# choi403/ALG

Measured on AMD Instinct MI355X. Metric: frames/sec (whole node) CogVideoX-5B-I2V 49f x 50-step ALG, higher is better.
Workload: dtype bf16; 1 GPU; BASELINE config 2: CogVideoX-5B-I2V bf16, 49 frames @ 480x720, 50 steps, ALG interval down_up (resize_factor 0.25, interval [0, 0.04]), guidance 6.0; one video per GPU; layers=42, dit_sample_forwards=12, parallelism=dp1

## Files before the change

alg_amd/_lib.py:

```python
from __future__ import annotations

import ctypes
from collections import OrderedDict
import os
from ctypes import POINTER, Structure, byref, c_char_p, c_float, c_int, c_int32, c_int64, c_void_p

import torch

_HERE = os.path.dirname(os.path.abspath(__file__))
LIB_PATH = os.environ.get("ALG_HIP_LIB") or os.path.join(_HERE, "libalg_hip.so")

ALG_F32, ALG_BF16 = 0, 1
ACT_NONE, ACT_GELU_TANH, ACT_SILU = 0, 1, 2
GEMM_BIAS_PER_ROW, GEMM_PERMUTE_COLS, GEMM_GATE_F32, GEMM_GATE_SEG_STRIDE = 1, 4, 8, 16
GEMM_B_PACKED11 = 32

EXPORTS = (
    "alg_version", "alg_last_error", "alg_reload_env", "alg_down_up", "alg_gaussian_blur", "alg_cfg_ddim_step", "alg_gemm_bf16", "alg_gemm_bf16_pair", "alg_gemm_bf16_pair_qk", "alg_pack_b_p11", "alg_pack_b_p11_bytes",
    "alg_flash_attn_d64", "alg_layernorm_modulate", "alg_qk_norm_rope", "alg_patchify", "alg_unpatchify",
    "alg_timestep_embedding", "alg_cfg_combine", "alg_lincomb", "alg_unipc_update", "alg_concat_cast", "alg_flash_attn_d128", "alg_layernorm_mod_f32", "alg_layernorm_mod_f32_fp8", "alg_rmsnorm_rope",
    "alg_wan_modulation", "alg_patchify3d", "alg_unpatchify3d", "alg_timestep_embedding_f32", "alg_linear_f32",
    "alg_gelu_erf", "alg_layernorm_modulate_seg", "alg_headnorm_rope", "alg_masked_mean", "alg_silu", "alg_gemm_fp8", "alg_quantize_fp8_rows",
    "alg_conv_cl_bf16", "alg_vae_groupnorm_workspace", "alg_vae_groupnorm_stats", "alg_vae_spatial_norm", "alg_vae_upsample",
    "alg_vae_pack_latent", "alg_vae_unpack_video", "alg_vae_group_norm", "alg_vae_pad", "alg_vae_repitch",
    "alg_vae_unpack_planes", "alg_rms_norm_rows", "alg_softmax_hilo", "alg_flash_attn_d128_ex", "alg_flash_attn_d128_dual", "alg_rope_half", "alg_patchify_t", "alg_unpatchify_t", "alg_qk_norm_rope_scaled", "alg_flash_attn_d64_ex", "alg_embed_rows", "alg_t5_layernorm", "alg_attn_bias", "alg_mul_bf16", "alg_quick_gelu",
    "alg_lowpass_tables_bytes", "alg_lowpass_tables_build", "alg_down_up_workspace_bytes", "alg_gaussian_blur_workspace_bytes",
    "alg_flash_attn_d64_workspace_bytes", "alg_calib_mfma_bf16", "alg_wall_clock_khz", "alg_attn_clock_tap",
)
_RET_I64 = ("alg_vae_groupnorm_workspace", "alg_lowpass_tables_bytes", "alg_down_up_workspace_bytes",
            "alg_gaussian_blur_workspace_bytes", "alg_flash_attn_d64_workspace_bytes", "alg_pack_b_p11_bytes")


class AlgHipError(RuntimeError):
    pass


class GemmArgs(Structure):
    _fields_ = [
        ("A", c_void_p), ("B", c_void_p), ("C", c_void_p), ("bias", c_void_p), ("R", c_void_p), ("gate", c_void_p),
        ("lda", c_int64), ("ldb", c_int64), ("ldc", c_int64), ("ldr", c_int64),
        ("strideA", c_int64), ("strideB", c_int64), ("strideC", c_int64), ("strideR", c_int64),
        ("strideGate", c_int64),
        ("M", c_int32), ("N", c_int32), ("K", c_int32), ("batch", c_int32),
        ("seg_split", c_int32), ("act", c_int32), ("flags", c_int32),
        ("gate_seg_stride", c_int64), ("perm_col0", c_int32), ("conv_cin_log2", c_int32),
        ("a_scale", c_void_p), ("b_scale", c_void_p), ("strideAScale", c_int64), ("strideBScale", c_int64),
        ("conv_wp", c_int32), ("conv_hpwp", c_int32), ("conv_kw", c_int32), ("reserved1", c_int32),
    ]


class QkNormRopeArgs(Structure):
    _fields_ = [("wq", c_void_p), ("bq", c_void_p), ("wk", c_void_p), ("bk", c_void_p), ("cos_tab", c_void_p),
                ("sin_tab", c_void_p), ("heads", c_int32), ("text_len", c_int32), ("eps", c_float),
                ("q_scale", c_float)]


class VaeGeom(Structure):
    _fields_ = [(n, c_int32) for n in ("frames", "H", "W", "C", "first_len", "seg_len", "lat_first_single", "lat_rate",
                                       "lat_scale", "lat_h", "lat_w")]


_lib = None


def build_library(verbose=False):
    import subprocess

    src = os.path.join(_HERE, "csrc")
    r = subprocess.run(["make", "-C", src, "-j8"], capture_output=True, text=True)
    if verbose or r.returncode != 0:
        print(r.stdout[-4000:])
        print(r.stderr[-4000:])
    if r.returncode != 0:
        raise AlgHipError("building libalg_hip.so failed (see output above)")
    return LIB_PATH


def load_library():
    global _lib
    if _lib is not None:
        return _lib
    if not os.path.exists(LIB_PATH):
        raise AlgHipError(
            "%s not found: the HIP extension is not built (run `python -c 'import __graft_entry__ as g; g.build()'` "
            "or `make -C alg_amd/csrc`).  There is no CPU fallback for the ALG hot path." % LIB_PATH)
    lib = ctypes.CDLL(LIB_PATH)
    lib.alg_version.restype = c_int
    lib.alg_last_error.restype = c_char_p
    lib.alg_reload_env.restype = None
    lib.alg_reload_env.argtypes = []
    lib.alg_down_up.argtypes = [c_void_p, c_void_p, c_int64, c_int, c_int, c_int, c_int, c_int, c_int, c_void_p, c_void_p,
                                c_int64, c_void_p]
    lib.alg_gaussian_blur.argtypes = [c_void_p, c_void_p, c_int64, c_int, c_int, c_int, c_float, c_int, c_void_p, c_int64,
                                      c_void_p]
    lib.alg_lowpass_tables_bytes.argtypes = [c_int] * 4
    lib.alg_lowpass_tables_build.argtypes = [c_void_p, c_int64] + [c_int] * 4 + [c_void_p]
    lib.alg_down_up_workspace_bytes.argtypes = [c_int64] + [c_int] * 4
    lib.alg_gaussian_blur_workspace_bytes.argtypes = [c_int64] + [c_int] * 3
    lib.alg_flash_attn_d64_workspace_bytes.argtypes = [c_int] * 4
    lib.alg_pack_b_p11_bytes.argtypes = [c_int, c_int]
    lib.alg_pack_b_p11_bytes.restype = c_int64
    lib.alg_pack_b_p11.argtypes = [c_void_p, c_void_p, c_int, c_int, c_int64, c_void_p]
    lib.alg_cfg_ddim_step.argtypes = [c_void_p, c_int, c_void_p, c_int, c_int, c_int64, c_float, c_float, c_float,
                                      c_float, c_float, c_void_p]
    lib.alg_cfg_combine.argtypes = [c_void_p, c_void_p, c_int, c_int, c_int64, c_float, c_void_p]
    lib.alg_lincomb.argtypes = [POINTER(c_void_p), POINTER(c_float), POINTER(c_int), c_int, c_void_p, c_int, c_int64,
                                c_void_p]
    lib.alg_concat_cast.argtypes = [POINTER(c_void_p), c_int, POINTER(c_void_p), c_int, c_int] + [c_int64] * 7 + [
        c_void_p, c_int, c_void_p]
    lib.alg_flash_attn_d128.argtypes = [c_void_p] * 4 + [c_int] * 4 + [c_int64] * 8 + [c_float, c_void_p]
    lib.alg_flash_attn_d128_ex.argtypes = [c_void_p] * 4 + [c_int] * 4 + [c_int64] * 8 + [c_float, c_int, c_int, c_void_p]
    lib.alg_flash_attn_d128_dual.argtypes = ([c_void_p] * 3 + [c_int] + [c_int64] * 4 + [c_void_p] * 2 + [c_int] + [c_int64] * 4 +
                                             [c_void_p] + [c_int] * 3 + [c_int64] * 4 + [c_float, c_void_p])
    lib.alg_rope_half.argtypes = [c_void_p, c_void_p, c_void_p, c_void_p, c_int64, c_int, c_int64, c_void_p]
    lib.alg_layernorm_mod_f32.argtypes = [c_void_p] * 6 + [c_int64, c_int, c_int, c_int, c_float, c_void_p]
    lib.alg_layernorm_mod_f32_fp8.argtypes = [c_void_p] * 7 + [c_int64, c_int, c_int, c_int, c_float, c_void_p]
    lib.alg_rmsnorm_rope.argtypes = [c_void_p] * 4 + [c_int64, c_int, c_int, c_int, c_float, c_void_p]
    lib.alg_wan_modulation.argtypes = [c_void_p] * 3 + [c_int] * 5 + [c_void_p]
    lib.alg_patchify3d.argtypes = [c_void_p, c_void_p] + [c_int] * 8 + [c_void_p]
    lib.alg_unpatchify3d.argtypes = [c_void_p, c_int64, c_void_p] + [c_int] * 8 + [c_void_p]
    lib.alg_layernorm_modulate_seg.argtypes = [c_void_p] * 6 + [c_int64, c_int64, c_int, c_int, c_int, c_int64, c_int64,
                                               c_int, c_float, c_void_p]
    lib.alg_headnorm_rope.argtypes = [c_void_p] * 4 + [c_int64, c_int64, c_int, c_int, c_int, c_int, c_float, c_void_p]
    lib.alg_masked_mean.argtypes = [c_void_p, c_void_p, c_void_p, c_int, c_int, c_int, c_void_p]
    lib.alg_silu.argtypes = [c_void_p, c_void_p, c_int64, c_void_p]
    lib.alg_rms_norm_rows.argtypes = [c_void_p, c_void_p, c_void_p, c_int64, c_int, c_int, c_int, c_void_p]
    lib.alg_softmax_hilo.argtypes = [c_void_p, c_void_p, c_void_p, c_int64, c_int, c_int64, ctypes.c_float, c_void_p]
    lib.alg_gemm_fp8.argtypes = [POINTER(GemmArgs), c_void_p]
    lib.alg_conv_cl_bf16.argtypes = [c_void_p] * 5 + [c_int] * 7 + [c_void_p]
    lib.alg_vae_groupnorm_workspace.argtypes = [POINTER(VaeGeom)]
    lib.alg_vae_groupnorm_stats.argtypes = [c_void_p, POINTER(VaeGeom), c_float, c_void_p, c_void_p, c_void_p]
    lib.alg_vae_spatial_norm.argtypes = [c_void_p] * 6 + [POINTER(VaeGeom), c_int, c_void_p]
    lib.alg_vae_group_norm.argtypes = [c_void_p] * 5 + [POINTER(VaeGeom), c_int, c_void_p]
    lib.alg_vae_pad.argtypes = [c_void_p, c_void_p] + [c_int] * 4 + [c_void_p]
    lib.alg_vae_repitch.argtypes = [c_void_p, c_void_p] + [c_int] * 6 + [c_void_p]
    lib.alg_vae_unpack_planes.argtypes = [c_void_p, c_void_p] + [c_int] * 4 + [c_void_p]
    lib.alg_embed_rows.argtypes = [c_void_p, c_void_p, c_void_p, c_int64, c_int, c_int, c_void_p]
    lib.alg_t5_layernorm.argtypes = [c_void_p, c_void_p, c_void_p, c_int64, c_int, c_float, c_void_p]
    lib.alg_attn_bias.argtypes = [c_void_p] * 7 + [c_int, c_int, c_int, c_int, c_int64, c_int64, c_float, c_int, c_void_p]
    lib.alg_quick_gelu.argtypes = [c_void_p, c_int64, c_void_p]
    lib.alg_mul_bf16.argtypes = [c_void_p, c_void_p, c_void_p, c_int64, c_void_p]
    lib.alg_vae_upsample.argtypes = [c_void_p, c_void_p] + [c_int] * 6 + [c_void_p]
    lib.alg_vae_pack_latent.argtypes = [c_void_p, c_int64, c_int64, c_void_p, c_int, c_int, c_int, c_int, c_float, c_void_p]
    lib.alg_vae_unpack_video.argtypes = [c_void_p, c_void_p, c_int, c_int, c_int, c_int, c_void_p]
    lib.alg_quantize_fp8_rows.argtypes = [c_void_p, c_int64, c_void_p, c_void_p, c_int64, c_int, c_void_p]
    lib.alg_timestep_embedding_f32.argtypes = [c_void_p, c_void_p, c_int, c_int, c_void_p]
    lib.alg_linear_f32.argtypes = [c_void_p] * 6 + [c_int] * 4 + [c_void_p]
    lib.alg_gelu_erf.argtypes = [c_void_p, c_int64, c_void_p]
    lib.alg_unipc_update.argtypes = [c_void_p] * 5 + [c_int64] + [c_float] * 6 + [c_void_p]
    lib.alg_gemm_bf16.argtypes = [POINTER(GemmArgs), c_void_p]
    lib.alg_gemm_bf16_pair.argtypes = [POINTER(GemmArgs), POINTER(GemmArgs), c_void_p]
    lib.alg_gemm_bf16_pair_qk.argtypes = [POINTER(GemmArgs), POINTER(GemmArgs), POINTER(QkNormRopeArgs), c_void_p]
    lib.alg_flash_attn_d64.argtypes = [c_void_p, c_void_p, c_void_p, c_void_p, c_int, c_int, c_int, c_int64, c_int64,
                                       c_int64, c_int64, c_int64, c_int64, c_float, c_void_p]
    lib.alg_layernorm_modulate.argtypes = [c_void_p, c_void_p, c_void_p, c_void_p, c_void_p, c_void_p, c_int64, c_int,
                                           c_int, c_int, c_int64, c_int64, c_int, c_float, c_void_p]
    lib.alg_qk_norm_rope.argtypes = [c_void_p, c_void_p, c_void_p, c_void_p, c_void_p, c_void_p, c_void_p, c_int,
                                     c_int, c_int, c_int, c_float, c_void_p]
    lib.alg_qk_norm_rope_scaled.argtypes = [c_void_p] * 7 + [c_int, c_int, c_int, c_int, c_float, c_float, c_void_p]
    lib.alg_flash_attn_d64_ex.argtypes = [c_void_p, c_void_p, c_void_p, c_void_p, c_int, c_int, c_int, c_int64, c_int64,
                                          c_int64, c_int64, c_int64, c_int64, c_float, c_int, c_void_p, c_int64, c_void_p]
    lib.alg_patchify.argtypes = [c_void_p, c_int64, POINTER(c_void_p), c_void_p, c_int, c_int, c_int, c_int, c_int,
                                 c_int, c_void_p]
    lib.alg_unpatchify.argtypes = [c_void_p, c_void_p, c_int, c_int, c_int, c_int, c_int, c_int, c_void_p]
    lib.alg_patchify_t.argtypes = [c_void_p, c_int64, POINTER(c_void_p), c_void_p] + [c_int] * 7 + [c_void_p]
    lib.alg_unpatchify_t.argtypes = [c_void_p, c_void_p] + [c_int] * 7 + [c_void_p]
    lib.alg_timestep_embedding.argtypes = [c_void_p, c_void_p, c_int, c_int, c_int, c_void_p]
    lib.alg_calib_mfma_bf16.argtypes = [c_void_p, c_int, ctypes.c_uint, c_int, c_void_p, c_void_p]
    lib.alg_attn_clock_tap.argtypes = [c_void_p, c_int]
    for name in EXPORTS:
        fn = getattr(lib, name)
        if name == "alg_attn_clock_tap":
            fn.restype = None
        elif name not in ("alg_version", "alg_last_error", "alg_reload_env"):
            fn.restype = c_int64 if name in _RET_I64 else c_int
    _lib = lib
    return lib


def reload_env():
    load_library().alg_reload_env()


def _check(rc, what):
    if rc != 0:
        msg = load_library().alg_last_error()
        raise AlgHipError("%s failed (code %d): %s" % (what, rc, msg.decode() if msg else "?"))


def _stream():
    return c_void_p(torch.cuda.current_stream().cuda_stream)


def _dt(t):
    if t.dtype == torch.float32:
        return ALG_F32
    if t.dtype == torch.bfloat16:
        return ALG_BF16
    raise AlgHipError("unsupported dtype %s (the HIP path handles float32 and bfloat16)" % t.dtype)


def _dev(t, name):
    if not t.is_cuda:
        raise AlgHipError("%s must be a device tensor: the ALG hot path is HIP-only (no CPU fallback)" % name)
    return t


def _ptr(t):
    return c_void_p(t.data_ptr()) if t is not None else c_void_p(0)



_TABLES = OrderedDict()
_TABLES_MAX = 64
_SCRATCH = {}
_PINNED = {}


def _stream_key(t):
    return (t.device.index, torch.cuda.current_stream(t.device).cuda_stream)


def _capturing():
    return torch.cuda.is_available() and torch.cuda.is_current_stream_capturing()


def _pin(t):
    _PINNED[id(t)] = t
    return t


def release_captured_buffers():
    _PINNED.clear()


def clear_caches():
    _TABLES.clear()
    _SCRATCH.clear()


def lowpass_tables(x, h1, w1):
    lib = load_library()
    H, W = x.shape[-2:]
    key = _stream_key(x) + (H, W, h1, w1)
    cap = _capturing()
    t = _TABLES.get(key)
    if t is not None:
        _TABLES.move_to_end(key)
        return _pin(t) if cap else t
    n = int(lib.alg_lowpass_tables_bytes(H, W, h1, w1))
    if n <= 0:
        return None
    t = torch.empty(n, dtype=torch.uint8, device=x.device)
    _check(lib.alg_lowpass_tables_build(_ptr(t), n, H, W, h1, w1, _stream()), "alg_lowpass_tables_build")
    if cap:
        return _pin(t)
    _TABLES[key] = t
    while len(_TABLES) > _TABLES_MAX:
        _TABLES.popitem(last=False)
    return t


def scratch(ref, nbytes, tag):
    if nbytes <= 0:
        return None
    key = _stream_key(ref) + (tag,)
    t = _SCRATCH.get(key)
    cap = _capturing()
    if t is None or t.numel() < nbytes:
        t = torch.empty(int(nbytes), dtype=torch.uint8, device=ref.device)
        if cap:
            return _pin(t)
        _SCRATCH[key] = t
    return _pin(t) if cap else t


def calib_mfma_bf16(sink, iters, seed=1, blocks=0, clocks=None):
    lib = load_library()
    if clocks is not None:
        if int(blocks) <= 0:
            blocks = 2 * torch.cuda.get_device_properties(sink.device).multi_processor_count
        if not (clocks.is_cuda and clocks.device == sink.device and clocks.dtype == torch.int64 and clocks.is_contiguous()
                and clocks.numel() >= 4 * int(blocks)):
            raise AlgHipError("calib_mfma_bf16: clocks must be a contiguous int64 tensor on the sink's device with >= 4 * %d "
                              "elements" % int(blocks))
    rc = lib.alg_calib_mfma_bf16(_ptr(_dev(sink, "sink")), int(iters), int(seed), int(blocks), _ptr(clocks), _stream())
    if rc <= 0:
        _check(rc if rc < 0 else -1, "alg_calib_mfma_bf16")
    return rc


def wall_clock_khz():
    return int(load_library().alg_wall_clock_khz())


def attn_clock_tap(buffer):
    lib = load_library()
    if buffer is None:
        lib.alg_attn_clock_tap(None, 0)
        return
    if not (buffer.is_cuda and buffer.dtype == torch.int64 and buffer.is_contiguous() and buffer.dim() == 2 and buffer.shape[1] == 4):
        raise AlgHipError("attn_clock_tap needs a contiguous int64 device tensor [slots, 4]")
    lib.alg_attn_clock_tap(_ptr(buffer), int(buffer.shape[0]))


def clock_mhz_from_taps(taps, wall_khz):
    t = taps.detach().cpu().to(torch.float64)
    dc, dw = t[:, 2] - t[:, 0], t[:, 3] - t[:, 1]
    ok = (dc > 0) & (dw > 0)
    if not bool(ok.any()) or wall_khz <= 0:
        return None
    mhz = dc[ok] / dw[ok] * (wall_khz / 1e3)
    return {"mean": float(mhz.mean()), "min": float(mhz.min()), "max": float(mhz.max()), "workgroups": int(ok.sum())}


def down_up(x, h1, w1, round_intermediate=True):
    lib = load_library()
    _dev(x, "x")
    if not x.is_contiguous():
        raise AlgHipError("down_up needs a contiguous tensor")
    H, W = x.shape[-2:]
    planes = x.numel() // (H * W) if x.numel() else 0
    out = torch.empty_like(x)
    if planes == 0:
        return out
    wsb = int(lib.alg_down_up_workspace_bytes(planes, H, W, h1, w1))
    ws = scratch(x, wsb, "down_up")
    tables = lowpass_tables(x, h1, w1) if wsb == 0 else None
    _check(lib.alg_down_up(_ptr(x), _ptr(out), planes, H, W, h1, w1, _dt(x), 1 if round_intermediate else 0,
                           _ptr(tables), _ptr(ws), wsb, _stream()), "alg_down_up")
    return out


def gaussian_blur(x, ksize, sigma):
    lib = load_library()
    _dev(x, "x")
    if not x.is_contiguous():
        raise AlgHipError("gaussian_blur needs a contiguous tensor")
    H, W = x.shape[-2:]
    planes = x.numel() // (H * W) if x.numel() else 0
    out = torch.empty_like(x)
    wsb = int(lib.alg_gaussian_blur_workspace_bytes(planes, H, W, int(ksize))) if planes else 0
    ws = scratch(x, wsb, "gaussian")
    _check(lib.alg_gaussian_blur(_ptr(x), _ptr(out), planes, H, W, int(ksize), float(sigma), _dt(x), _ptr(ws), wsb,
                                 _stream()), "alg_gaussian_blur")
    return out


def cfg_ddim_step_(pred, latents, n_pass, guidance_scale, sqrt_alpha_t, sqrt_beta_t, coef_a, coef_b):
    lib = load_library()
    _dev(pred, "pred")
    _dev(latents, "latents")
    if not (pred.is_contiguous() and latents.is_contiguous()):
        raise AlgHipError("cfg_ddim_step_ needs contiguous tensors")
    numel = latents.numel()
    if pred.numel() != n_pass * numel:
        raise AlgHipError("pred has %d elements, expected n_pass*numel = %d" % (pred.numel(), n_pass * numel))
    _check(lib.alg_cfg_ddim_step(_ptr(pred), _dt(pred), _ptr(latents), _dt(latents), n_pass, numel,
                                 float(guidance_scale), float(sqrt_alpha_t), float(sqrt_beta_t), float(coef_a),
                                 float(coef_b), _stream()), "alg_cfg_ddim_step")
    return latents


def cfg_combine(pred, n_pass, guidance_scale):
    lib = load_library()
    _dev(pred, "pred")
    if not pred.is_contiguous() or pred.shape[0] % n_pass:
        raise AlgHipError("cfg_combine needs a contiguous [n_pass * B, ...] tensor")
    out = torch.empty((pred.shape[0] // n_pass,) + tuple(pred.shape[1:]), device=pred.device, dtype=pred.dtype)
    _check(lib.alg_cfg_combine(_ptr(pred), _ptr(out), _dt(pred), n_pass, out.numel(), float(guidance_scale), _stream()),
           "alg_cfg_combine")
    return out


def lincomb(terms, out_dtype, out=None):
    lib = load_library()
    xs = [t for _, t in terms]
    for t in xs:
        _dev(t, "term")
        if not t.is_contiguous() or t.shape != xs[0].shape:
            raise AlgHipError("lincomb needs contiguous tensors of one shape")
    n = len(xs)
    if out is None:
        out = torch.empty(xs[0].shape, device=xs[0].device, dtype=out_dtype)
    elif out.dtype != out_dtype or out.shape != xs[0].shape or not out.is_contiguous():
        raise AlgHipError("lincomb: `out` must be a contiguous tensor of the requested dtype and shape")
    arr = (c_void_p * n)(*[t.data_ptr() for t in xs])
    cf = (c_float * n)(*[float(c) for c, _ in terms])
    dts = (c_int * n)(*[_dt(t) for t in xs])
    _check(lib.alg_lincomb(arr, cf, dts, n, _ptr(out), ALG_F32 if out_dtype == torch.float32 else ALG_BF16,
                           out.numel(), _stream()), "alg_lincomb")
    return out


def concat_cast(src0, src1, O, A0, A1, R, s0_ostride, s1_ostride, a1_off, out_dtype):
    lib = load_library()
    n = len(src0)
    for t in list(src0) + list(src1):
        _dev(t, "concat source")
        if not t.is_contiguous():
            raise AlgHipError("concat_cast needs contiguous sources")
    out = torch.empty((n, O, A0 + A1, R), device=src0[0].device, dtype=out_dtype)
    a0 = (c_void_p * n)(*[t.data_ptr() for t in src0])
    a1 = (c_void_p * n)(*[t.data_ptr() for t in src1])
    _check(lib.alg_concat_cast(a0, _dt(src0[0]), a1, _dt(src1[0]), n, O, A0, A1, R, s0_ostride, s1_ostride, a1_off,
                               _ptr(out), ALG_F32 if out_dtype == torch.float32 else ALG_BF16, _stream()),
           "alg_concat_cast")
    return out


def rope_half_(x, cos, sin, pos, rows, heads, x_rstride, x_off=0):
    _check(load_library().alg_rope_half(_p(x, x_off), _p(cos), _p(sin), _p(pos), rows, heads, x_rstride, _stream()),
           "alg_rope_half")
    return x


def flash_attn_d128_dual(q, k, vt, Skv, k_bs, k_rs, vt_bs, vt_rs, k2, vt2, Skv2, k2_bs, k2_rs, vt2_bs, vt2_rs, o, batch, heads, Sq,
                         q_bs, q_rs, o_bs, o_rs, scale):
    lib = load_library()
    for t in (q, k, vt, k2, vt2, o):
        _dev(t, "attention operand")
    _check(lib.alg_flash_attn_d128_dual(_p(q), _p(k), _p(vt), Skv, k_bs, k_rs, vt_bs, vt_rs, _p(k2), _p(vt2), Skv2, k2_bs, k2_rs,
                                        vt2_bs, vt2_rs, _p(o), batch, heads, Sq, q_bs, q_rs, o_bs, o_rs, float(scale), _stream()),
           "alg_flash_attn_d128_dual")
    return o


def flash_attn_d128(q, k, vt, o, batch, heads, Sq, Skv, q_bs, q_rs, k_bs, k_rs, vt_bs, vt_rs, o_bs, o_rs, scale,
                    q_off=0, k_off=0, vt_off=0, o_off=0, kv_group=1, causal=False):
    lib = load_library()
    for t in (q, k, vt, o):
        _dev(t, "attention operand")
    at = lambda t, off: c_void_p(t.data_ptr() + 2 * off)
    if kv_group != 1 or causal:
        _check(lib.alg_flash_attn_d128_ex(at(q, q_off), at(k, k_off), at(vt, vt_off), at(o, o_off), batch, heads, Sq, Skv, q_bs,
                                          q_rs, k_bs, k_rs, vt_bs, vt_rs, o_bs, o_rs, float(scale), int(kv_group),
                                          int(bool(causal)), _stream()), "alg_flash_attn_d128_ex")
        return o
    _check(lib.alg_flash_attn_d128(at(q, q_off), at(k, k_off), at(vt, vt_off), at(o, o_off), batch, heads, Sq, Skv, q_bs, q_rs, k_bs, k_rs, vt_bs, vt_rs, o_bs, o_rs, float(scale),
                                   _stream()), "alg_flash_attn_d128")
    return o


def _p(t, off=0):
    if t is None:
        return c_void_p(0)
    _dev(t, "tensor")
    return c_void_p(t.data_ptr() + off * t.element_size())


def layernorm_mod_f32(x, y, weight, bias, scale, shift, mod_bstride, batch, rows, D, eps, scale_off=0, shift_off=0):
    _check(load_library().alg_layernorm_mod_f32(_p(x), _p(y), _p(weight), _p(bias), _p(scale, scale_off),
                                                _p(shift, shift_off), mod_bstride, batch, rows, D, float(eps), _stream()),
           "alg_layernorm_mod_f32")
    return y


def layernorm_mod_f32_fp8(x, q8, q8_scale, weight, bias, scale, shift, mod_bstride, batch, rows, D, eps, scale_off=0,
                          shift_off=0):
    _check(load_library().alg_layernorm_mod_f32_fp8(_p(x), _p(q8), _p(q8_scale), _p(weight), _p(bias),
                                                    _p(scale, scale_off), _p(shift, shift_off), mod_bstride, batch, rows,
                                                    D, float(eps), _stream()), "alg_layernorm_mod_f32_fp8")
    return q8


def rmsnorm_rope_(x, weight, cos, sin, x_rstride, batch, rows, D, eps, x_off=0):
    _check(load_library().alg_rmsnorm_rope(_p(x, x_off), _p(weight), _p(cos), _p(sin), x_rstride, batch, rows, D,
                                           float(eps), _stream()), "alg_rmsnorm_rope")
    return x


def wan_modulation(table, vec, out, layers, batch, J, D, vec_per_j):
    _check(load_library().alg_wan_modulation(_p(table), _p(vec), _p(out), layers, batch, J, D, int(vec_per_j), _stream()),
           "alg_wan_modulation")
    return out


def patchify3d(x, out, n, C, F, H, W, ph, pw, Kpad):
    _check(load_library().alg_patchify3d(_p(x), _p(out), n, C, F, H, W, ph, pw, Kpad, _stream()), "alg_patchify3d")
    return out


def unpatchify3d(x, ldin, out, n, C, F, H, W, ph, pw, channel_major=False):
    _check(load_library().alg_unpatchify3d(_p(x), ldin, _p(out), n, C, F, H, W, ph, pw, int(channel_major), _stream()),
           "alg_unpatchify3d")
    return out


def layernorm_modulate_seg(x, y, weight, bias, scale, shift, mod_bstride, seg_stride, batch, rows, D, seg_split, eps,
                           x_bstride=None, y_bstride=None, x_off=0, y_off=0, scale_off=0, shift_off=0):
    x_bstride = rows * D if x_bstride is None else x_bstride
    y_bstride = rows * D if y_bstride is None else y_bstride
    _check(load_library().alg_layernorm_modulate_seg(_p(x, x_off), _p(y, y_off), _p(weight), _p(bias), _p(scale, scale_off),
                                                     _p(shift, shift_off), mod_bstride, seg_stride, batch, rows, D,
                                                     x_bstride, y_bstride, seg_split, float(eps), _stream()),
           "alg_layernorm_modulate_seg")
    return y


def headnorm_rope_(x, weight, cos, sin, x_rstride, x_bstride, batch, rows, heads, rope_tokens, eps, x_off=0):
    _check(load_library().alg_headnorm_rope(_p(x, x_off), _p(weight), _p(cos), _p(sin), x_rstride, x_bstride, batch, rows,
                                            heads, rope_tokens, float(eps), _stream()), "alg_headnorm_rope")
    return x


def masked_mean(x, valid, out, batch, L, D):
    _check(load_library().alg_masked_mean(_p(x), _p(valid), _p(out), batch, L, D, _stream()), "alg_masked_mean")
    return out


def silu(x, y):
    _check(load_library().alg_silu(_p(x), _p(y), x.numel(), _stream()), "alg_silu")
    return y


def rms_norm_rows(x, gamma, y, rows, C, Cp, silu=True):
    _check(load_library().alg_rms_norm_rows(_p(x), _p(gamma), _p(y), rows, C, Cp, int(silu), _stream()), "alg_rms_norm_rows")
    return y


def softmax_hilo(neg_hi, lo, p, rows, cols, ld, scale):
    _check(load_library().alg_softmax_hilo(_p(neg_hi), _p(lo), _p(p), rows, cols, ld, float(scale), _stream()),
           "alg_softmax_hilo")
    return p


CONV_PLAIN, CONV_PAIR, CONV_STRIDE2 = 0, 1, 2


def conv_cl(x, w, bias, res, y, frames, Hp, Wp, Cin, Cout, kt, pair=False, stride2=False, x_off=0, y_off=0, res_off=0):
    mode = CONV_STRIDE2 if stride2 else (CONV_PAIR if pair else CONV_PLAIN)
    _check(load_library().alg_conv_cl_bf16(_p(x, x_off), _p(w), _p(bias), _p(res, res_off), _p(y, y_off), frames, Hp, Wp,
                                           Cin, Cout, kt, mode, _stream()), "alg_conv_cl_bf16")
    return y


def embed_rows(ids, table, out):
    _check(load_library().alg_embed_rows(_p(ids), _p(table), _p(out), ids.numel(), table.shape[1], table.shape[0],
                                         _stream()), "alg_embed_rows")
    return out


def t5_layernorm(x, weight, y, rows, D, eps):
    _check(load_library().alg_t5_layernorm(_p(x), _p(weight), _p(y), rows, D, eps, _stream()), "alg_t5_layernorm")
    return y


def attn_bias(qkv, out, bias_table, rel_bucket, key_mask, batch, heads, L, scale=1.0, head_dim=64, causal=False):
    inner = heads * head_dim
    _check(load_library().alg_attn_bias(_p(qkv), _p(qkv, inner), _p(qkv, 2 * inner), _p(out), _p(bias_table),
                                        _p(rel_bucket), _p(key_mask), batch, heads, head_dim, L, 3 * inner, inner,
                                        float(scale), int(causal), _stream()), "alg_attn_bias")
    return out


def quick_gelu_(x):
    _check(load_library().alg_quick_gelu(_p(x), x.numel(), _stream()), "alg_quick_gelu")
    return x


def mul_bf16(a, b, out):
    _check(load_library().alg_mul_bf16(_p(a), _p(b), _p(out), a.numel(), _stream()), "alg_mul_bf16")
    return out


def vae_group_norm(x, stats, gamma, beta, out, g, silu=True):
    _check(load_library().alg_vae_group_norm(_p(x), _p(stats), _p(gamma), _p(beta), _p(out), byref(g), int(silu),
                                             _stream()), "alg_vae_group_norm")
    return out


def vae_pad(x, out, frames, H, W, C):
    _check(load_library().alg_vae_pad(_p(x), _p(out), frames, H, W, C, _stream()), "alg_vae_pad")
    return out


def vae_repitch(x, out, frames, H, W, C, src_rows, src_wp):
    _check(load_library().alg_vae_repitch(_p(x), _p(out), frames, H, W, C, src_rows, src_wp, _stream()), "alg_vae_repitch")
    return out


def vae_unpack_planes(x, out, frames, H, W, C):
    _check(load_library().alg_vae_unpack_planes(_p(x), _p(out), frames, H, W, C, _stream()), "alg_vae_unpack_planes")
    return out


def pack_conv_pair(w, bias, taps_t):
    co = w.shape[0]
    w = w.reshape(co, taps_t, 3, 3, -1)
    wp = w.new_zeros(2, co, taps_t, 3, 4, w.shape[-1])
    wp[0, :, :, :, 0:3] = w
    wp[1, :, :, :, 1:4] = w
    return wp.reshape(2 * co, -1).contiguous(), torch.cat([bias, bias]).contiguous()


def vae_geom(**kw):
    g = VaeGeom()
    for k, v in kw.items():
        setattr(g, k, v)
    return g


def vae_groupnorm_workspace(g):
    n = load_library().alg_vae_groupnorm_workspace(byref(g))
    if n < 0:
        _check(1, "alg_vae_groupnorm_workspace")
    return n


def vae_groupnorm_stats(x, g, eps, workspace, stats):
    _check(load_library().alg_vae_groupnorm_stats(_p(x), byref(g), eps, _p(workspace), _p(stats), _stream()),
           "alg_vae_groupnorm_stats")
    return stats


def vae_spatial_norm(x, stats, gamma, beta, zyb, out, g, silu=True):
    _check(load_library().alg_vae_spatial_norm(_p(x), _p(stats), _p(gamma), _p(beta), _p(zyb), _p(out), byref(g),
                                               int(silu), _stream()), "alg_vae_spatial_norm")
    return out


def vae_upsample(x, out, frames_out, H, W, C, compress_time, first_single):
    _check(load_library().alg_vae_upsample(_p(x), _p(out), frames_out, H, W, C, int(compress_time), int(first_single),
                                           _stream()), "alg_vae_upsample")
    return out


def vae_pack_latent(z, c_stride, frame_stride, out, frames, h, w, channels, scale, z_off=0):
    _check(load_library().alg_vae_pack_latent(_p(z, z_off), c_stride, frame_stride, _p(out), frames, h, w, channels, scale,
                                              _stream()), "alg_vae_pack_latent")
    return out


def vae_unpack_video(x, out, frames, H, W, to_uint8=False):
    _check(load_library().alg_vae_unpack_video(_p(x), _p(out), frames, H, W, int(to_uint8), _stream()),
           "alg_vae_unpack_video")
    return out


def timestep_embedding_f32(t, out, n, dim):
    _check(load_library().alg_timestep_embedding_f32(_p(t), _p(out), n, dim, _stream()), "alg_timestep_embedding_f32")
    return out


def linear_f32(x, W, b, y, y_bf16, y_silu_bf16, M, N, K, act=0):
    _check(load_library().alg_linear_f32(_p(x), _p(W), _p(b), _p(y), _p(y_bf16), _p(y_silu_bf16), M, N, K, act, _stream()),
           "alg_linear_f32")


def gelu_erf_(x):
    _check(load_library().alg_gelu_erf(_p(x), x.numel(), _stream()), "alg_gelu_erf")
    return x


def unipc_update(x, m0, m1, m_new, r, c, k, rk=1.0, rho0=0.0, rho_new=0.0):
    lib = load_library()
    for t in (x, m0, m1, m_new):
        if t is None:
            continue
        _dev(t, "unipc term")
        if t.dtype != torch.float32 or not t.is_contiguous() or t.shape != x.shape:
            raise AlgHipError("unipc_update needs contiguous fp32 tensors of one shape")
    out = torch.empty_like(x)
    p = lambda t: None if t is None else _ptr(t)
    _check(lib.alg_unipc_update(p(x), p(m0), p(m1), p(m_new), _ptr(out), x.numel(), float(r), float(c), float(k),
                                float(rk), float(rho0), float(rho_new), _stream()), "alg_unipc_update")
    return out


def gemm_args(A, B, C, M, N, K, lda, ldb, ldc, bias=None, R=None, ldr=0, gate=None, batch=1, strideA=0, strideB=0,
              strideC=0, strideR=0, strideGate=0, seg_split=0, act=ACT_NONE, flags=0, a_off=0, b_off=0, c_off=0, r_off=0,
              gate_off=0, gate_seg_stride=None, bias_off=0, perm_col0=0, a_scale=None, b_scale=None, strideAScale=0,
              strideBScale=0, a_scale_off=0, b_scale_off=0):
    args = GemmArgs()
    fp8 = a_scale is not None
    if isinstance(B, PackedB):
        if fp8:
            raise AlgHipError("a packed B holds bf16 weight fragments for GEMM schedule 11: the e4m3 GEMM takes a row-major B")
        if (B.N, B.K) != (N, K) or b_off or strideB:
            raise AlgHipError("packed B was built for N = %d, K = %d (shared by the batch, no offset)" % (B.N, B.K))
        flags |= GEMM_B_PACKED11
    args.A = A.data_ptr() + A.element_size() * a_off
    args.B = B.data_ptr() + B.element_size() * b_off
    if fp8:
        args.a_scale = a_scale.data_ptr() + 4 * a_scale_off
        args.b_scale = b_scale.data_ptr() + 4 * b_scale_off
        args.strideAScale, args.strideBScale = strideAScale, strideBScale
    args.C = C.data_ptr() + 2 * c_off
    args.bias = (bias.data_ptr() + 2 * bias_off) if bias is not None else None
    if gate_seg_stride is not None:
        flags |= GEMM_GATE_SEG_STRIDE
        args.gate_seg_stride = gate_seg_stride
    args.R = (R.data_ptr() + 2 * r_off) if R is not None else None
    args.gate = (gate.data_ptr() + gate.element_size() * gate_off) if gate is not None else None
    args.lda, args.ldb, args.ldc, args.ldr = lda, ldb, ldc, ldr
    args.strideA, args.strideB, args.strideC, args.strideR, args.strideGate = strideA, strideB, strideC, strideR, strideGate
    args.M, args.N, args.K, args.batch = M, N, K, batch
    args.seg_split, args.act, args.flags = seg_split, act, flags
    args.perm_col0 = perm_col0
    return args, fp8


class PackedB:

    def __init__(self, w):
        lib = load_library()
        _dev(w, "weight")
        if w.dtype != torch.bfloat16 or w.dim() != 2 or w.stride(1) != 1:
            raise AlgHipError("PackedB takes a 2-D bf16 weight with unit column stride")
        self.N, self.K = int(w.shape[0]), int(w.shape[1])
        nbytes = int(lib.alg_pack_b_p11_bytes(self.N, self.K))
        if nbytes <= 0:
            raise AlgHipError("PackedB: K = %d must be a positive multiple of 64" % self.K)
        self.data = torch.empty(nbytes, dtype=torch.uint8, device=w.device)
        _check(lib.alg_pack_b_p11(_ptr(w), _ptr(self.data), self.N, self.K, int(w.stride(0)), _stream()), "alg_pack_b_p11")

    def data_ptr(self):
        return self.data.data_ptr()

    def element_size(self):
        return 2


def gemm(*a, **kw):
    lib = load_library()
    args, fp8 = gemm_args(*a, **kw)
    if fp8:
        _check(lib.alg_gemm_fp8(ctypes.byref(args), _stream()), "alg_gemm_fp8")
    else:
        _check(lib.alg_gemm_bf16(ctypes.byref(args), _stream()), "alg_gemm_bf16")


def gemm_pair(first, second):
    lib = load_library()
    a, fa = gemm_args(*first[0], **first[1])
    b, fb = gemm_args(*second[0], **second[1])
    if fa or fb:
        raise AlgHipError("gemm_pair takes bf16 problems")
    _check(lib.alg_gemm_bf16_pair(ctypes.byref(a), ctypes.byref(b), _stream()), "alg_gemm_bf16_pair")


def gemm_pair_qk(first, second, wq, bq, wk, bk, cos, sin, heads, text_len, eps, q_scale=1.0):
    lib = load_library()
    a, fa = gemm_args(*first[0], **first[1])
    b, fb = gemm_args(*second[0], **second[1])
    if fa or fb:
        raise AlgHipError("gemm_pair_qk takes bf16 problems")
    ptrs = [t.data_ptr() if t is not None else None for t in (wq, bq, wk, bk, cos, sin)]
    e = QkNormRopeArgs(*ptrs, heads, text_len, float(eps), float(q_scale))
    _check(lib.alg_gemm_bf16_pair_qk(ctypes.byref(a), ctypes.byref(b), ctypes.byref(e), _stream()), "alg_gemm_bf16_pair_qk")


def quantize_fp8_rows(x, q, scale, rows, K, x_rstride=None, x_off=0, q_off=0, scale_off=0):
    x_rstride = K if x_rstride is None else x_rstride
    _check(load_library().alg_quantize_fp8_rows(_p(x, x_off), x_rstride, _p(q, q_off), _p(scale, scale_off), rows, K,
                                                _stream()), "alg_quantize_fp8_rows")
    return q, scale


ATTN_Q_PRESCALED = 1


def flash_attn_d64(q, k, vt, o, batch, heads, S, q_bstride, q_rstride, vt_bstride, vt_rstride, o_bstride, o_rstride,
                   scale, q_off=0, k_off=0, q_prescaled=False):
    lib = load_library()
    flags = ATTN_Q_PRESCALED if q_prescaled else 0
    wsb = int(lib.alg_flash_attn_d64_workspace_bytes(batch, heads, S, flags))
    ws = scratch(o, wsb, "attn_d64")
    _check(lib.alg_flash_attn_d64_ex(c_void_p(q.data_ptr() + 2 * q_off), c_void_p(k.data_ptr() + 2 * k_off), _ptr(vt),
                                     _ptr(o), batch, heads, S, q_bstride, q_rstride, vt_bstride, vt_rstride, o_bstride,
                                     o_rstride, float(scale), flags, _ptr(ws), wsb, _stream()),
           "alg_flash_attn_d64")


def layernorm_modulate(x, y, weight, bias, scale, shift, mod_bstride, batch, rows, D, seg_split, eps,
                       x_bstride=None, y_bstride=None, x_off=0, y_off=0, scale_off=0, shift_off=0):
    lib = load_library()
    x_bstride = rows * D if x_bstride is None else x_bstride
    y_bstride = rows * D if y_bstride is None else y_bstride
    sc = c_void_p(scale.data_ptr() + 2 * scale_off) if scale is not None else c_void_p(0)
    sh = c_void_p(shift.data_ptr() + 2 * shift_off) if shift is not None else c_void_p(0)
    _check(lib.alg_layernorm_modulate(c_void_p(x.data_ptr() + 2 * x_off), c_void_p(y.data_ptr() + 2 * y_off),
                                      _ptr(weight), _ptr(bias), sc, sh, mod_bstride, batch, rows, D, x_bstride,
                                      y_bstride, seg_split, float(eps), _stream()), "alg_layernorm_modulate")


def qk_norm_rope_(qk, wq, bq, wk, bk, cos, sin, batch, S, heads, text_len, eps, q_scale=1.0):
    lib = load_library()
    _check(lib.alg_qk_norm_rope_scaled(_ptr(qk), _ptr(wq), _ptr(bq), _ptr(wk), _ptr(bk), _ptr(cos), _ptr(sin), batch, S,
                                       heads, text_len, float(eps), float(q_scale), _stream()), "alg_qk_norm_rope")


def patchify(latents, lat_bstride, conds, out, n_samples, frames, C, H, W, p, p_t=1):
    lib = load_library()
    arr = (c_void_p * n_samples)(*[c.data_ptr() for c in conds])
    _check(lib.alg_patchify_t(_ptr(latents), lat_bstride, arr, _ptr(out), n_samples, frames, C, H, W, p, p_t, _stream()),
           "alg_patchify")


def unpatchify(x, out, n_samples, frames, C, H, W, p, p_t=1):
    lib = load_library()
    _check(lib.alg_unpatchify_t(_ptr(x), _ptr(out), n_samples, frames, C, H, W, p, p_t, _stream()), "alg_unpatchify")


def timestep_embedding(t, out, n, dim, flip_sin_to_cos=True):
    lib = load_library()
    _check(lib.alg_timestep_embedding(_ptr(t), _ptr(out), n, dim, 1 if flip_sin_to_cos else 0, _stream()),
           "alg_timestep_embedding")
```

alg_amd/csrc/capi.hip:

```cpp
#include <stdarg.h>
#include <stdlib.h>
#include <string.h>

#include "common.h"

namespace alg {

static thread_local char g_err[512] = "";

void set_error(const char* fmt, ...) {
  va_list ap;
  va_start(ap, fmt);
  vsnprintf(g_err, sizeof(g_err), fmt, ap);
  va_end(ap);
}

int check_launch(const char* what) {
  hipError_t e = hipGetLastError();
  if (e != hipSuccess) {
    set_error("%s: launch failed: %s", what, hipGetErrorString(e));
    return ALG_ELAUNCH;
  }
  return ALG_OK;
}

struct OptDef {
  const char* name;
  int def;
  int n_ok;
  int ok[4];
};
static const OptDef g_defs[OPT_COUNT] = {
    {"ALG_ATTN_SPLIT_TAIL", 1, 2, {0, 1}},
    {"ALG_ATTN_PP", 4, 3, {0, 4, 7}},
    {"ALG_ATTN_VARIANT", 33, 2, {1, 33}},
    {"ALG_ATTN128_PIPE", 1, 2, {0, 1}},
    {"ALG_ATTN128_Q64", 1, 4, {0, 1, 2, 3}},
    {"ALG_GEMM_PIPE", 10, 3, {6, 9, 10}},
    {"ALG_LOWPASS_PATH", 0, 0, {}},
};
static std::atomic<int> g_opt[OPT_COUNT];

static void load_options() {
  for (int i = 0; i < OPT_COUNT; ++i) {
    const OptDef& d = g_defs[i];
    int v = d.def;
    const char* e = getenv(d.name);
    if (e && *e) {
      char* end = nullptr;
      const long x = strtol(e, &end, 10);
      bool ok = end != e && *end == '\0' && x >= -2147483647L && x <= 2147483647L && (d.n_ok == 0);
      if (end != e && *end == '\0')
        for (int j = 0; j < d.n_ok; ++j) ok |= d.ok[j] == x;
      if (ok) v = (int)x;
    }
    g_opt[i].store(v, std::memory_order_relaxed);
  }
}
namespace {
struct OptInit {
  OptInit() { load_options(); }
} g_opt_init;
}

int opt(Opt o) { return g_opt[o].load(std::memory_order_relaxed); }

}

extern "C" void alg_reload_env(void) { alg::load_options(); }
extern "C" int alg_version(void) { return ALG_VERSION; }
extern "C" const char* alg_last_error(void) { return alg::g_err; }
```

alg_amd/csrc/gemm.hip:

```cpp
#include <stdlib.h>

#include "common.h"

namespace alg {
constexpr int BM = 256, BN = 256;
int launch_gemm_p6(const alg_gemm_args* a, int m_tiles, int n_tiles, int64_t nwg, hipStream_t s);
int launch_gemm_p9(const alg_gemm_args* a, int m_tiles, int n_tiles, int64_t nwg, hipStream_t s);
int launch_gemm_p9_pair(const alg_gemm_args* a, int m_tiles_a, int n_tiles_a, const alg_gemm_args* b, int m_tiles_b, int n_tiles_b,
                        hipStream_t s);
int launch_gemm_p9_pair_qk(const alg_gemm_args* a, int m_tiles_a, int n_tiles_a, const alg_gemm_args* b, int m_tiles_b, int n_tiles_b,
                           const alg_qk_norm_rope_args* e, hipStream_t s);
int launch_gemm_p10(const alg_gemm_args* a, int m_tiles, int n_tiles, int64_t nwg, hipStream_t s);
int launch_gemm_p10_pair(const alg_gemm_args* a, int m_tiles_a, int n_tiles_a, const alg_gemm_args* b, int m_tiles_b, int n_tiles_b,
                         hipStream_t s);
int launch_gemm_p10_pair_qk(const alg_gemm_args* a, int m_tiles_a, int n_tiles_a, const alg_gemm_args* b, int m_tiles_b, int n_tiles_b,
                            const alg_qk_norm_rope_args* e, hipStream_t s);
int launch_gemm_p11(const alg_gemm_args* a, int m_tiles, int n_tiles, int64_t nwg, hipStream_t s);
int launch_gemm_p6_fp8(const alg_gemm_args* a, int m_tiles, int n_tiles, int64_t nwg, hipStream_t s);
int launch_gemm_p9_fp8(const alg_gemm_args* a, int m_tiles, int n_tiles, int64_t nwg, hipStream_t s);
int launch_gemm_p6_conv(const alg_gemm_args* a, int m_tiles, int n_tiles, int64_t nwg, hipStream_t s);
static int gemm_pipe() { return opt(OPT_GEMM_PIPE); }
static bool asm_pipe() { return gemm_pipe() == 9 || gemm_pipe() == 10; }
}

using namespace alg;

static int gemm_entry(const alg_gemm_args* a, void* stream, bool fp8, bool validate_only = false) {
  if (!a || !a->A || !a->B || !a->C) {
    set_error("alg_gemm_bf16: null argument");
    return ALG_EINVAL;
  }
  if (a->M <= 0 || a->N <= 0 || a->K <= 0 || a->batch <= 0) {
    set_error("alg_gemm_bf16: bad shape M=%d N=%d K=%d batch=%d", a->M, a->N, a->K, a->batch);
    return ALG_EINVAL;
  }
  if (a->K % (fp8 ? 128 : 64) != 0) {
    set_error("alg_gemm_%s: K=%d must be a multiple of %d", fp8 ? "fp8" : "bf16", a->K, fp8 ? 128 : 64);
    return ALG_EINVAL;
  }
  const int al = fp8 ? 16 : 8;
  if (a->lda % al || a->ldb % al || a->strideA % al || a->strideB % al || ((uintptr_t)a->A & 15) ||
      ((uintptr_t)a->B & 15)) {
    set_error("alg_gemm: A/B must be 16-byte aligned with lda/ldb/strides multiples of 16 bytes");
    return ALG_EINVAL;
  }
  if (fp8 && (!a->a_scale || !a->b_scale || ((uintptr_t)a->b_scale & 15) || (a->strideBScale & 3))) {
    set_error("alg_gemm_fp8: a_scale / b_scale are required (b_scale 16-byte aligned)");
    return ALG_EINVAL;
  }
  if (a->act < ALG_ACT_NONE || a->act > ALG_ACT_SILU) {
    set_error("alg_gemm_bf16: unknown activation %d", a->act);
    return ALG_EINVAL;
  }
  if ((a->flags & ALG_GEMM_PERMUTE_COLS) && (a->R || a->gate)) {
    set_error("alg_gemm_bf16: PERMUTE_COLS cannot be combined with residual/gate");
    return ALG_EINVAL;
  }
  if (a->R && a->act != ALG_ACT_NONE) {
    set_error("alg_gemm_bf16: an activation cannot be combined with the residual epilogue");
    return ALG_EINVAL;
  }
  if (a->gate && !a->R) {
    set_error("alg_gemm_bf16: gate needs a residual");
    return ALG_EINVAL;
  }
  if ((a->N & 3) == 0) {
    const bool bad = (a->ldc & 3) || (a->strideC & 3) || ((uintptr_t)a->C & 7) ||
                     (a->bias && !(a->flags & ALG_GEMM_BIAS_PER_ROW) && ((uintptr_t)a->bias & 7)) ||
                     (a->R && ((a->ldr & 3) || (a->strideR & 3) || ((uintptr_t)a->R & 7))) ||
                     (a->gate && ((a->strideGate & 3) ||
                                  ((uintptr_t)a->gate & ((a->flags & ALG_GEMM_GATE_F32) ? 15 : 7))));
    if (bad) {
      set_error("alg_gemm_bf16: C/bias/R/gate must be 8-byte aligned with ldc/ldr/strides multiples of 4 elements");
      return ALG_EINVAL;
    }
  }
  if (a->conv_wp) {
    const int cl = a->conv_cin_log2;
    const int taps = (cl >= 6 && cl <= 12) ? a->K >> cl : 0;
    const int kw = a->conv_kw;
    if (fp8 || (kw != 3 && kw != 4) || (taps != 3 * kw && taps != 9 * kw) || (taps << cl) != a->K ||
        (a->lda != ((int64_t)(kw - 2) << cl) && !(kw == 3 && a->lda == (2ll << cl))) || a->conv_wp < 3 ||
        a->conv_hpwp < 3 * a->conv_wp || a->act != ALG_ACT_NONE ||
        ((2ll * a->conv_hpwp + 2ll * a->conv_wp + 3) << cl) >= (1ll << 31)) {
      set_error("alg_gemm_bf16: bad convolution addressing (cin_log2=%d K=%d lda=%lld wp=%d hpwp=%d)", cl, a->K,
                (long long)a->lda, a->conv_wp, a->conv_hpwp);
      return ALG_EINVAL;
    }
  }
  if (a->flags & ALG_GEMM_B_PACKED11) {
    if (fp8) {
      set_error("alg_gemm_fp8: a packed B (ALG_GEMM_B_PACKED11) holds bf16 fragments for schedule 11; the e4m3 GEMM reads a row-major B");
      return ALG_EINVAL;
    }
    if (a->conv_wp) {
      set_error("alg_gemm_bf16: convolution addressing cannot be combined with a packed B (ALG_GEMM_B_PACKED11)");
      return ALG_EINVAL;
    }
    if (a->K < 128 || 256 * a->lda * 2 + (int64_t)a->K * 2 >= (1ll << 32) || a->strideB != 0 ||
        (a->flags & (ALG_GEMM_BIAS_PER_ROW | ALG_GEMM_PERMUTE_COLS)) || ((uintptr_t)a->B & 15)) {
      set_error("alg_gemm_bf16: a packed B (ALG_GEMM_B_PACKED11) needs K >= 128, 32-bit byte offsets inside a 256-row A panel, a B shared by "
                "the batch (strideB = 0) and a plain column layout (no per-row bias / column permutation)");
      return ALG_EINVAL;
    }
  }
  if (validate_only) return ALG_OK;
  if ((int64_t)a->M * a->ldc >= (1ll << 31) || (a->R && (int64_t)a->M * a->ldr >= (1ll << 31))) {
    const int64_t ld = (a->R && a->ldr > a->ldc) ? a->ldr : a->ldc;
    const int64_t rows = ((1ll << 31) - 1) / ld / BM * BM;
    if (a->conv_wp || rows <= 0) {
      set_error("alg_gemm_bf16: M*ldc must stay below 2^31 (32-bit epilogue offsets)");
      return ALG_ELIMIT;
    }
    const int64_t esz = fp8 ? 1 : 2;
    for (int64_t m0 = 0; m0 < a->M; m0 += rows) {
      alg_gemm_args c = *a;
      c.M = (int32_t)((a->M - m0) < rows ? (a->M - m0) : rows);
      c.A = (const char*)a->A + m0 * a->lda * esz;
      c.C = (char*)a->C + m0 * a->ldc * 2;
      if (a->R) c.R = (const char*)a->R + m0 * a->ldr * 2;
      if (a->bias && (a->flags & ALG_GEMM_BIAS_PER_ROW)) c.bias = (const char*)a->bias + m0 * 2;
      if (a->a_scale) c.a_scale = a->a_scale + m0;
      c.seg_split = a->seg_split > m0 ? (int32_t)(a->seg_split - m0) : 0;
      const int rc = gemm_entry(&c, stream, fp8);
      if (rc != ALG_OK) return rc;
    }
    return ALG_OK;
  }
  const int m_tiles = (a->M + BM - 1) / BM, n_tiles = (a->N + BN - 1) / BN;
  const int64_t nwg = (int64_t)m_tiles * n_tiles * a->batch;
  if (nwg > 0x7fffffff) {
    set_error("alg_gemm_bf16: grid too large");
    return ALG_ELIMIT;
  }
  hipStream_t s = (hipStream_t)stream;
  if (fp8) {
    if (asm_pipe() && a->K >= 256 && 256 * a->lda + (int64_t)a->K < (1ll << 32) && 256 * a->ldb + (int64_t)a->K < (1ll << 32))
      return launch_gemm_p9_fp8(a, m_tiles, n_tiles, nwg, s);
    return launch_gemm_p6_fp8(a, m_tiles, n_tiles, nwg, s);
  }
  if (a->conv_wp) return launch_gemm_p6_conv(a, m_tiles, n_tiles, nwg, s);
  if (a->flags & ALG_GEMM_B_PACKED11) return launch_gemm_p11(a, m_tiles, n_tiles, nwg, s);
  switch (gemm_pipe()) {
    case 9:
    case 10:
      if (a->K >= 128 && 256 * a->lda * 2 + (int64_t)a->K * 2 < (1ll << 32) && 256 * a->ldb * 2 + (int64_t)a->K * 2 < (1ll << 32))
        return gemm_pipe() == 10 ? launch_gemm_p10(a, m_tiles, n_tiles, nwg, s) : launch_gemm_p9(a, m_tiles, n_tiles, nwg, s);
      return launch_gemm_p6(a, m_tiles, n_tiles, nwg, s);
    default: return launch_gemm_p6(a, m_tiles, n_tiles, nwg, s);
  }
}

extern "C" int alg_gemm_bf16(const alg_gemm_args* a, void* stream) { return gemm_entry(a, stream, false); }

static bool pair_eligible(const alg_gemm_args* a) {
  return a && a->A && a->B && a->C && !(a->flags & ALG_GEMM_B_PACKED11) && !a->R && !a->gate && a->act == ALG_ACT_NONE &&
         !a->conv_wp && a->M > 0 && a->N > 0 && a->batch > 0 && a->K >= 128 && a->K % 64 == 0 && 256 * a->lda * 2 + (int64_t)a->K * 2 < (1ll << 32) &&
         256 * a->ldb * 2 + (int64_t)a->K * 2 < (1ll << 32) && (int64_t)a->M * a->ldc < (1ll << 31) &&
         !(a->lda % 8 || a->ldb % 8 || a->strideA % 8 || a->strideB % 8 || ((uintptr_t)a->A & 15) || ((uintptr_t)a->B & 15)) &&
         ((a->N & 3) != 0 || !((a->ldc & 3) || (a->strideC & 3) || ((uintptr_t)a->C & 7) ||
                               (a->bias && !(a->flags & ALG_GEMM_BIAS_PER_ROW) && ((uintptr_t)a->bias & 7))));
}

extern "C" int alg_gemm_bf16_pair(const alg_gemm_args* a, const alg_gemm_args* b, void* stream) {
  int rc = gemm_entry(a, stream, false, true);
  if (rc == ALG_OK) rc = gemm_entry(b, stream, false, true);
  if (rc != ALG_OK) return rc;
  if (asm_pipe() && pair_eligible(a) && pair_eligible(b)) {
    const int64_t ta = (int64_t)((a->M + BM - 1) / BM) * ((a->N + BN - 1) / BN) * a->batch;
    const int64_t tb = (int64_t)((b->M + BM - 1) / BM) * ((b->N + BN - 1) / BN) * b->batch;
    if (ta + tb <= 0x7fffffff)
      return (gemm_pipe() == 10 ? launch_gemm_p10_pair : launch_gemm_p9_pair)(a, (a->M + BM - 1) / BM, (a->N + BN - 1) / BN, b, (b->M + BM - 1) / BM, (b->N + BN - 1) / BN,
                                 (hipStream_t)stream);
  }
  rc = gemm_entry(a, stream, false);
  return rc != ALG_OK ? rc : gemm_entry(b, stream, false);
}

extern "C" int alg_gemm_bf16_pair_qk(const alg_gemm_args* a, const alg_gemm_args* b, const alg_qk_norm_rope_args* e, void* stream) {
  int rc = gemm_entry(a, stream, false, true);
  if (rc == ALG_OK) rc = gemm_entry(b, stream, false, true);
  if (rc != ALG_OK) return rc;
  if (!e || !e->wq || !e->bq || !e->wk || !e->bk || e->heads <= 0 || e->text_len < 0 || e->text_len > a->M ||
      (e->cos_tab == nullptr) != (e->sin_tab == nullptr)) {
    set_error("alg_gemm_bf16_pair_qk: bad LayerNorm / rotary arguments");
    return ALG_EINVAL;
  }
  if (((uintptr_t)e->wq & 15) || ((uintptr_t)e->bq & 15) || ((uintptr_t)e->wk & 15) || ((uintptr_t)e->bk & 15) ||
      ((uintptr_t)e->cos_tab & 15) || ((uintptr_t)e->sin_tab & 15) || ((uintptr_t)a->C & 15)) {
    set_error("alg_gemm_bf16_pair_qk: pointers must be 16-byte aligned");
    return ALG_EINVAL;
  }
  if (a->N != 2 * e->heads * 64 || a->ldc != a->N || a->strideC != (int64_t)a->M * a->N || (a->flags & ALG_GEMM_PERMUTE_COLS) ||
      a->R || a->act != ALG_ACT_NONE) {
    set_error("alg_gemm_bf16_pair_qk: qk must be a plain GEMM onto the contiguous [batch][S][2][heads][64] tensor (N=%d heads=%d ldc=%lld)",
              a->N, e->heads, (long long)a->ldc);
    return ALG_EINVAL;
  }
  const bool fused = asm_pipe() && pair_eligible(a) && pair_eligible(b) && e->heads % 4 == 0 &&
                     !(a->bias && (a->flags & ALG_GEMM_BIAS_PER_ROW));
  if (fused) {
    const int64_t ta = (int64_t)((a->M + BM - 1) / BM) * ((a->N + BN - 1) / BN) * a->batch;
    const int64_t tb = (int64_t)((b->M + BM - 1) / BM) * ((b->N + BN - 1) / BN) * b->batch;
    if (ta + tb <= 0x7fffffff)
      return (gemm_pipe() == 10 ? launch_gemm_p10_pair_qk : launch_gemm_p9_pair_qk)(a, (a->M + BM - 1) / BM, (a->N + BN - 1) / BN, b, (b->M + BM - 1) / BM, (b->N + BN - 1) / BN, e,
                                    (hipStream_t)stream);
  }
  rc = alg_gemm_bf16_pair(a, b, stream);
  if (rc != ALG_OK) return rc;
  return alg_qk_norm_rope_scaled(a->C, e->wq, e->bq, e->wk, e->bk, e->cos_tab, e->sin_tab, a->batch, a->M, e->heads, e->text_len,
                                 e->eps, e->q_scale, stream);
}

extern "C" int alg_gemm_fp8(const alg_gemm_args* a, void* stream) { return gemm_entry(a, stream, true); }

extern "C" int alg_conv_cl_bf16(const void* x, const void* w, const void* bias, const void* res, void* y, int frames,
                                int Hp, int Wp, int Cin, int Cout, int kt, int mode, void* stream) {
  const bool pair = mode == ALG_CONV_PAIR, down = mode == ALG_CONV_STRIDE2;
  if (frames <= 0 || Hp < 3 || Wp < 3 || (kt != 1 && kt != 3) || Cin < 64 || (Cin & (Cin - 1)) || Cout <= 0 || (Cout & 3) ||
      mode < 0 || mode > ALG_CONV_STRIDE2 || (pair && (((Hp * Wp) & 1) || Cout > 128)) ||
      (down && (kt != 1 || (Hp & 1) || (Wp & 1)))) {
    set_error("alg_conv_cl_bf16: bad shape frames=%d Hp=%d Wp=%d Cin=%d Cout=%d kt=%d (Cin a power of two >= 64, Cout %% 4 == 0)",
              frames, Hp, Wp, Cin, Cout, kt);
    return ALG_EINVAL;
  }
  alg_gemm_args a = {};
  a.A = x, a.B = w, a.C = y, a.bias = bias, a.R = res;
  const int vox = pair ? 2 : 1, kw = pair ? 4 : 3;
  a.lda = (int64_t)vox * Cin, a.ldb = (int64_t)kt * 3 * kw * Cin, a.ldc = (int64_t)vox * Cout, a.ldr = a.ldc;
  a.strideA = (int64_t)Hp * Wp * Cin, a.strideB = 0, a.strideC = (int64_t)Hp * Wp * Cout, a.strideR = a.strideC;
  a.M = Hp * Wp / vox, a.N = vox * Cout, a.K = kt * 3 * kw * Cin, a.batch = frames;
  a.act = ALG_ACT_NONE;
  a.conv_cin_log2 = __builtin_ctz((unsigned)Cin), a.conv_wp = Wp, a.conv_hpwp = Hp * Wp, a.conv_kw = kw;
  if (down) {
    a.A = (const bf16_t*)x + (int64_t)(Wp + 1) * Cin;
    a.lda = 2ll * Cin;
    a.M = (Hp - 2) / 2 * Wp;
    a.strideC = a.strideR = (int64_t)a.M * Cout;
  }
  return gemm_entry(&a, stream, false);
}
```

alg_amd/csrc/gemm_kernel.h:

```cpp
#pragma once
#include <stdlib.h>

#include <type_traits>

#include "common.h"
#include "qk_norm_rope.h"
#ifdef ALG_P9_LOOP_INC
#include ALG_P9_LOOP_INC
#else
#include "gemm_p9_loop.inc"
#endif
#include "gemm_p9_fp8_loop.inc"
#ifdef ALG_P11_LOOP_INC
#include ALG_P11_LOOP_INC
#else
#include "gemm_p11_loop.inc"
#endif
#ifdef ALG_P10_LOOP_INC
#include ALG_P10_LOOP_INC
#else
#include "gemm_p10_loop.inc"
#endif

#ifndef ALG_FP8_MX
#define ALG_FP8_MX 1
#endif

namespace alg {

#ifdef ALG_ABL_NOSTORE
#define ALG_STORE16(ptr, val) asm volatile("" ::"v"((val).x), "v"((val).y), "v"((val).z), "v"((val).w))
#else
#define ALG_STORE16(ptr, val) (*(uint4*)(ptr) = (val))
#endif
#ifdef ALG_GEMM_TAP
static __device__ uint64_t gemm_tap_buf[1024 * 4];
static inline int gemm_tap_read(uint64_t* host) { return hipMemcpyFromSymbol(host, HIP_SYMBOL(gemm_tap_buf), sizeof(uint64_t) * 4096) == hipSuccess ? 0 : -1; }
#endif

#ifndef ALG_AUX_A
#define ALG_AUX_A 0
#endif
#ifndef ALG_AUX_B
#define ALG_AUX_B 0
#endif
constexpr int BM = 256, BN = 256;
constexpr int GEMM_LDS = 128 * 1024;
constexpr int GEMM_LDS_P9 = 160 * 1024;
constexpr int GROUP_M = 8;

template <int V>
struct IntC { static constexpr int value = V; };

template <typename F, int... I>
__device__ __forceinline__ void static_for_impl(F&& f, std::integer_sequence<int, I...>) {
  (f(IntC<I>{}), ...);
}
template <int N, typename F>
__device__ __forceinline__ void static_for(F&& f) {
  static_for_impl(f, std::make_integer_sequence<int, N>{});
}

template <int BLK>
__device__ __forceinline__ f32x16 read_acc_block() {
  float f[16];
  asm volatile("v_accvgpr_read_b32 %0, a[%c16]\n\tv_accvgpr_read_b32 %1, a[%c17]\n\tv_accvgpr_read_b32 %2, a[%c18]\n\t"
               "v_accvgpr_read_b32 %3, a[%c19]\n\tv_accvgpr_read_b32 %4, a[%c20]\n\tv_accvgpr_read_b32 %5, a[%c21]\n\t"
               "v_accvgpr_read_b32 %6, a[%c22]\n\tv_accvgpr_read_b32 %7, a[%c23]\n\tv_accvgpr_read_b32 %8, a[%c24]\n\t"
               "v_accvgpr_read_b32 %9, a[%c25]\n\tv_accvgpr_read_b32 %10, a[%c26]\n\tv_accvgpr_read_b32 %11, a[%c27]\n\t"
               "v_accvgpr_read_b32 %12, a[%c28]\n\tv_accvgpr_read_b32 %13, a[%c29]\n\tv_accvgpr_read_b32 %14, a[%c30]\n\t"
               "v_accvgpr_read_b32 %15, a[%c31]\n\ts_nop 0"
               : "=v"(f[0]), "=v"(f[1]), "=v"(f[2]), "=v"(f[3]), "=v"(f[4]), "=v"(f[5]), "=v"(f[6]), "=v"(f[7]), "=v"(f[8]),
                 "=v"(f[9]), "=v"(f[10]), "=v"(f[11]), "=v"(f[12]), "=v"(f[13]), "=v"(f[14]), "=v"(f[15])
               : "n"(BLK * 16), "n"(BLK * 16 + 1), "n"(BLK * 16 + 2), "n"(BLK * 16 + 3), "n"(BLK * 16 + 4), "n"(BLK * 16 + 5),
                 "n"(BLK * 16 + 6), "n"(BLK * 16 + 7), "n"(BLK * 16 + 8), "n"(BLK * 16 + 9), "n"(BLK * 16 + 10),
                 "n"(BLK * 16 + 11), "n"(BLK * 16 + 12), "n"(BLK * 16 + 13), "n"(BLK * 16 + 14), "n"(BLK * 16 + 15)
               : ALG_GEMM_P9_ACC_CLOBBERS);
  f32x16 r;
#pragma unroll
  for (int e = 0; e < 16; ++e) r[e] = f[e];
  return r;
}

typedef const __attribute__((address_space(1))) void* gptr_t;
typedef __attribute__((address_space(3))) void* lptr_t;

__device__ __forceinline__ float act_apply(float x, int act) {
  if (act == ALG_ACT_GELU_TANH) {
    const float k1 = -2.0f * 1.4426950408889634f * 0.7978845608028654f, k2 = 0.044715f * k1;
    return x * __builtin_amdgcn_rcpf(1.0f + __builtin_amdgcn_exp2f(x * fmaf(k2, x * x, k1)));
  }
  if (act == ALG_ACT_SILU) {
    return x * __builtin_amdgcn_rcpf(1.0f + __builtin_amdgcn_exp2f(-1.4426950408889634f * x));
  }
  return x;
}

__device__ __forceinline__ void unpack4(const uint2 v, float (&f)[4]) {
  f[0] = __uint_as_float(v.x << 16);
  f[1] = __uint_as_float(v.x & 0xffff0000u);
  f[2] = __uint_as_float(v.y << 16);
  f[3] = __uint_as_float(v.y & 0xffff0000u);
}

struct GemmNoPair {};
struct GemmPairArgs {
  alg_gemm_args p;
  int m_tiles, n_tiles, group_m;
};
struct GemmPairQkArgs : GemmPairArgs {
  QkNormRope qe;
};
template <int PAIR> struct GemmPairT { typedef GemmNoPair type; };
template <> struct GemmPairT<1> { typedef GemmPairArgs type; };
template <> struct GemmPairT<2> { typedef GemmPairQkArgs type; };
template <int ACT, bool RES, int PIPE, int WNW = 4, bool FP8 = false, bool CONV = false, int PAIR = 0>
__global__ __launch_bounds__((PIPE == 11 ? 1 : 2) * WNW * 64) void gemm_bf16_kernel(
    const alg_gemm_args p1, int m_tiles1, int n_tiles1, int group_m1, const typename GemmPairT<PAIR>::type pr) {
  constexpr bool P9 = PIPE == 9 || PIPE == 10 || PIPE == 11;
  constexpr bool M16 = PIPE == 10 || PIPE == 11;
  constexpr bool P11 = PIPE == 11;
  constexpr int WMW = P11 ? 1 : 2;
  constexpr int MT = BM / WMW / 32;
  static_assert(!PAIR || (P9 && !P11 && !RES && ACT == ALG_ACT_NONE), "the pair launch is built for the plain schedule-9 / 10 kernels");
  static_assert(!FP8 || PIPE == 6 || PIPE == 9, "the fp8 operands are built on the ping-pong schedule and on schedule 9");
  static_assert(!CONV || (PIPE == 6 && !FP8), "the convolution addressing is built on the bf16 ping-pong schedule");
  typedef typename std::conditional<FP8, uint8_t, bf16_t>::type elem_t;
  constexpr int EPS = 16 / (int)sizeof(elem_t);
  constexpr int GEMM_THREADS = WMW * WNW * 64;
  constexpr int NT = BN / WNW / 32;
  static_assert(PIPE == 0 || PIPE == 6 || PIPE == 7 || PIPE == 8 || P9,
                "schedules built: 0 (2-stage ring), 6 (ping-pong), 7 (4-wave interleaved), 8 (4-wave BK = 32 ring), 9 / 10 (asm loops)");
  static_assert((PIPE == 7 || PIPE == 8 || PIPE == 9 || PIPE == 10) == (WNW == 2) && P11 == (WNW == 4 && WMW == 1),
                "PIPE 7 / 8 / 9 / 10 are the 2 x 2 4-wave layouts, 11 the 1 x 4 one, the others run 8 waves");
  static_assert(!P11 || (!FP8 && !CONV), "schedule 11 takes bf16 plain GEMM addressing with a packed B");
  static_assert(!P9 || !CONV, "schedules 9 / 10 take plain GEMM addressing (bf16, or e4m3 on 9 since round 4)");
  constexpr bool BK64 = true;
  constexpr bool PP = PIPE == 6;
  constexpr int BK = FP8 ? 128 : 64;
  constexpr int NSTAGE = 2;
  constexpr int ROW_BYTES = BK * (int)sizeof(elem_t);
  constexpr int SLOTS = ROW_BYTES / 16;
  constexpr int TILE_BYTES = BM * ROW_BYTES;
  constexpr int STAGE_BYTES = 2 * TILE_BYTES;
  constexpr int LD_PER_OP = TILE_BYTES / (GEMM_THREADS * 16);
  constexpr int ROWS_PER_LD = GEMM_THREADS / SLOTS;
  static_assert(NSTAGE * STAGE_BYTES == GEMM_LDS, "ring must fill the 128 KiB LDS budget");

  extern __shared__ __attribute__((aligned(16))) char smem[];
  const int tid = threadIdx.x;
  const int lane = tid & 63;
  const int wave = __builtin_amdgcn_readfirstlane(tid >> 6);
  const int wm = wave / WNW, wn = wave % WNW;

  constexpr int abl = 0;
#ifdef ALG_GEMM_TAP
  uint64_t tap_loop = 0, tap_tiles = 0;
  const uint64_t tap_c0 = __builtin_readcyclecounter(), tap_r0 = wall_clock64();
#endif
  group_m1 &= 0xffff;
  const int total1 = m_tiles1 * n_tiles1 * p1.batch;
  auto do_tile = [&](const int wg_in) __attribute__((always_inline)) {
  bool second = false;
  if constexpr (PAIR) second = wg_in >= total1;
  const alg_gemm_args& p = [&]() -> const alg_gemm_args& {
    if constexpr (PAIR) return second ? pr.p : p1;
    else return p1;
  }();
  int m_tiles = m_tiles1, n_tiles = n_tiles1, group_m = group_m1, wg = wg_in;
  if constexpr (PAIR) {
    if (second) m_tiles = pr.m_tiles, n_tiles = pr.n_tiles, group_m = pr.group_m, wg = wg_in - total1;
  }
  const int tiles = m_tiles * n_tiles;
  const int b = wg / tiles;
  int t = wg - b * tiles;
  const int grp = t / (group_m * n_tiles);
  const int first_m = grp * group_m;
  const int gsize = min(m_tiles - first_m, group_m);
  t -= grp * group_m * n_tiles;
  const int m0 = (first_m + t % gsize) * BM;
  const int n0 = (t / gsize) * BN;

  const elem_t* A = (const elem_t*)p.A + (int64_t)b * p.strideA;
  const elem_t* B = (const elem_t*)p.B + (int64_t)b * p.strideB;

  const int srow = tid / SLOTS;
  const int sw_src = !BK64 ? ((tid >> 4) & 3) : ((tid >> 4) & 7);
  const int sslot = (tid & (SLOTS - 1)) ^ sw_src;
  const elem_t* a_src[LD_PER_OP];
  const elem_t* b_src[LD_PER_OP];
#pragma unroll
  for (int i = 0; i < LD_PER_OP; ++i) {
    const int r = i * ROWS_PER_LD + srow;
    const int am = (abl & 8) ? 0 : m0, bn = (abl & 8) ? 0 : n0;
    a_src[i] = A + (int64_t)min(am + r, p.M - 1) * p.lda + sslot * EPS;
    b_src[i] = B + (int64_t)min(bn + r, p.N - 1) * p.ldb + sslot * EPS;
  }
  auto a_koff = [&](int kt) -> int {
    if constexpr (CONV) {
      const int cl = p.conv_cin_log2 - 6;
      const int tap = kt >> cl;
      const bool k4 = p.conv_kw == 4;
      const int dt = k4 ? tap / 12 : tap / 9, r9 = tap - dt * (k4 ? 12 : 9);
      const int dy = k4 ? r9 >> 2 : r9 / 3, dx = r9 - dy * (k4 ? 4 : 3);
      return ((dt * p.conv_hpwp + dy * p.conv_wp + dx) << p.conv_cin_log2) + (kt & ((1 << cl) - 1)) * BK;
    } else {
      return kt * BK;
    }
  };
  auto stage = [&](int buf, int kt) {
    char* base = smem + buf * STAGE_BYTES;
#pragma unroll
    for (int i = 0; i < LD_PER_OP; ++i) {
      __builtin_amdgcn_global_load_lds((gptr_t)(a_src[i] + kt * BK),
                                       (lptr_t)(base + (i * GEMM_THREADS + wave * 64) * 16), 16, 0, 0);
      __builtin_amdgcn_global_load_lds((gptr_t)(b_src[i] + kt * BK),
                                       (lptr_t)(base + TILE_BYTES + (i * GEMM_THREADS + wave * 64) * 16), 16, 0, 0);
    }
  };

  auto stage_piece = [&](int buf, int kt, int w) {
    char* base = smem + buf * STAGE_BYTES;
    const int i = w >> 1;
    if (w & 1)
      __builtin_amdgcn_global_load_lds((gptr_t)(b_src[i] + kt * BK),
                                       (lptr_t)(base + TILE_BYTES + (i * GEMM_THREADS + wave * 64) * 16), 16, 0, 0);
    else
      __builtin_amdgcn_global_load_lds((gptr_t)(a_src[i] + kt * BK),
                                       (lptr_t)(base + (i * GEMM_THREADS + wave * 64) * 16), 16, 0, 0);
  };

  const int l31 = lane & 31, h2 = lane >> 5;
  const int sw = !BK64 ? ((l31 >> 2) & 3) : ((l31 >> 1) & 7);
  const int a_row_off = (wm * 128 + l31) * ROW_BYTES;
  const int b_row_off = (wn * (NT * 32) + l31) * ROW_BYTES;
  auto pp_a_row = [&](int mt) { return ((mt >> 1) * 128 + wm * 64 + (mt & 1) * 32 + l31) * ROW_BYTES; };
  auto pp_b_row = [&](int nt) { return (nt * 128 + wn * 32 + l31) * ROW_BYTES; };

  auto fma_frag = [](const bf16x8 bfrag, const bf16x8 afrag, f32x16 c) -> f32x16 {
    if constexpr (FP8) {
      typedef long l2 __attribute__((ext_vector_type(2)));
      const l2 bq = __builtin_bit_cast(l2, bfrag), aq = __builtin_bit_cast(l2, afrag);
      c = __builtin_amdgcn_mfma_f32_32x32x16_fp8_fp8(bq[0], aq[0], c, 0, 0, 0);
      return __builtin_amdgcn_mfma_f32_32x32x16_fp8_fp8(bq[1], aq[1], c, 0, 0, 0);
    } else {
      return __builtin_amdgcn_mfma_f32_32x32x16_bf16(bfrag, afrag, c, 0, 0, 0);
    }
  };

  f32x16 acc[4][NT];
  if constexpr (!P9) {
#pragma unroll
    for (int i = 0; i < 4; ++i)
#pragma unroll
      for (int j = 0; j < NT; ++j)
#pragma unroll
        for (int e = 0; e < 16; ++e) acc[i][j][e] = 0.0f;
  }
  auto get_acc = [&](auto mt_c, auto nt_c) -> f32x16 {
    constexpr int mt = decltype(mt_c)::value, nt = decltype(nt_c)::value;
    if constexpr (P9)
      return read_acc_block<NT * mt + nt>();
    else
      return acc[mt][nt];
  };

  auto load_frags = [&](const char* As, const char* Bs, int ks, bf16x8 (&af)[4], bf16x8 (&bfr)[NT]) {
    const int so = ((2 * ks + h2) ^ sw) * 16;
#pragma unroll
    for (int nt = 0; nt < NT; ++nt) bfr[nt] = *(const bf16x8*)(Bs + b_row_off + nt * 32 * ROW_BYTES + so);
#pragma unroll
    for (int mt = 0; mt < 4; ++mt) af[mt] = *(const bf16x8*)(As + a_row_off + mt * 32 * ROW_BYTES + so);
  };
  auto mma = [&](const bf16x8 (&af)[4], const bf16x8 (&bfr)[NT]) {
#pragma unroll
    for (int mt = 0; mt < 4; ++mt)
#pragma unroll
      for (int nt = 0; nt < NT; ++nt)
        acc[mt][nt] = fma_frag(bfr[nt], af[mt], acc[mt][nt]);
  };
  auto compute = [&](int buf) {
    const char* As = smem + buf * STAGE_BYTES;
    const char* Bs = As + TILE_BYTES;
    constexpr int KS = BK / 16;
    bf16x8 af0[4], bf0[NT], af1[4], bf1[NT];
    load_frags(As, Bs, 0, af0, bf0);
    auto interleave = [&]() {
#pragma unroll
      for (int i = 0; i < 4 + NT; ++i) {
        __builtin_amdgcn_sched_group_barrier(0x008, 1, 0);
        __builtin_amdgcn_sched_group_barrier(0x100, 1, 0);
      }
      __builtin_amdgcn_sched_group_barrier(0x008, 4 * NT - (4 + NT), 0);
    };
    __builtin_amdgcn_sched_barrier(0);
#pragma unroll
    for (int ks = 0; ks < KS; ks += 2) {
      load_frags(As, Bs, ks + 1, af1, bf1);
      mma(af0, bf0);
      interleave();
      __builtin_amdgcn_sched_barrier(0);
      if (ks + 2 < KS) {
        load_frags(As, Bs, ks + 2, af0, bf0);
        mma(af1, bf1);
        interleave();
      } else {
        mma(af1, bf1);
      }
      __builtin_amdgcn_sched_barrier(0);
    }
  };

  const int nk = p.K / BK;
  if constexpr (PIPE == 0) {
    stage(0, 0);
    for (int kt = 0; kt < nk; ++kt) {
      asm volatile("s_waitcnt vmcnt(0)" ::: "memory");
      __syncthreads();
      if (kt + 1 < nk) stage((kt + 1) & 1, kt + 1);
      compute(kt & 1);
    }
  } else if constexpr (PIPE == 6) {
    auto stage_half = [&](int kt, int kind) {
      char* base = smem + (kt & 1) * STAGE_BYTES + (kind >> 1) * TILE_BYTES;
#pragma unroll
      for (int ii = 0; ii < 2; ++ii) {
        const int i = (kind & 1) * 2 + ii;
        const elem_t* src = (kind >> 1) ? b_src[i] + kt * BK : a_src[i] + a_koff(kt);
        if (kind >> 1)
          __builtin_amdgcn_global_load_lds((gptr_t)src, (lptr_t)(base + (i * GEMM_THREADS + wave * 64) * 16), 16, 0, ALG_AUX_B);
        else
          __builtin_amdgcn_global_load_lds((gptr_t)src, (lptr_t)(base + (i * GEMM_THREADS + wave * 64) * 16), 16, 0, ALG_AUX_A);
      }
    };
    bf16x8 af[2][4], b0f[4], b1f[4];
    auto load_a = [&](const char* As, int half) {
#pragma unroll
      for (int m2 = 0; m2 < 2; ++m2)
#pragma unroll
        for (int ks = 0; ks < 4; ++ks)
          af[m2][ks] = *(const bf16x8*)(As + pp_a_row(half * 2 + m2) + (((2 * ks + h2) ^ sw) * 16));
    };
    auto load_b = [&](const char* Bs, int half, bf16x8 (&bf)[4]) {
#pragma unroll
      for (int ks = 0; ks < 4; ++ks) bf[ks] = *(const bf16x8*)(Bs + pp_b_row(half) + (((2 * ks + h2) ^ sw) * 16));
    };
    auto quad = [&](int mh, int nt, const bf16x8 (&bf)[4]) {
      __builtin_amdgcn_s_setprio(1);
      if constexpr (FP8 && ALG_FP8_MX) {
        typedef int i8v __attribute__((ext_vector_type(8)));
        typedef int i4v __attribute__((ext_vector_type(4)));
        auto cat = [](const bf16x8 lo, const bf16x8 hi) -> i8v {
          const i4v l = __builtin_bit_cast(i4v, lo), h = __builtin_bit_cast(i4v, hi);
          return i8v{l[0], l[1], l[2], l[3], h[0], h[1], h[2], h[3]};
        };
#pragma unroll
        for (int kp = 0; kp < 2; ++kp) {
          const i8v bq = cat(bf[2 * kp], bf[2 * kp + 1]);
#pragma unroll
          for (int m2 = 0; m2 < 2; ++m2)
            acc[mh * 2 + m2][nt] = __builtin_amdgcn_mfma_scale_f32_32x32x64_f8f6f4(
                bq, cat(af[m2][2 * kp], af[m2][2 * kp + 1]), acc[mh * 2 + m2][nt], 0, 0, 0, 0x7f7f7f7f, 0, 0x7f7f7f7f);
        }
      } else {
#pragma unroll
        for (int ks = 0; ks < 4; ++ks)
#pragma unroll
          for (int m2 = 0; m2 < 2; ++m2)
            acc[mh * 2 + m2][nt] = fma_frag(bf[ks], af[m2][ks], acc[mh * 2 + m2][nt]);
      }
      __builtin_amdgcn_s_setprio(0);
    };
    auto enter_mfma = [&]() {
      asm volatile("s_waitcnt lgkmcnt(0)" ::: "memory");
      __builtin_amdgcn_s_barrier();
      __builtin_amdgcn_sched_barrier(0);
    };
    auto leave_mfma = [&]() {
      __builtin_amdgcn_sched_barrier(0);
      __builtin_amdgcn_s_barrier();
      __builtin_amdgcn_sched_barrier(0);
    };
    stage_half(0, 0); stage_half(0, 3); stage_half(0, 1); stage_half(0, 2);
    if (nk > 1) {
      stage_half(1, 0); stage_half(1, 3); stage_half(1, 1);
      asm volatile("s_waitcnt vmcnt(6)" ::: "memory");
    } else {
      asm volatile("s_waitcnt vmcnt(0)" ::: "memory");
    }
    __builtin_amdgcn_s_barrier();
    if (wm == 1) __builtin_amdgcn_s_barrier();
    for (int t = 0; t < nk; ++t) {
      const char* As = smem + (t & 1) * STAGE_BYTES;
      const char* Bs = As + TILE_BYTES;
      bool do_b0 = true, do_b1 = true;
      if constexpr (CONV) {
        if (p.conv_kw == 4 && p.N == 256) {
          const int dx = (t >> (p.conv_cin_log2 - 6)) & 3;
          do_b0 = dx != 3, do_b1 = dx != 0;
        }
      }
      load_a(As, 0);
      if (do_b0) load_b(Bs, 0, b0f);
      if (t + 1 < nk) stage_half(t + 1, 2);
      enter_mfma();
      if (do_b0) quad(0, 0, b0f);
      leave_mfma();
      if (do_b1) load_b(Bs, 1, b1f);
      if (t + 2 < nk) stage_half(t + 2, 0);
      enter_mfma();
      if (do_b1) quad(0, 1, b1f);
      leave_mfma();
      load_a(As, 1);
      if (t + 2 < nk) stage_half(t + 2, 3);
      enter_mfma();
      if (do_b1) quad(1, 1, b1f);
      leave_mfma();
      if (t + 2 < nk) {
        stage_half(t + 2, 1);
        asm volatile("s_waitcnt vmcnt(6)" ::: "memory");
      } else {
        asm volatile("s_waitcnt vmcnt(0)" ::: "memory");
      }
      enter_mfma();
      if (do_b0) quad(1, 0, b0f);
      leave_mfma();
    }
    if (wm == 0) __builtin_amdgcn_s_barrier();
  } else if constexpr (PIPE == 7) {
    constexpr int NDMA = 2 * LD_PER_OP;
    bf16x8 af0[4], bf0[NT], af1[4], bf1[NT];
    auto il_ds = [&]() {
#pragma unroll
      for (int i = 0; i < 4 + NT; ++i) {
        __builtin_amdgcn_sched_group_barrier(0x008, 1, 0);
        __builtin_amdgcn_sched_group_barrier(0x100, 1, 0);
      }
      __builtin_amdgcn_sched_group_barrier(0x008, 4 * NT - (4 + NT), 0);
    };
    auto il_ds_dma = [&]() {
#pragma unroll
      for (int i = 0; i < 4 + NT; ++i) {
        __builtin_amdgcn_sched_group_barrier(0x008, 1, 0);
        __builtin_amdgcn_sched_group_barrier(0x100, 1, 0);
      }
#pragma unroll
      for (int i = 0; i < NDMA / 2; ++i) {
        __builtin_amdgcn_sched_group_barrier(0x008, 1, 0);
        __builtin_amdgcn_sched_group_barrier(0x010, 1, 0);
      }
    };
    auto iter = [&](int kt, auto dma0_c, auto bar_c, auto dma3_c) {
      constexpr bool DMA0 = decltype(dma0_c)::value, BAR = decltype(bar_c)::value, DMA3 = decltype(dma3_c)::value;
      const char* As = smem + (kt & 1) * STAGE_BYTES;
      const char* Bs = As + TILE_BYTES;
      load_frags(As, Bs, 1, af1, bf1);
      mma(af0, bf0);
      if (DMA0) {
#pragma unroll
        for (int w = NDMA / 2; w < NDMA; ++w) stage_piece((kt + 1) & 1, kt + 1, w);
        il_ds_dma();
      } else {
        il_ds();
      }
      __builtin_amdgcn_sched_barrier(0);
      load_frags(As, Bs, 2, af0, bf0);
      mma(af1, bf1);
      il_ds();
      __builtin_amdgcn_sched_barrier(0);
      load_frags(As, Bs, 3, af1, bf1);
      mma(af0, bf0);
      il_ds();
      __builtin_amdgcn_sched_barrier(0);
      if (BAR) {
        asm volatile("s_waitcnt vmcnt(0) lgkmcnt(0)" ::: "memory");
        __builtin_amdgcn_s_barrier();
        __builtin_amdgcn_sched_barrier(0);
        const char* An = smem + ((kt + 1) & 1) * STAGE_BYTES;
        load_frags(An, An + TILE_BYTES, 0, af0, bf0);
        mma(af1, bf1);
        if (DMA3) {
#pragma unroll
          for (int w = 0; w < NDMA / 2; ++w) stage_piece(kt & 1, kt + 2, w);
          il_ds_dma();
        } else {
          il_ds();
        }
        __builtin_amdgcn_sched_barrier(0);
      } else {
        mma(af1, bf1);
      }
    };
    using T = IntC<1>;
    using F = IntC<0>;
    stage(0, 0);
    asm volatile("s_waitcnt vmcnt(0)" ::: "memory");
    __syncthreads();
    if (nk > 1) stage(1, 1);
    load_frags(smem, smem + TILE_BYTES, 0, af0, bf0);
    __builtin_amdgcn_sched_barrier(0);
    if (nk == 1) {
      iter(0, F{}, F{}, F{});
    } else if (nk == 2) {
      iter(0, F{}, T{}, F{});
      iter(1, F{}, F{}, F{});
    } else {
      iter(0, F{}, T{}, T{});
      for (int kt = 1; kt + 2 < nk; ++kt) iter(kt, T{}, T{}, T{});
      iter(nk - 2, T{}, T{}, F{});
      iter(nk - 1, F{}, F{}, F{});
    }
  }

  auto staged_epilogue = [&]() -> bool {
    const int64_t gs = (p.flags & ALG_GEMM_GATE_SEG_STRIDE) ? p.gate_seg_stride : p.N;
    const int c0p = (p.flags & ALG_GEMM_PERMUTE_COLS) ? p.perm_col0 : 0;
    return (p.N & 7) == 0 && (p.ldc & 7) == 0 && (p.strideC & 7) == 0 && (((uintptr_t)p.C) & 15) == 0 && (c0p & 15) == 0 &&
           !(abl & 32) && (!RES || ((p.ldr & 7) == 0 && (p.strideR & 7) == 0 && (((uintptr_t)p.R) & 15) == 0)) &&
           (!(RES && p.gate) || ((p.strideGate & 7) == 0 && (gs & 7) == 0 && (((uintptr_t)p.gate) & 15) == 0));
  };
  constexpr int NIT = 2 * MT * NT;
  uint4 rbuf[RES ? NIT : 1];
  constexpr bool BIAS_EARLY = P9 && !RES && !FP8;
  uint2 bcol_early[BIAS_EARLY ? NT : 1][4];

  if constexpr (P9) {
#ifdef ALG_GEMM_TAP
    const uint64_t tap_l0s = __builtin_readcyclecounter();
#endif
    auto uniform64 = [](const void* ptr) -> uint64_t {
      const uint64_t v = (uint64_t)(uintptr_t)ptr;
      return ((uint64_t)(uint32_t)__builtin_amdgcn_readfirstlane((int)(v >> 32)) << 32) |
             (uint32_t)__builtin_amdgcn_readfirstlane((int)(uint32_t)v);
    };
    const uint64_t pa = uniform64(A + (int64_t)m0 * p.lda);
    const uint64_t pb = uniform64(B + (int64_t)n0 * p.ldb);
    const int lda2_ = (int)p.lda * (int)sizeof(elem_t), ldb2_ = (int)p.ldb * (int)sizeof(elem_t);
    const int rmaxa_ = min(255, p.M - 1 - m0), rmaxb_ = min(255, p.N - 1 - n0);
    int zero = 0;
    asm volatile("" : "+s"(zero));
    const int ln = __builtin_amdgcn_mbcnt_hi(~0u, __builtin_amdgcn_mbcnt_lo(~0u, zero));
    const int l31q = ln & 31, h2q = ln >> 5, swq = (l31q >> 1) & 7;
    const int vrow = wave * 8 + (ln >> 3);
    const int vslot = ((ln & 7) ^ ((wave * 4 + (ln >> 4)) & 7)) * 16;
    const int l15q = ln & 15, g4q = ln >> 4, sw16 = (l15q >> 1) & 7;
    const int vl0 = M16 ? l15q * 128 + (((0 + g4q) ^ sw16) * 16) : l31q * 128 + (((0 + h2q) ^ swq) * 16);
    const int vl1 = M16 ? l15q * 128 + (((4 + g4q) ^ sw16) * 16) : l31q * 128 + (((2 + h2q) ^ swq) * 16);
    const int vl2 = l31q * 128 + (((4 + h2q) ^ swq) * 16), vl3 = l31q * 128 + (((6 + h2q) ^ swq) * 16);
    const int vb0 = ln * 16, vb1 = ln * 16 + 4096;
    const int wave1k_ = (int)(uintptr_t)(lptr_t)smem + wave * 1024;
    const int nloop_ = p.K / BK - 2, wn2_ = 2 + wn;
    int t0, t1, t2, t3, t4, t5, t6, t7, t8, t9;
    auto sreg = [](int v) -> int { return __builtin_amdgcn_readfirstlane(v); };
    const int lda2 = sreg(lda2_), ldb2 = sreg(ldb2_), rmaxa = sreg(rmaxa_), rmaxb = sreg(rmaxb_), nloop = sreg(nloop_);
    const int wm_s = sreg(wm), wn2 = sreg(wn2_), wave1k = sreg(wave1k_);
    if constexpr (RES) {
      const bf16_t* Rq = (const bf16_t*)p.R + (int64_t)b * p.strideR;
      const int ldr_ = (int)p.ldr;
      typedef int i32x4 __attribute__((ext_vector_type(4)));
      typedef unsigned int u32x4 __attribute__((ext_vector_type(4)));
      const uint64_t rbase = uniform64(Rq);
      const i32x4 rs = {(int)(uint32_t)rbase, (int)(uint32_t)(rbase >> 32) & 0xffff,
                        sreg((int)(uint32_t)((((int64_t)p.M - 1) * ldr_ + p.N) * 2)), 0x00020000};
      const int rvoff = (int)(((uint32_t)(m0 + wm * (MT * 32) + (ln >> 2)) * (uint32_t)ldr_ +
                               (uint32_t)(n0 + wn * (NT * 32) + (ln & 3) * 8)) * 2u);
      const int ldr16 = sreg(ldr_ * 32);
      u32x4 q[32];
#define ALG_Q(i) [r##i] "=&v"(q[i])
#define ALG_P9_RES_STATEMENT(TEXT, CLOBBERS) \
      asm volatile(TEXT \
                   : [t0] "=&s"(t0), [t1] "=&s"(t1), [t2] "=&s"(t2), [t3] "=&s"(t3), [t4] "=&s"(t4), [t5] "=&s"(t5), \
                     [t6] "=&s"(t6), [t7] "=&s"(t7), [t8] "=&s"(t8), [t9] "=&s"(t9), ALG_Q(0), ALG_Q(1), ALG_Q(2), ALG_Q(3), \
                     ALG_Q(4), ALG_Q(5), ALG_Q(6), ALG_Q(7), ALG_Q(8), ALG_Q(9), ALG_Q(10), ALG_Q(11), ALG_Q(12), ALG_Q(13), \
                     ALG_Q(14), ALG_Q(15), ALG_Q(16), ALG_Q(17), ALG_Q(18), ALG_Q(19), ALG_Q(20), ALG_Q(21), ALG_Q(22), \
                     ALG_Q(23), ALG_Q(24), ALG_Q(25), ALG_Q(26), ALG_Q(27), ALG_Q(28), ALG_Q(29), ALG_Q(30), ALG_Q(31) \
                   : [vl0] "v"(vl0), [vl1] "v"(vl1), [vl2] "v"(vl2), [vl3] "v"(vl3), [vrow] "v"(vrow), [vslot] "v"(vslot), \
                     [pa] "s"(pa), [pb] "s"(pb), [lda2] "s"(lda2), [ldb2] "s"(ldb2), [rmaxa] "s"(rmaxa), [rmaxb] "s"(rmaxb), \
                     [nloop] "s"(nloop), [wm] "s"(wm_s), [wn2] "s"(wn2), [wave1k] "s"(wave1k), [rs] "s"(rs), \
                     [rvoff] "v"(rvoff), [ldr16] "s"(ldr16) \
                   : "memory", "vcc", "scc", CLOBBERS)
      if constexpr (P11) {
        const uint64_t bbase = uniform64((const char*)p.B + ((int64_t)(n0 / BN) * (p.K / BK)) * 32768 + wave * 8192);
        const i32x4 db = {(int)(uint32_t)bbase, (int)(uint32_t)(bbase >> 32) & 0xffff, sreg((p.K / BK) * 32768 - wave * 8192), 0x00020000};
        asm volatile(ALG_GEMM_P11_LOOP_ASM_RES
                     : [t0] "=&s"(t0), [t1] "=&s"(t1), [t2] "=&s"(t2), [t3] "=&s"(t3), [t4] "=&s"(t4), [t5] "=&s"(t5),
                       [t6] "=&s"(t6), [t7] "=&s"(t7), [t8] "=&s"(t8), [t9] "=&s"(t9), ALG_Q(0), ALG_Q(1), ALG_Q(2), ALG_Q(3),
                       ALG_Q(4), ALG_Q(5), ALG_Q(6), ALG_Q(7), ALG_Q(8), ALG_Q(9), ALG_Q(10), ALG_Q(11), ALG_Q(12), ALG_Q(13),
                       ALG_Q(14), ALG_Q(15), ALG_Q(16), ALG_Q(17), ALG_Q(18), ALG_Q(19), ALG_Q(20), ALG_Q(21), ALG_Q(22),
                       ALG_Q(23), ALG_Q(24), ALG_Q(25), ALG_Q(26), ALG_Q(27), ALG_Q(28), ALG_Q(29), ALG_Q(30), ALG_Q(31)
                     : [vl0] "v"(vl0), [vl1] "v"(vl1), [vrow] "v"(vrow), [vslot] "v"(vslot), [vb0] "v"(vb0), [vb1] "v"(vb1),
                       [pa] "s"(pa), [db] "s"(db), [lda2] "s"(lda2), [rmaxa] "s"(rmaxa), [nloop] "s"(nloop), [wave1k] "s"(wave1k),
                       [rs] "s"(rs), [rvoff] "v"(rvoff), [ldr16] "s"(ldr16)
                     : "memory", "vcc", "scc", ALG_GEMM_P11_CLOBBERS);
      } else if constexpr (FP8) {
        ALG_P9_RES_STATEMENT(ALG_GEMM_P9_FP8_LOOP_ASM_RES, ALG_GEMM_P9_CLOBBERS);
      } else if constexpr (M16) {
        ALG_P9_RES_STATEMENT(ALG_GEMM_P10_LOOP_ASM_RES, ALG_GEMM_P10_CLOBBERS);
      } else
      asm volatile(ALG_GEMM_P9_LOOP_ASM_RES
                   : [t0] "=&s"(t0), [t1] "=&s"(t1), [t2] "=&s"(t2), [t3] "=&s"(t3), [t4] "=&s"(t4), [t5] "=&s"(t5),
                     [t6] "=&s"(t6), [t7] "=&s"(t7), [t8] "=&s"(t8), [t9] "=&s"(t9), ALG_Q(0), ALG_Q(1), ALG_Q(2), ALG_Q(3),
                     ALG_Q(4), ALG_Q(5), ALG_Q(6), ALG_Q(7), ALG_Q(8), ALG_Q(9), ALG_Q(10), ALG_Q(11), ALG_Q(12), ALG_Q(13),
                     ALG_Q(14), ALG_Q(15), ALG_Q(16), ALG_Q(17), ALG_Q(18), ALG_Q(19), ALG_Q(20), ALG_Q(21), ALG_Q(22),
                     ALG_Q(23), ALG_Q(24), ALG_Q(25), ALG_Q(26), ALG_Q(27), ALG_Q(28), ALG_Q(29), ALG_Q(30), ALG_Q(31)
                   : [vl0] "v"(vl0), [vl1] "v"(vl1), [vl2] "v"(vl2), [vl3] "v"(vl3), [vrow] "v"(vrow), [vslot] "v"(vslot),
                     [pa] "s"(pa), [pb] "s"(pb), [lda2] "s"(lda2), [ldb2] "s"(ldb2), [rmaxa] "s"(rmaxa), [rmaxb] "s"(rmaxb),
                     [nloop] "s"(nloop), [wm] "s"(wm_s), [wn2] "s"(wn2), [wave1k] "s"(wave1k), [rs] "s"(rs),
                     [rvoff] "v"(rvoff), [ldr16] "s"(ldr16)
                   : "memory", "vcc", "scc", ALG_GEMM_P9_CLOBBERS);
#undef ALG_P9_RES_STATEMENT
#undef ALG_Q
#pragma unroll
      for (int it = 0; it < 32; ++it) rbuf[it] = make_uint4(q[it][0], q[it][1], q[it][2], q[it][3]);
    } else {
      if constexpr (BIAS_EARLY) {
        const bf16_t* bias_q = (const bf16_t*)p.bias;
        const bool col_bias = bias_q && !(p.flags & ALG_GEMM_BIAS_PER_ROW) && (p.N & 7) == 0;
#pragma unroll
        for (int nt = 0; nt < NT; ++nt)
#pragma unroll
          for (int g = 0; g < (M16 ? 2 : 4); ++g) {
            const int n = n0 + wn * (NT * 32) + nt * 32 + (M16 ? 16 * g + 4 * (ln >> 4) : 8 * g + 4 * (ln >> 5));
            bcol_early[nt][g] = col_bias ? *(const uint2*)(bias_q + (n < p.N ? n : 0)) : make_uint2(0u, 0u);
          }
      }
#ifdef ALG_GEMM_P9_BUF
    typedef int i32x4 __attribute__((ext_vector_type(4)));
    auto rsrc = [](uint64_t base) -> i32x4 {
      return i32x4{(int)(uint32_t)base, (int)(uint32_t)(base >> 32) & 0xffff, -1, 0x00020000};
    };
    const i32x4 da = rsrc(pa), db = rsrc(pb);
    asm volatile(ALG_GEMM_P9_LOOP_ASM
                 : [t0] "=&s"(t0), [t1] "=&s"(t1), [t2] "=&s"(t2), [t3] "=&s"(t3), [t4] "=&s"(t4), [t5] "=&s"(t5),
                   [t6] "=&s"(t6), [t7] "=&s"(t7), [t8] "=&s"(t8), [t9] "=&s"(t9)
                 : [vl0] "v"(vl0), [vl1] "v"(vl1), [vl2] "v"(vl2), [vl3] "v"(vl3), [vrow] "v"(vrow), [vslot] "v"(vslot),
                   [da] "s"(da), [db] "s"(db), [lda2] "s"(lda2), [ldb2] "s"(ldb2), [rmaxa] "s"(rmaxa), [rmaxb] "s"(rmaxb),
                   [nloop] "s"(nloop), [wm] "s"(wm_s), [wn2] "s"(wn2), [wave1k] "s"(wave1k)
                 : "memory", "vcc", "scc", ALG_GEMM_P9_CLOBBERS);
#else
#define ALG_P9_STATEMENT(TEXT, CLOBBERS) \
    asm volatile(TEXT \
                 : [t0] "=&s"(t0), [t1] "=&s"(t1), [t2] "=&s"(t2), [t3] "=&s"(t3), [t4] "=&s"(t4), [t5] "=&s"(t5), \
                   [t6] "=&s"(t6), [t7] "=&s"(t7), [t8] "=&s"(t8), [t9] "=&s"(t9) \
                 : [vl0] "v"(vl0), [vl1] "v"(vl1), [vl2] "v"(vl2), [vl3] "v"(vl3), [vrow] "v"(vrow), [vslot] "v"(vslot), \
                   [pa] "s"(pa), [pb] "s"(pb), [lda2] "s"(lda2), [ldb2] "s"(ldb2), [rmaxa] "s"(rmaxa), [rmaxb] "s"(rmaxb), \
                   [nloop] "s"(nloop), [wm] "s"(wm_s), [wn2] "s"(wn2), [wave1k] "s"(wave1k) \
                 : "memory", "vcc", "scc", CLOBBERS)
    if constexpr (P11) {
      typedef int i32x4 __attribute__((ext_vector_type(4)));
      const uint64_t bbase = uniform64((const char*)p.B + ((int64_t)(n0 / BN) * (p.K / BK)) * 32768 + wave * 8192);
      const i32x4 db = {(int)(uint32_t)bbase, (int)(uint32_t)(bbase >> 32) & 0xffff, sreg((p.K / BK) * 32768 - wave * 8192), 0x00020000};
      asm volatile(ALG_GEMM_P11_LOOP_ASM
                   : [t0] "=&s"(t0), [t1] "=&s"(t1), [t2] "=&s"(t2), [t3] "=&s"(t3), [t4] "=&s"(t4), [t5] "=&s"(t5),
                     [t6] "=&s"(t6), [t7] "=&s"(t7), [t8] "=&s"(t8), [t9] "=&s"(t9)
                   : [vl0] "v"(vl0), [vl1] "v"(vl1), [vrow] "v"(vrow), [vslot] "v"(vslot), [vb0] "v"(vb0), [vb1] "v"(vb1),
                     [pa] "s"(pa), [db] "s"(db), [lda2] "s"(lda2), [rmaxa] "s"(rmaxa), [nloop] "s"(nloop), [wave1k] "s"(wave1k)
                   : "memory", "vcc", "scc", ALG_GEMM_P11_CLOBBERS);
    } else if constexpr (FP8) {
      ALG_P9_STATEMENT(ALG_GEMM_P9_FP8_LOOP_ASM, ALG_GEMM_P9_CLOBBERS);
    } else if constexpr (M16) {
      ALG_P9_STATEMENT(ALG_GEMM_P10_LOOP_ASM, ALG_GEMM_P10_CLOBBERS);
    } else {
      ALG_P9_STATEMENT(ALG_GEMM_P9_LOOP_ASM, ALG_GEMM_P9_CLOBBERS);
    }
#undef ALG_P9_STATEMENT
#endif
    }
#ifdef ALG_GEMM_TAP
    tap_loop += __builtin_readcyclecounter() - tap_l0s, ++tap_tiles;
#endif
    __builtin_amdgcn_s_barrier();
  }

  if constexpr (PIPE == 8) {
    constexpr int SB = 32768, OPB = 16384;
    const int nst = p.K / 32;
    const int sw8 = (l31 >> 2) & 3;
    const elem_t* a8[4];
    const elem_t* b8[4];
    {
      const int r0 = tid >> 2, q = (tid & 3) ^ ((tid >> 4) & 3);
      const int am = (abl & 8) ? 0 : m0, bn = (abl & 8) ? 0 : n0;
#pragma unroll
      for (int i = 0; i < 4; ++i) {
        a8[i] = A + (int64_t)min(am + i * 64 + r0, p.M - 1) * p.lda + q * 8;
        b8[i] = B + (int64_t)min(bn + i * 64 + r0, p.N - 1) * p.ldb + q * 8;
      }
    }
    auto src_off = [&](int st) -> int64_t { return (int64_t)st * 32; };
    auto stage8 = [&](int st) {
      char* base = smem + (st & 3) * SB;
#pragma unroll
      for (int i = 0; i < 4; ++i) {
        __builtin_amdgcn_global_load_lds((gptr_t)(a8[i] + src_off(st)), (lptr_t)(base + (i * 256 + wave * 64) * 16), 16, 0, ALG_AUX_A);
        __builtin_amdgcn_global_load_lds((gptr_t)(b8[i] + src_off(st)), (lptr_t)(base + OPB + (i * 256 + wave * 64) * 16), 16, 0, ALG_AUX_B);
      }
    };
    const int a_off8 = (wm * 128 + l31) * 64, b_off8 = (wn * 128 + l31) * 64;
    auto load8 = [&](int st, bf16x8 (&af)[2][4], bf16x8 (&bfr)[2][4]) {
      const char* As = smem + (st & 3) * SB;
      const char* Bs = As + OPB;
#pragma unroll
      for (int ksl = 0; ksl < 2; ++ksl) {
        const int so = ((2 * ksl + h2) ^ sw8) * 16;
#pragma unroll
        for (int nt = 0; nt < 4; ++nt) bfr[ksl][nt] = *(const bf16x8*)(Bs + b_off8 + nt * 32 * 64 + so);
#pragma unroll
        for (int mt = 0; mt < 4; ++mt) af[ksl][mt] = *(const bf16x8*)(As + a_off8 + mt * 32 * 64 + so);
      }
    };
    auto mma8 = [&](const bf16x8 (&af)[2][4], const bf16x8 (&bfr)[2][4]) {
#pragma unroll
      for (int ksl = 0; ksl < 2; ++ksl)
#pragma unroll
        for (int mt = 0; mt < 4; ++mt)
#pragma unroll
          for (int nt = 0; nt < 4; ++nt) acc[mt][nt] = fma_frag(bfr[ksl][nt], af[ksl][mt], acc[mt][nt]);
    };
    bf16x8 fa0[2][4], fb0[2][4], fa1[2][4], fb1[2][4];
    auto step = [&](int j, bf16x8 (&ca)[2][4], bf16x8 (&cb)[2][4], bf16x8 (&na)[2][4], bf16x8 (&nb)[2][4]) {
      asm volatile("s_waitcnt vmcnt(16) lgkmcnt(0)" ::: "memory");
      __builtin_amdgcn_s_barrier();
      __builtin_amdgcn_sched_barrier(0);
#ifndef ALG_P8_NO_READS
      load8(j + 1, na, nb);
#endif
#ifndef ALG_P8_NO_DMA
      {
        const int st = min(j + 4, nst - 1);
        char* base = smem + (j & 3) * SB;
#pragma unroll
        for (int i = 0; i < 4; ++i) {
          __builtin_amdgcn_global_load_lds((gptr_t)(a8[i] + src_off(st)), (lptr_t)(base + (i * 256 + wave * 64) * 16), 16, 0, ALG_AUX_A);
          __builtin_amdgcn_global_load_lds((gptr_t)(b8[i] + src_off(st)), (lptr_t)(base + OPB + (i * 256 + wave * 64) * 16), 16, 0, ALG_AUX_B);
        }
      }
#endif
      mma8(ca, cb);
#pragma unroll
      for (int i = 0; i < 16; ++i) {
        __builtin_amdgcn_sched_group_barrier(0x008, 1, 0);
        __builtin_amdgcn_sched_group_barrier(0x100, 1, 0);
      }
#pragma unroll
      for (int i = 0; i < 8; ++i) {
        __builtin_amdgcn_sched_group_barrier(0x008, 1, 0);
        __builtin_amdgcn_sched_group_barrier(0x010, 1, 0);
      }
      __builtin_amdgcn_sched_group_barrier(0x008, 8, 0);
      __builtin_amdgcn_sched_barrier(0);
    };
    stage8(0);
    stage8(1);
    stage8(min(2, nst - 1));
    stage8(min(3, nst - 1));
    asm volatile("s_waitcnt vmcnt(24)" ::: "memory");
    __builtin_amdgcn_s_barrier();
    load8(0, fa0, fb0);
    __builtin_amdgcn_sched_barrier(0);
    for (int j = 0; j < nst; j += 2) {
      step(j, fa0, fb0, fa1, fb1);
      step(j + 1, fa1, fb1, fa0, fb0);
    }
    asm volatile("s_waitcnt vmcnt(0) lgkmcnt(0)" ::: "memory");
    __builtin_amdgcn_s_barrier();
  }

  const bf16_t* bias = (const bf16_t*)p.bias;
  const bf16_t* R = RES ? (const bf16_t*)p.R + (int64_t)b * p.strideR : nullptr;
  const bf16_t* gate = (RES && p.gate) ? (const bf16_t*)p.gate + (int64_t)b * p.strideGate : nullptr;
  const bool bias_row = p.flags & ALG_GEMM_BIAS_PER_ROW;
  const bool perm = p.flags & ALG_GEMM_PERMUTE_COLS;
  const int64_t gate_seg = (p.flags & ALG_GEMM_GATE_SEG_STRIDE) ? p.gate_seg_stride : p.N;
  const bool gate_f32 = RES && p.gate && (p.flags & ALG_GEMM_GATE_F32);
  bf16_t* Cb = (bf16_t*)p.C + (int64_t)b * p.strideC;
  const int ldc = (int)p.ldc, ldr = (int)p.ldr;
  const int col0 = perm ? p.perm_col0 : 0;
  const bool n_vec = (p.N & 3) == 0 && (col0 & 15) == 0;
  auto blk_row = [&](int mt) { return PP ? (mt >> 1) * 128 + wm * 64 + (mt & 1) * 32 : wm * (MT * 32) + mt * 32; };
  auto blk_col = [&](int nt) { return PP ? nt * 128 + wn * 32 : wn * (NT * 32) + nt * 32; };
  auto quad_row = [](int q, int ln_) { return M16 ? 16 * (q >> 1) + (ln_ & 15) : (ln_ & 31); };
  auto quad_col = [](int q, int ln_) { return M16 ? 16 * (q & 1) + 4 * (ln_ >> 4) : 8 * q + 4 * (ln_ >> 5); };
  auto rq = [](int q) { return M16 ? q >> 1 : 0; };
  auto cq = [](int q) { return M16 ? q & 1 : q; };
  constexpr int NRQ = M16 ? 2 : 1, NCQ = M16 ? 2 : 4;
  if constexpr (PP || PIPE == 8 || P9) {
    const bool staged = staged_epilogue() && ((!RES && ACT == ALG_ACT_NONE) || !(bias && bias_row));
    int lane_e = lane, l31_e = l31, h2_e = h2;
    if constexpr (P9) {
      int z = 0;
      asm volatile("" : "+s"(z));
      lane_e = __builtin_amdgcn_mbcnt_hi(~0u, __builtin_amdgcn_mbcnt_lo(~0u, z));
      l31_e = lane_e & 31, h2_e = lane_e >> 5;
    }
    if (staged) {
      char* const my = smem + wave * (MT * NT * 2048);
      constexpr bool NT_OUTER = FP8 && PIPE == 9 && RES;
      uint2 bcol[NT_OUTER ? 1 : NT][4];
      float4 scol[FP8 && !NT_OUTER ? NT : 1][FP8 && !NT_OUTER ? 4 : 1];
      float brow4[MT][NRQ], a_sc4[MT];
      if constexpr (!NT_OUTER)
#pragma unroll
      for (int nt = 0; nt < NT; ++nt)
#pragma unroll
        for (int g = 0; g < NCQ; ++g) {
          const int n = n0 + blk_col(nt) + (M16 ? quad_col(g, lane_e) : 8 * g + 4 * h2_e);
          const int nc = n < p.N ? n : 0;
          if constexpr (BIAS_EARLY) bcol[nt][g] = bcol_early[nt][g];
          else bcol[nt][g] = (bias && !bias_row) ? *(const uint2*)(bias + nc) : make_uint2(0u, 0u);
          if constexpr (FP8) scol[nt][g] = *(const float4*)(p.b_scale + (int64_t)b * p.strideBScale + nc);
        }
#pragma unroll
      for (int mt = 0; mt < MT; ++mt) {
#pragma unroll
        for (int r = 0; r < NRQ; ++r) {
          const int row = m0 + blk_row(mt) + quad_row(2 * r, lane_e);
          const int rowc = row < p.M ? row : p.M - 1;
          brow4[mt][r] = (bias && bias_row) ? bf2f(bias[rowc]) : 0.0f;
          if (r == 0) a_sc4[mt] = FP8 ? p.a_scale[(int64_t)b * p.strideAScale + rowc] : 1.0f;
        }
      }
      constexpr bool GATE_EARLY = false;
      const bool seg_lo = m0 + BM <= p.seg_split, seg_hi = m0 >= p.seg_split;
      const int gkind = !RES ? -1 : !gate ? 0 : !gate_f32 ? 1 : (seg_lo || seg_hi) ? 2 : 3;
      uint4 g0p[RES ? NT : 1], g1p[RES ? NT : 1];
      float4 gfa[RES ? NT : 1], gfb[RES ? NT : 1];
      auto load_gates = [&]() {
        if (gkind != 1 && gkind != 2) return;
#pragma unroll
        for (int nt = 0; nt < NT; ++nt) {
          const int c0 = n0 + blk_col(nt) + (lane_e & 3) * 8;
          const int cc = c0 < p.N ? c0 : 0;
          if (gkind == 1) {
            g0p[nt] = *(const uint4*)(gate + cc);
            g1p[nt] = *(const uint4*)(gate + gate_seg + cc);
          } else {
            const float* gp = (const float*)p.gate + (int64_t)b * p.strideGate + (seg_hi ? gate_seg : 0) + cc;
            gfa[nt] = *(const float4*)gp;
            gfb[nt] = *(const float4*)(gp + 4);
          }
        }
      };
      if constexpr (RES && GATE_EARLY) load_gates();
      constexpr bool BIAS_F32 = P9 && !RES && !FP8;
      float bvf[BIAS_F32 ? NT : 1][4][4];
      if constexpr (BIAS_F32) {
#pragma unroll
        for (int nt = 0; nt < NT; ++nt)
#pragma unroll
          for (int g = 0; g < NCQ; ++g) unpack4(bcol[nt][g], bvf[nt][g]);
      }
      __builtin_amdgcn_sched_barrier(0);
      auto park_band = [&](auto mt_c, auto br_c) {
        constexpr int mt = decltype(mt_c)::value;
        constexpr bool BR = decltype(br_c)::value != 0;
        const float a_sc = a_sc4[mt];
        static_for<NT>([&](auto nt_c) {
          constexpr int nt = decltype(nt_c)::value;
          const f32x16 blk = get_acc(mt_c, nt_c);
#pragma unroll
          for (int g = 0; g < 4; ++g) {
            const float brow = brow4[mt][rq(g)];
            float bv[4], sv[4] = {1.f, 1.f, 1.f, 1.f};
            if constexpr (BIAS_F32) {
#pragma unroll
              for (int i = 0; i < 4; ++i) bv[i] = bvf[nt][cq(g)][i];
            } else {
              unpack4(bcol[nt][cq(g)], bv);
            }
            if constexpr (FP8) {
              const float4 s4 = scol[nt][g];
              sv[0] = s4.x * a_sc; sv[1] = s4.y * a_sc; sv[2] = s4.z * a_sc; sv[3] = s4.w * a_sc;
            }
            float v[4];
#pragma unroll
            for (int i = 0; i < 4; ++i) {
              const float dot = FP8 ? blk[4 * g + i] * sv[i] : blk[4 * g + i];
              v[i] = BR ? dot + bv[i] + brow : dot + bv[i];
            }
            if constexpr (ACT != ALG_ACT_NONE) {
#pragma unroll
              for (int i = 0; i < 4; i += 2) {
                const uint32_t pk = pack_bf2(v[i], v[i + 1]);
                v[i] = act_apply(__uint_as_float(pk << 16), ACT);
                v[i + 1] = act_apply(__uint_as_float(pk & 0xffff0000u), ACT);
              }
            }
            uint2 o;
            o.x = pack_bf2(v[0], v[1]);
            o.y = pack_bf2(v[2], v[3]);
            if constexpr (M16) {
              const int pr_ = quad_row(g, lane_e), pc_ = quad_col(g, lane_e);
              *(uint2*)(my + (mt * NT + nt) * 2048 + pr_ * 64 + (((pc_ >> 3) ^ ((pr_ >> 2) & 3)) * 16) + (pc_ & 7) * 2) = o;
            } else {
              *(uint2*)(my + (mt * NT + nt) * 2048 + l31_e * 64 + ((g ^ ((l31_e >> 2) & 3)) * 16) + h2_e * 8) = o;
            }
          }
          if constexpr (FP8 && PIPE == 9) __builtin_amdgcn_sched_barrier(0);
        });
      };
      if constexpr (NT_OUTER) {
        uint2 bc[2][4];
        float4 sc4[2][4];
        auto load_cols = [&](auto nt_c) {
          constexpr int nt = decltype(nt_c)::value;
#pragma unroll
          for (int g = 0; g < 4; ++g) {
            const int n = n0 + blk_col(nt) + 8 * g + 4 * h2_e;
            const int nc = n < p.N ? n : 0;
            bc[nt & 1][g] = (bias && !bias_row) ? *(const uint2*)(bias + nc) : make_uint2(0u, 0u);
            sc4[nt & 1][g] = *(const float4*)(p.b_scale + (int64_t)b * p.strideBScale + nc);
          }
        };
        load_cols(IntC<0>{});
        static_for<NT>([&](auto nt_c) {
          constexpr int nt = decltype(nt_c)::value;
          if constexpr (nt + 1 < NT) load_cols(IntC<nt + 1>{});
          static_for<4>([&](auto mt_c) {
            constexpr int mt = decltype(mt_c)::value;
            const float a_sc = a_sc4[mt];
            const f32x16 blk = get_acc(mt_c, nt_c);
#pragma unroll
            for (int g = 0; g < 4; ++g) {
              float bv[4];
              unpack4(bc[nt & 1][g], bv);
              const float4 s4 = sc4[nt & 1][g];
              const float sv[4] = {s4.x * a_sc, s4.y * a_sc, s4.z * a_sc, s4.w * a_sc};
              float v[4];
#pragma unroll
              for (int i = 0; i < 4; ++i) v[i] = blk[4 * g + i] * sv[i] + bv[i];
              uint2 o;
              o.x = pack_bf2(v[0], v[1]);
              o.y = pack_bf2(v[2], v[3]);
              *(uint2*)(my + (mt * NT + nt) * 2048 + l31_e * 64 + ((g ^ ((l31_e >> 2) & 3)) * 16) + h2_e * 8) = o;
            }
            __builtin_amdgcn_sched_barrier(0);
          });
        });
      } else {
      constexpr bool BR_SPLIT = !RES && ACT == ALG_ACT_NONE;
      constexpr bool BR_ALWAYS = BR_SPLIT && FP8 && PIPE == 9;
      if (BR_ALWAYS) {
        static_for<MT>([&](auto mt_c) { park_band(mt_c, IntC<1>{}); });
      } else if (BR_SPLIT && bias && bias_row) {
        static_for<MT>([&](auto mt_c) { park_band(mt_c, IntC<1>{}); });
      } else {
        static_for<MT>([&](auto mt_c) { park_band(mt_c, IntC<0>{}); });
      }
      }
      asm volatile("s_waitcnt lgkmcnt(0)" ::: "memory");
      if (RES && !P9) {
#pragma unroll
        for (int it = 0; it < NIT; ++it) {
          const int blk = it >> 1, mt = blk / NT, nt = blk % NT;
          const int rr = (it & 1) * 16 + (lane_e >> 2), ch = lane_e & 3;
          const int row = m0 + blk_row(mt) + rr;
          const int c0 = n0 + blk_col(nt) + ch * 8;
          rbuf[it] = (row < p.M && c0 < p.N) ? *(const uint4*)(R + row * ldr + c0) : make_uint4(0, 0, 0, 0);
        }
        __builtin_amdgcn_sched_barrier(0);
      }
      if constexpr (RES) {
        auto res_loop = [&](auto kind_c) {
          constexpr int KIND = decltype(kind_c)::value;
          if constexpr (!GATE_EARLY) load_gates();
          if constexpr (KIND == 1) {
#pragma unroll
            for (int nt = 0; nt < NT; ++nt)
              asm volatile("" : "+v"(g0p[nt].x), "+v"(g0p[nt].y), "+v"(g0p[nt].z), "+v"(g0p[nt].w), "+v"(g1p[nt].x),
                           "+v"(g1p[nt].y), "+v"(g1p[nt].z), "+v"(g1p[nt].w));
          }
          if constexpr (KIND == 2) {
#pragma unroll
            for (int nt = 0; nt < NT; ++nt)
              asm volatile("" : "+v"(gfa[nt].x), "+v"(gfa[nt].y), "+v"(gfa[nt].z), "+v"(gfa[nt].w), "+v"(gfb[nt].x),
                           "+v"(gfb[nt].y), "+v"(gfb[nt].z), "+v"(gfb[nt].w));
          }
          const int lrow = lane_e >> 2, ch = lane_e & 3;
          const uint32_t voff = (uint32_t)(lrow * ldc + ch * 8) * 2;
          const char* ldsl = my + lrow * 64 + ((ch ^ ((lrow >> 2) & 3)) * 16);
          auto lds_raw = [&](auto it_c) -> uint4 {
            constexpr int it = decltype(it_c)::value;
            return *(const uint4*)(ldsl + (it >> 1) * 2048 + (it & 1) * 1024);
          };
          uint4 raw_next = lds_raw(IntC<0>{});
          static_for<NIT>([&](auto it_c) {
            constexpr int it = decltype(it_c)::value;
            constexpr int blk = it >> 1, mt = blk / NT, nt = blk % NT;
            const uint4 raw = raw_next;
            if constexpr (it + 1 < NIT) raw_next = lds_raw(IntC<it + 1>{});
            const int r0 = m0 + blk_row(mt) + (it & 1) * 16, cb = n0 + blk_col(nt);
            char* const cp = (char*)(Cb + (int64_t)r0 * ldc + cb);
            const bool ok = lrow < p.M - r0 && ch * 8 < p.N - cb;
            const uint4 rraw = rbuf[it];
            const uint32_t u[4] = {raw.x, raw.y, raw.z, raw.w};
            const uint32_t ru[4] = {rraw.x, rraw.y, rraw.z, rraw.w};
            uint32_t gu[4] = {0, 0, 0, 0};
            float gq[8] = {1.f, 1.f, 1.f, 1.f, 1.f, 1.f, 1.f, 1.f};
            if constexpr (KIND == 1) {
              const bool seg1 = lrow >= p.seg_split - r0;
              gu[0] = seg1 ? g1p[nt].x : g0p[nt].x; gu[1] = seg1 ? g1p[nt].y : g0p[nt].y;
              gu[2] = seg1 ? g1p[nt].z : g0p[nt].z; gu[3] = seg1 ? g1p[nt].w : g0p[nt].w;
            }
            if constexpr (KIND == 2) {
              gq[0] = gfa[nt].x; gq[1] = gfa[nt].y; gq[2] = gfa[nt].z; gq[3] = gfa[nt].w;
              gq[4] = gfb[nt].x; gq[5] = gfb[nt].y; gq[6] = gfb[nt].z; gq[7] = gfb[nt].w;
            }
            float y[8];
#pragma unroll
            for (int k = 0; k < 4; ++k) {
              const float x0 = __uint_as_float(u[k] << 16), x1 = __uint_as_float(u[k] & 0xffff0000u);
              const float r0f = __uint_as_float(ru[k] << 16), r1f = __uint_as_float(ru[k] & 0xffff0000u);
              if constexpr (KIND == 0) {
                y[2 * k] = r0f + x0;
                y[2 * k + 1] = r1f + x1;
              } else if constexpr (KIND == 1) {
                const uint32_t pk = pack_bf2(__uint_as_float(gu[k] << 16) * x0, __uint_as_float(gu[k] & 0xffff0000u) * x1);
                y[2 * k] = r0f + __uint_as_float(pk << 16);
                y[2 * k + 1] = r1f + __uint_as_float(pk & 0xffff0000u);
              } else {
                float m0_ = gq[2 * k] * x0, m1_ = gq[2 * k + 1] * x1;
                asm volatile("" : "+v"(m0_), "+v"(m1_));
                y[2 * k] = r0f + m0_;
                y[2 * k + 1] = r1f + m1_;
              }
            }
            if (ok) {
              uint4 outv;
              outv.x = pack_bf2(y[0], y[1]); outv.y = pack_bf2(y[2], y[3]);
              outv.z = pack_bf2(y[4], y[5]); outv.w = pack_bf2(y[6], y[7]);
              ALG_STORE16(cp + voff, outv);
            }
            __builtin_amdgcn_sched_barrier(0);
          });
        };
        if (gkind == 0) { res_loop(IntC<0>{}); return; }
        if (gkind == 1) { res_loop(IntC<1>{}); return; }
        if (gkind == 2) { res_loop(IntC<2>{}); return; }
      } else {
        const int lrow = lane_e >> 2, ch = lane_e & 3;
        const uint32_t voff = (uint32_t)(lrow * ldc + ch * 8) * 2;
        const char* ldsl = my + lrow * 64 + ((ch ^ ((lrow >> 2) & 3)) * 16);
        auto plain_loop = [&](auto perm_c) {
          constexpr bool PERM = decltype(perm_c)::value != 0;
          static_for<NIT / 8>([&](auto grp_c) {
            constexpr int g0 = decltype(grp_c)::value * 8;
            uint4 raw[8];
            static_for<8>([&](auto j_c) {
              constexpr int it = g0 + decltype(j_c)::value;
              raw[decltype(j_c)::value] = *(const uint4*)(ldsl + (it >> 1) * 2048 + (it & 1) * 1024);
            });
            static_for<8>([&](auto j_c) {
              constexpr int it = g0 + decltype(j_c)::value;
              constexpr int blk = it >> 1, mt = blk / NT, nt = blk % NT;
              const int r0 = m0 + blk_row(mt) + (it & 1) * 16, cb = n0 + blk_col(nt);
              const uint4 outv = raw[decltype(j_c)::value];
              if (lrow < p.M - r0 && ch * 8 < p.N - cb) {
                if constexpr (PERM) {
                  const int c0 = cb + ch * 8;
                  bf16_t* crow = Cb + (int64_t)(r0 + lrow) * ldc;
                  const int base = col0 + (c0 & ~12), b3 = (c0 >> 3) & 1;
                  *(uint2*)(crow + base + (b3 << 2)) = make_uint2(outv.x, outv.y);
                  *(uint2*)(crow + base + 8 + (b3 << 2)) = make_uint2(outv.z, outv.w);
                } else {
                  ALG_STORE16((char*)(Cb + (int64_t)r0 * ldc + cb) + voff, outv);
                }
              }
            });
            __builtin_amdgcn_sched_barrier(0);
          });
        };
        if constexpr (PAIR == 2) {
          if (!second) {
            const QkNormRope& e = pr.qe;
            const bool is_k = n0 >= e.heads * 64;
            const float qs = is_k ? 1.0f : e.q_scale;
            float wA[8], bA[8], wB[8], bB[8];
            unpack8(*(const uint4*)((is_k ? e.wk : e.wq) + ch * 8), wA);
            unpack8(*(const uint4*)((is_k ? e.wk : e.wq) + 32 + ch * 8), wB);
            unpack8(*(const uint4*)((is_k ? e.bk : e.bq) + ch * 8), bA);
            unpack8(*(const uint4*)((is_k ? e.bk : e.bq) + 32 + ch * 8), bB);
            const bool any_rope = e.cos_tab && e.text_len < p.M;
            float tab[2][32] = {};
            bool rp[2];
            auto fetch = [&](auto u_c) {
              constexpr int u = decltype(u_c)::value, slot = u & 1;
              const int srow = m0 + blk_row(u >> 1) + (u & 1) * 16 + lrow;
              rp[slot] = any_rope && srow >= e.text_len && srow < p.M;
              if (any_rope) {
                const int64_t pos = rp[slot] ? (int64_t)(srow - e.text_len) * 64 + ch * 8 : (int64_t)ch * 8;
                const float4 c0 = *(const float4*)(e.cos_tab + pos), c1 = *(const float4*)(e.cos_tab + pos + 4);
                const float4 c2 = *(const float4*)(e.cos_tab + pos + 32), c3 = *(const float4*)(e.cos_tab + pos + 36);
                const float4 s0 = *(const float4*)(e.sin_tab + pos), s1 = *(const float4*)(e.sin_tab + pos + 4);
                const float4 s2 = *(const float4*)(e.sin_tab + pos + 32), s3 = *(const float4*)(e.sin_tab + pos + 36);
                const float4 q[8] = {c0, c1, c2, c3, s0, s1, s2, s3};
#pragma unroll
                for (int k = 0; k < 8; ++k)
                  tab[slot][4 * k] = q[k].x, tab[slot][4 * k + 1] = q[k].y, tab[slot][4 * k + 2] = q[k].z, tab[slot][4 * k + 3] = q[k].w;
              }
            };
            fetch(IntC<0>{});
            static_for<8>([&](auto u_c) {
              constexpr int u = decltype(u_c)::value, mt = u >> 1, half = u & 1, slot = u & 1;
              uint4 raw[4];
              static_for<4>([&](auto nt_c) {
                constexpr int nt = decltype(nt_c)::value;
                raw[nt] = *(const uint4*)(ldsl + (mt * NT + nt) * 2048 + half * 1024);
              });
              const bool roped = rp[slot];
              float csA[8], csB[8], snA[8], snB[8];
#pragma unroll
              for (int k = 0; k < 8; ++k)
                csA[k] = tab[slot][k], csB[k] = tab[slot][8 + k], snA[k] = tab[slot][16 + k], snB[k] = tab[slot][24 + k];
              if constexpr (u + 1 < 8) fetch(IntC<u + 1>{});
              static_for<2>([&](auto hh_c) {
                constexpr int hh = decltype(hh_c)::value;
                uint4& ra = raw[2 * hh];
                uint4& rb = raw[2 * hh + 1];
                float va[8], vb[8];
                unpack8(ra, va);
                unpack8(rb, vb);
                float sa = qk_chunk_sum(va), sb = qk_chunk_sum(vb);
                sa += __shfl_xor(sa, 1, 64); sb += __shfl_xor(sb, 1, 64);
                sa += __shfl_xor(sa, 2, 64); sb += __shfl_xor(sb, 2, 64);
                const float mean = qk_mean(sa + sb);
                float qa = qk_chunk_sqdev(va, mean), qb = qk_chunk_sqdev(vb, mean);
                qa += __shfl_xor(qa, 1, 64); qb += __shfl_xor(qb, 1, 64);
                qa += __shfl_xor(qa, 2, 64); qb += __shfl_xor(qb, 2, 64);
                const float rstd = qk_rstd(qa + qb, e.eps);
                float oa[8], ob[8];
                qk_ln_chunk(va, mean, rstd, wA, bA, roped, qs, oa);
                qk_ln_chunk(vb, mean, rstd, wB, bB, roped, qs, ob);
                float ta[8], tb[8];
#pragma unroll
                for (int k = 0; k < 8; ++k) ta[k] = oa[k], tb[k] = ob[k];
                qk_rope_chunk(ta, csA, snA, qs);
                qk_rope_chunk(tb, csB, snB, qs);
#pragma unroll
                for (int k = 0; k < 8; ++k) oa[k] = roped ? ta[k] : oa[k], ob[k] = roped ? tb[k] : ob[k];
                ra = pack8(oa);
                rb = pack8(ob);
              });
              const int r0 = m0 + blk_row(mt) + half * 16;
              static_for<4>([&](auto nt_c) {
                constexpr int nt = decltype(nt_c)::value;
                const int cb = n0 + blk_col(nt);
                if (lrow < p.M - r0 && ch * 8 < p.N - cb) *(uint4*)((char*)(Cb + (int64_t)r0 * ldc + cb) + voff) = raw[nt];
              });
              __builtin_amdgcn_sched_barrier(0);
            });
            return;
          }
        }
        if (perm) plain_loop(IntC<1>{}); else plain_loop(IntC<0>{});
        return;
      }
#pragma unroll
      for (int it = 0; it < NIT; ++it) {
        const int blk = it >> 1, mt = blk / NT, nt = blk % NT;
        const int rr = (it & 1) * 16 + (lane_e >> 2), ch = lane_e & 3;
        const uint4 raw = *(const uint4*)(my + blk * 2048 + rr * 64 + ((ch ^ ((rr >> 2) & 3)) * 16));
        const int row = m0 + blk_row(mt) + rr;
        const int c0 = n0 + blk_col(nt) + ch * 8;
        if (row < p.M && c0 < p.N) {
          uint4 outv = raw;
          if (RES) {
            float x[8], r[8], gq[8];
            const uint32_t u[4] = {raw.x, raw.y, raw.z, raw.w};
            const uint4 rraw = rbuf[it];
            const uint32_t ru[4] = {rraw.x, rraw.y, rraw.z, rraw.w};
#pragma unroll
            for (int k = 0; k < 4; ++k) {
              x[2 * k] = __uint_as_float(u[k] << 16);
              x[2 * k + 1] = __uint_as_float(u[k] & 0xffff0000u);
              r[2 * k] = __uint_as_float(ru[k] << 16);
              r[2 * k + 1] = __uint_as_float(ru[k] & 0xffff0000u);
              gq[2 * k] = gq[2 * k + 1] = 1.0f;
            }
            const bool seg1 = row >= p.seg_split;
            if (gate) {
              if (gate_f32) {
                const float* gp = (const float*)p.gate + (int64_t)b * p.strideGate + (seg1 ? gate_seg : 0) + c0;
                const float4 g0 = *(const float4*)gp, g1 = *(const float4*)(gp + 4);
                gq[0] = g0.x; gq[1] = g0.y; gq[2] = g0.z; gq[3] = g0.w; gq[4] = g1.x; gq[5] = g1.y; gq[6] = g1.z; gq[7] = g1.w;
              } else {
                const uint4 graw = *(const uint4*)(gate + (seg1 ? gate_seg : 0) + c0);
                const uint32_t gu[4] = {graw.x, graw.y, graw.z, graw.w};
#pragma unroll
                for (int k = 0; k < 4; ++k) {
                  gq[2 * k] = __uint_as_float(gu[k] << 16);
                  gq[2 * k + 1] = __uint_as_float(gu[k] & 0xffff0000u);
                }
              }
            }
            float y[8];
#pragma unroll
            for (int k = 0; k < 8; ++k) y[k] = gate_f32 ? r[k] + gq[k] * x[k] : r[k] + rbf(gq[k] * x[k]);
            outv.x = pack_bf2(y[0], y[1]); outv.y = pack_bf2(y[2], y[3]);
            outv.z = pack_bf2(y[4], y[5]); outv.w = pack_bf2(y[6], y[7]);
          }
          bf16_t* crow = Cb + row * ldc;
          if (perm) {
            const int base = col0 + (c0 & ~12), b3 = (c0 >> 3) & 1;
            *(uint2*)(crow + base + (b3 << 2)) = make_uint2(outv.x, outv.y);
            *(uint2*)(crow + base + 8 + (b3 << 2)) = make_uint2(outv.z, outv.w);
          } else {
            *(uint4*)(crow + c0) = outv;
          }
        }
      }
      return;
    }
  }

  auto epilogue_band = [&](auto mt_c) {
    constexpr int mt = decltype(mt_c)::value;
    int row_[NRQ], rowc_[NRQ];
    float brow_[NRQ];
#pragma unroll
    for (int r = 0; r < NRQ; ++r) {
      row_[r] = (PP ? m0 + (mt >> 1) * 128 + wm * 64 + (mt & 1) * 32 : m0 + wm * (MT * 32) + mt * 32) + quad_row(2 * r, lane);
      rowc_[r] = row_[r] < p.M ? row_[r] : p.M - 1;
      brow_[r] = (bias && bias_row) ? bf2f(bias[rowc_[r]]) : 0.0f;
    }
    const float a_sc = FP8 ? p.a_scale[(int64_t)b * p.strideAScale + rowc_[0]] : 1.0f;
    static_for<NT>([&](auto nt_c) {
      constexpr int nt = decltype(nt_c)::value;
      const f32x16 blk = get_acc(mt_c, nt_c);
#pragma unroll
      for (int g = 0; g < 4; ++g) {
        const int row = row_[rq(g)], rowc = rowc_[rq(g)];
        const bool row_ok = row < p.M;
        const float brow = brow_[rq(g)];
        const bool seg1 = row >= p.seg_split;
        const int n = (PP ? n0 + nt * 128 + wn * 32 : n0 + wn * (NT * 32) + nt * 32) + quad_col(g, lane);
        if (n_vec) {
          if (n < p.N) {
            float bv[4] = {0.f, 0.f, 0.f, 0.f}, gv[4] = {1.f, 1.f, 1.f, 1.f}, rv[4] = {0.f, 0.f, 0.f, 0.f};
            if (bias && !bias_row) unpack4(*(const uint2*)(bias + n), bv);
            if (RES && gate) {
              if (gate_f32) {
                const float4 g4 = *(const float4*)((const float*)p.gate + (int64_t)b * p.strideGate + (seg1 ? gate_seg : 0) + n);
                gv[0] = g4.x; gv[1] = g4.y; gv[2] = g4.z; gv[3] = g4.w;
              } else {
                unpack4(*(const uint2*)(gate + (seg1 ? gate_seg : 0) + n), gv);
              }
            }
            if (RES) unpack4(*(const uint2*)(R + rowc * ldr + n), rv);
            float sv[4] = {1.f, 1.f, 1.f, 1.f};
            if (FP8) {
              const float4 s4 = *(const float4*)(p.b_scale + (int64_t)b * p.strideBScale + n);
              sv[0] = s4.x * a_sc; sv[1] = s4.y * a_sc; sv[2] = s4.z * a_sc; sv[3] = s4.w * a_sc;
            }
            float v[4];
#pragma unroll
            for (int i = 0; i < 4; ++i) {
              const float dot = FP8 ? blk[4 * g + i] * sv[i] : blk[4 * g + i];
              float x = rbf(dot + bv[i] + brow);
              if (ACT != ALG_ACT_NONE) x = rbf(act_apply(x, ACT));
              if (RES) x = gate_f32 ? rv[i] + gv[i] * x : rv[i] + rbf(gv[i] * x);
              v[i] = x;
            }
            if (row_ok) {
              const int nc = perm ? col0 + ((n & ~12) | ((n & 4) << 1) | ((n & 8) >> 1)) : n;
              uint2 o;
              o.x = pack_bf2(v[0], v[1]);
              o.y = pack_bf2(v[2], v[3]);
              *(uint2*)(Cb + row * ldc + nc) = o;
            }
          }
        } else {
#pragma unroll
          for (int i = 0; i < 4; ++i) {
            const int nn = n + i;
            if (nn < p.N && row_ok) {
              const float dot = FP8 ? blk[4 * g + i] * (a_sc * p.b_scale[(int64_t)b * p.strideBScale + nn]) : blk[4 * g + i];
              float x = rbf(dot + ((bias && !bias_row) ? bf2f(bias[nn]) : 0.0f) + brow);
              if (ACT != ALG_ACT_NONE) x = rbf(act_apply(x, ACT));
              if (RES) {
                if (gate_f32) {
                  x = bf2f(R[rowc * ldr + nn]) +
                      ((const float*)p.gate)[(int64_t)b * p.strideGate + (seg1 ? gate_seg : 0) + nn] * x;
                } else {
                  const float gg = gate ? bf2f(gate[(seg1 ? gate_seg : 0) + nn]) : 1.0f;
                  x = bf2f(R[rowc * ldr + nn]) + rbf(gg * x);
                }
              }
              const int nj = nn + col0;
              const int nc = perm ? ((nj & ~12) | ((nj & 4) << 1) | ((nj & 8) >> 1)) : nn;
              Cb[row * ldc + nc] = f2bf(x);
            }
          }
        }
      }
    });
  };
#ifndef ALG_EPI_STAGED_ONLY
  static_for<MT>([&](auto mt_c) { epilogue_band(mt_c); });
#endif
  };

  int total_wg = total1;
  if constexpr (PAIR) total_wg += pr.m_tiles * pr.n_tiles * pr.p.batch;
  for (int L = blockIdx.x; L < total_wg; L += gridDim.x) {
    const int xcd = L & 7, q = total_wg >> 3, r = total_wg & 7;
    const int wg = (xcd < r ? xcd * (q + 1) : r * (q + 1) + (xcd - r) * q) + (L >> 3);
    if (L != (int)blockIdx.x) __syncthreads();
    do_tile(wg);
  }
#ifdef ALG_GEMM_TAP
  if (threadIdx.x == 0 && blockIdx.x < 1024) {
    uint64_t* t = gemm_tap_buf + blockIdx.x * 4;
    t[0] = __builtin_readcyclecounter() - tap_c0, t[1] = wall_clock64() - tap_r0, t[2] = tap_loop, t[3] = tap_tiles;
  }
#endif
}

inline unsigned gemm_grid(int64_t nwg) {
  static std::atomic<int> cus{0};
  int n = cus.load();
  if (n == 0) {
    hipDeviceProp_t prop;
    int dev = 0;
    n = (hipGetDevice(&dev) == hipSuccess && hipGetDeviceProperties(&prop, dev) == hipSuccess) ? prop.multiProcessorCount : 256;
    n &= ~7;
    if (n < 8) n = 8;
    cus.store(n);
  }
  return (unsigned)(nwg < n ? nwg : n);
}

inline int gemm_group_m(int pipe, int n_tiles = 0, int K = 0) {
  const int dflt = (pipe != 9 && pipe != 10 && pipe != 11) ? GROUP_M : n_tiles >= 32 ? 4 : (K >= 8192 && n_tiles <= 16) ? 2 : 3;
#ifdef ALG_GROUP_M_OVERRIDE
  return ALG_GROUP_M_OVERRIDE;
#endif
  return dflt;
}

}

using namespace alg;

template <int PIPE, int WNW = 4, bool FP8 = false>
int launch_gemm(const alg_gemm_args* a, int m_tiles, int n_tiles, int64_t nwg, hipStream_t s) {
  constexpr int LDS = (PIPE == 9 || PIPE == 10 || PIPE == 11) ? GEMM_LDS_P9 : GEMM_LDS;
  static PerDeviceOnce attr_set;
  const int dev_slot = current_device_slot();
  if (!device_done(attr_set, dev_slot)) {
    const void* fns[4] = {(const void*)gemm_bf16_kernel<ALG_ACT_NONE, true, PIPE, WNW, FP8>,
                          (const void*)gemm_bf16_kernel<ALG_ACT_GELU_TANH, false, PIPE, WNW, FP8>,
                          (const void*)gemm_bf16_kernel<ALG_ACT_SILU, false, PIPE, WNW, FP8>,
                          (const void*)gemm_bf16_kernel<ALG_ACT_NONE, false, PIPE, WNW, FP8>};
    for (const void* fn : fns) {
      hipError_t e = hipFuncSetAttribute(fn, hipFuncAttributeMaxDynamicSharedMemorySize, LDS);
      if (e != hipSuccess) {
        set_error("alg_gemm_bf16: hipFuncSetAttribute(%d B LDS): %s", LDS, hipGetErrorString(e));
        return ALG_ELAUNCH;
      }
    }
    device_mark(attr_set, dev_slot);
  }
  const dim3 grid(gemm_grid(nwg)), block((PIPE == 11 ? 1 : 2) * WNW * 64);
  const int gm = gemm_group_m(PIPE, n_tiles, a->K);
  if (a->R) {
    hipLaunchKernelGGL((gemm_bf16_kernel<ALG_ACT_NONE, true, PIPE, WNW, FP8>), grid, block, LDS, s, *a, m_tiles,
                       n_tiles, gm, GemmNoPair{});
  } else if (a->act == ALG_ACT_GELU_TANH) {
    hipLaunchKernelGGL((gemm_bf16_kernel<ALG_ACT_GELU_TANH, false, PIPE, WNW, FP8>), grid, block, LDS, s, *a, m_tiles,
                       n_tiles, gm, GemmNoPair{});
  } else if (a->act == ALG_ACT_SILU) {
    hipLaunchKernelGGL((gemm_bf16_kernel<ALG_ACT_SILU, false, PIPE, WNW, FP8>), grid, block, LDS, s, *a, m_tiles,
                       n_tiles, gm, GemmNoPair{});
  } else {
    hipLaunchKernelGGL((gemm_bf16_kernel<ALG_ACT_NONE, false, PIPE, WNW, FP8>), grid, block, LDS, s, *a, m_tiles,
                       n_tiles, gm, GemmNoPair{});
  }
  return check_launch("alg_gemm_bf16");
}
```

alg_amd/csrc/gemm_p11.hip:

```cpp
#include "gemm_kernel.h"

namespace alg {
int launch_gemm_p11(const alg_gemm_args* a, int m_tiles, int n_tiles, int64_t nwg, hipStream_t s) {
  return launch_gemm<11, 4>(a, m_tiles, n_tiles, nwg, s);
}

__global__ __launch_bounds__(256) void pack_b_p11_kernel(const bf16_t* __restrict__ w, uint4* __restrict__ out, int N, int K, int64_t ldb,
                                                          int64_t total) {
  const int64_t i = (int64_t)blockIdx.x * 256 + threadIdx.x;
  if (i >= total) return;
  const int lane = (int)(i & 63);
  const int f = (int)((i >> 6) & 7), wv = (int)((i >> 9) & 3);
  const int64_t tile = i >> 11;
  const int nkt = K / 64;
  const int kt = (int)(tile % nkt);
  const int64_t nt = tile / nkt;
  const int n = (int)(nt * 256) + wv * 64 + (f & 3) * 16 + (lane & 15);
  const int k = kt * 64 + (f >> 2) * 32 + (lane >> 4) * 8;
  uint4 v = make_uint4(0u, 0u, 0u, 0u);
  if (n < N) v = *(const uint4*)(w + (int64_t)n * ldb + k);
  out[i] = v;
}
}

using namespace alg;

extern "C" int64_t alg_pack_b_p11_bytes(int N, int K) {
  if (N <= 0 || K <= 0 || K % 64) return 0;
  return (int64_t)((N + 255) / 256) * (K / 64) * 32768;
}

extern "C" int alg_pack_b_p11(const void* w, void* packed, int N, int K, int64_t ldb, void* stream) {
  if (!w || !packed || N <= 0 || K < 128 || K % 64 || ldb < K || ldb % 8 || ((uintptr_t)w & 15) || ((uintptr_t)packed & 15)) {
    set_error("alg_pack_b_p11: bad argument (N=%d K=%d ldb=%lld; K a multiple of 64 and >= 128, 16-byte aligned rows)", N, K, (long long)ldb);
    return ALG_EINVAL;
  }
  const int64_t total = alg_pack_b_p11_bytes(N, K) / 16;
  hipLaunchKernelGGL(pack_b_p11_kernel, dim3((unsigned)((total + 255) / 256)), dim3(256), 0, (hipStream_t)stream, (const bf16_t*)w,
                     (uint4*)packed, N, K, ldb, total);
  return check_launch("alg_pack_b_p11");
}

#ifdef ALG_GEMM_TAP
extern "C" int alg_dbg_gemm_tap(uint64_t* host) { return alg::gemm_tap_read(host); }
#endif
```

alg_amd/transformer_cogvideox.py:

```python
from __future__ import annotations

import math
import os
from dataclasses import dataclass, asdict
from typing import Optional

import torch

from . import _lib


@dataclass
class CogVideoXTransformerConfig:

    num_attention_heads: int = 48
    attention_head_dim: int = 64
    in_channels: int = 32
    out_channels: int = 16
    num_layers: int = 42
    time_embed_dim: int = 512
    text_embed_dim: int = 4096
    max_text_seq_length: int = 226
    sample_width: int = 90
    sample_height: int = 60
    sample_frames: int = 49
    patch_size: int = 2
    patch_size_t: Optional[int] = None
    temporal_compression_ratio: int = 4
    ff_inner_mult: int = 4
    norm_eps: float = 1e-5
    qk_norm_eps: float = 1e-6
    flip_sin_to_cos: bool = True
    freq_shift: int = 0
    use_rotary_positional_embeddings: bool = True
    use_learned_positional_embeddings: bool = True
    ofs_embed_dim: Optional[int] = None
    spatial_interpolation_scale: float = 1.875
    temporal_interpolation_scale: float = 1.0

    @property
    def inner_dim(self):
        return self.num_attention_heads * self.attention_head_dim

    def to_dict(self):
        return asdict(self)


def _bf(t, device):
    return t.to(device=device, dtype=torch.bfloat16).contiguous()


class CogVideoXTransformer3DModel:
    dtype = torch.bfloat16

    def __init__(self, config: CogVideoXTransformerConfig, weights: dict, device="cuda"):
        cfg = self.config = config
        self.device = torch.device(device)
        if self.device.type != "cuda":
            raise _lib.AlgHipError("CogVideoXTransformer3DModel runs on the GPU only (HIP kernels, no CPU fallback)")
        if cfg.attention_head_dim != 64:
            raise _lib.AlgHipError("the attention kernel is specialised for head_dim 64")
        if cfg.ofs_embed_dim is not None and cfg.ofs_embed_dim != cfg.time_embed_dim:
            raise _lib.AlgHipError("ofs_embed_dim must equal time_embed_dim (emb = emb + ofs_emb)")
        D = cfg.inner_dim
        if D % 512:
            raise _lib.AlgHipError("inner_dim must be a multiple of 512 (LayerNorm kernel tiling)")
        _lib.load_library()
        self.attn_prescale = True
        self.pair_qkv = True
        self.fuse_qk_norm = False
        self.packed_weights = True
        self._sincos = {}
        dev = self.device
        w = weights
        p = cfg.patch_size
        self.p_t = cfg.patch_size_t or 1
        self.k_patch = cfg.in_channels * p * p * self.p_t
        if self.k_patch % 64 or cfg.text_embed_dim % 64 or cfg.time_embed_dim % 64:
            raise _lib.AlgHipError("GEMM K dimensions must be multiples of 64")
        self.w_patch = _bf(w["patch_embed.proj.weight"].reshape(D, self.k_patch), dev)
        self.b_patch = _bf(w["patch_embed.proj.bias"], dev)
        self.w_text = _bf(w["patch_embed.text_proj.weight"], dev)
        self.b_text = _bf(w["patch_embed.text_proj.bias"], dev)
        self.pos_emb = _bf(w["patch_embed.pos_embedding"][0], dev) if cfg.use_learned_positional_embeddings else None
        self.w_t1 = _bf(w["time_embedding.linear_1.weight"], dev)
        self.b_t1 = _bf(w["time_embedding.linear_1.bias"], dev)
        self.w_t2 = _bf(w["time_embedding.linear_2.weight"], dev)
        self.b_t2 = _bf(w["time_embedding.linear_2.bias"], dev)
        if cfg.ofs_embed_dim is not None:
            self.w_o1, self.b_o1 = _bf(w["ofs_embedding.linear_1.weight"], dev), _bf(w["ofs_embedding.linear_1.bias"], dev)
            self.w_o2, self.b_o2 = _bf(w["ofs_embedding.linear_2.weight"], dev), _bf(w["ofs_embedding.linear_2.bias"], dev)

        def reorder6(t):
            c = t.chunk(6, dim=0)
            return torch.cat([c[3], c[0], c[4], c[1], c[5], c[2]], dim=0)

        mw, mb = [], []
        self.layers = []
        for i in range(cfg.num_layers):
            b = "transformer_blocks.%d." % i
            L = {}
            for nm in ("norm1", "norm2"):
                mw.append(reorder6(w[b + nm + ".linear.weight"]))
                mb.append(reorder6(w[b + nm + ".linear.bias"]))
                L[nm + "_w"] = _bf(w[b + nm + ".norm.weight"], dev)
                L[nm + "_b"] = _bf(w[b + nm + ".norm.bias"], dev)
            L["wqk"] = _bf(torch.cat([w[b + "attn1.to_q.weight"], w[b + "attn1.to_k.weight"]], dim=0), dev)
            L["bqk"] = _bf(torch.cat([w[b + "attn1.to_q.bias"], w[b + "attn1.to_k.bias"]], dim=0), dev)
            L["wv"] = _bf(w[b + "attn1.to_v.weight"], dev)
            L["bv"] = _bf(w[b + "attn1.to_v.bias"], dev)
            for nm in ("norm_q", "norm_k"):
                L[nm + "_w"] = _bf(w[b + "attn1." + nm + ".weight"], dev)
                L[nm + "_b"] = _bf(w[b + "attn1." + nm + ".bias"], dev)
            L["wo"] = _bf(w[b + "attn1.to_out.0.weight"], dev)
            L["bo"] = _bf(w[b + "attn1.to_out.0.bias"], dev)
            L["wf1"] = _bf(w[b + "ff.net.0.proj.weight"], dev)
            L["bf1"] = _bf(w[b + "ff.net.0.proj.bias"], dev)
            L["wf2"] = _bf(w[b + "ff.net.2.weight"], dev)
            L["bf2"] = _bf(w[b + "ff.net.2.bias"], dev)
            for nm in ("wo", "wf1", "wf2"):
                L["p" + nm] = _lib.PackedB(L[nm])
            self.layers.append(L)
        ow, ob = w["norm_out.linear.weight"], w["norm_out.linear.bias"]
        sh_w, sc_w = ow.chunk(2, dim=0)
        sh_b, sc_b = ob.chunk(2, dim=0)
        mw.append(torch.cat([sh_w, sh_w, sc_w, sc_w], dim=0))
        mb.append(torch.cat([sh_b, sh_b, sc_b, sc_b], dim=0))
        self.w_mod = _bf(torch.cat(mw, dim=0), dev)
        self.b_mod = _bf(torch.cat(mb, dim=0), dev)
        self.mod_cols = self.w_mod.shape[0]
        self.norm_final_w = _bf(w["norm_final.weight"], dev)
        self.norm_final_b = _bf(w["norm_final.bias"], dev)
        self.norm_out_w = _bf(w["norm_out.norm.weight"], dev)
        self.norm_out_b = _bf(w["norm_out.norm.bias"], dev)
        self.w_out = _bf(w["proj_out.weight"], dev)
        self.b_out = _bf(w["proj_out.bias"], dev)
        self._ws = {}
        self._rope_cache = {}
        self.profile = None

    def _positional(self, Hh, Ww, Fr, S):
        cfg = self.config
        learned = cfg.use_learned_positional_embeddings
        if not learned and cfg.use_rotary_positional_embeddings:
            return None
        pre_frames = (Fr - 1) * cfg.temporal_compression_ratio + 1
        if learned and pre_frames == cfg.sample_frames and self.pos_emb is not None and self.pos_emb.shape[0] == S:
            return self.pos_emb
        p = cfg.patch_size
        gh, gw, gt = Hh // p, Ww // p, Fr // self.p_t
        key = (gh, gw, gt)
        hit = self._sincos.get(key)
        if hit is None:
            D = cfg.inner_dim
            ds, dt = 3 * D // 4, D // 4

            def sc1(dim, pos):
                omega = 1.0 / 10000 ** (torch.arange(dim // 2, dtype=torch.float64) / (dim / 2.0))
                out = torch.outer(pos.reshape(-1).double(), omega)
                return torch.cat([out.sin(), out.cos()], dim=1)

            hh = torch.arange(gh, dtype=torch.float32) / cfg.spatial_interpolation_scale
            ww = torch.arange(gw, dtype=torch.float32) / cfg.spatial_interpolation_scale
            tt = torch.arange(gt, dtype=torch.float32) / cfg.temporal_interpolation_scale
            grid = torch.stack(torch.meshgrid(ww, hh, indexing="xy"), dim=0).reshape(2, 1, gh, gw)
            sp = torch.cat([sc1(ds // 2, grid[0]), sc1(ds // 2, grid[1])], dim=1)
            tp = sc1(dt, tt)
            pe = torch.cat([tp[:, None].expand(-1, gh * gw, -1), sp[None].expand(gt, -1, -1)], dim=-1).reshape(gt * gh * gw, D)
            joint = torch.zeros(cfg.max_text_seq_length + pe.shape[0], D, dtype=torch.float32)
            joint[cfg.max_text_seq_length:] = pe.float()
            hit = joint.to(device=self.device, dtype=torch.bfloat16).contiguous()
            self._sincos[key] = hit
        if hit.shape[0] != S:
            raise ValueError("positional embedding covers %d tokens, the sequence has %d" % (hit.shape[0], S))
        return hit

    def _timed(self, name, fn, *args, **kwargs):
        if self.profile is None:
            return fn(*args, **kwargs)
        e0, e1 = torch.cuda.Event(enable_timing=True), torch.cuda.Event(enable_timing=True)
        e0.record()
        out = fn(*args, **kwargs)
        e1.record()
        self.profile.setdefault(name, []).append((e0, e1))
        return out

    @classmethod
    def from_synthetic(cls, config=None, seed=1234, std=0.02, device="cuda", randomize_affine=False):
        from .weights import synthetic_state_dict

        config = config or CogVideoXTransformerConfig()
        return cls(config, synthetic_state_dict(config, seed=seed, std=std, device=device,
                                                 randomize_affine=randomize_affine), device=device)

    @classmethod
    def from_pretrained(cls, path, subfolder="transformer", torch_dtype=torch.bfloat16, device="cuda", **_):
        from .weights import load_diffusers_transformer

        config, sd = load_diffusers_transformer(path, subfolder)
        return cls(config, sd, device=device)

    def to(self, *args, **kwargs):
        return self

    def _workspace(self, N, S, P):
        key = (N, S, P)
        ws = self._ws.get(key)
        if ws is not None:
            return ws
        cfg, dev = self.config, self.device
        D = cfg.inner_dim
        bf = dict(device=dev, dtype=torch.bfloat16)
        S_pad = (S + 127) // 128 * 128
        ws = dict(
            S_pad=S_pad,
            x=torch.empty(N, S, D, **bf),
            y=torch.empty(N, S, D, **bf),
            qk=torch.empty(N, S, 2 * D, **bf),
            vt=torch.zeros(N, D, S_pad, **bf),
            att=torch.empty(N, S, D, **bf),
            h=torch.empty(N, S, cfg.ff_inner_mult * D, **bf),
            patches=torch.empty(N, P, self.k_patch, **bf),
            tsin=torch.empty(N, D, **bf),
            t1=torch.empty(N, cfg.time_embed_dim, **bf),
            semb=torch.empty(N, cfg.time_embed_dim, **bf),
            mod=torch.empty(N, self.mod_cols, **bf),
            po=torch.empty(N * P, self.w_out.shape[0], **bf),
        )
        if len(self._ws) >= 4:
            self._ws.pop(next(iter(self._ws)))
        self._ws[key] = ws
        return ws

    def _rope(self, image_rotary_emb):
        if image_rotary_emb is None:
            return None, None
        cos, sin = image_rotary_emb
        key = (cos.data_ptr(), sin.data_ptr(), tuple(cos.shape))
        hit = self._rope_cache.get(key)
        if hit is None:
            hit = (cos.to(device=self.device, dtype=torch.float32).contiguous(),
                   sin.to(device=self.device, dtype=torch.float32).contiguous())
            self._rope_cache = {key: hit}
        return hit

    def forward_assembled(self, latents, conds, encoder_hidden_states, timestep, image_rotary_emb=None, ofs=None):
        cfg = self.config
        N = len(conds)
        lat = latents.to(device=self.device, dtype=torch.bfloat16).contiguous()
        Bl, Fr, C, Hh, Ww = lat.shape
        if Bl not in (1, N):
            raise ValueError("latents batch must be 1 or len(conds)")
        if 2 * C != cfg.in_channels:
            raise ValueError("latents have %d channels, transformer expects in_channels=%d" % (C, cfg.in_channels))
        conds = [c.to(device=self.device, dtype=torch.bfloat16).contiguous() for c in conds]
        for c in conds:
            if c.numel() != Fr * C * Hh * Ww:
                raise ValueError("conditioning latents must have shape [1, F, C, H, W] matching the latents")
        ehs = encoder_hidden_states.to(device=self.device, dtype=torch.bfloat16).contiguous()
        if ehs.shape[0] != N:
            raise ValueError("encoder_hidden_states batch %d != %d samples" % (ehs.shape[0], N))
        T = ehs.shape[1]
        p, p_t = cfg.patch_size, self.p_t
        if Fr % p_t:
            raise ValueError("latent frames (%d) must be a multiple of patch_size_t=%d (cog:963-968 pads them)" % (Fr, p_t))
        P = (Fr // p_t) * (Hh // p) * (Ww // p)
        S = T + P
        D, Hn = cfg.inner_dim, cfg.num_attention_heads
        if cfg.use_learned_positional_embeddings:
            if cfg.sample_width != Ww or cfg.sample_height != Hh:
                raise ValueError(
                    "It is currently not possible to generate videos at a different resolution that the defaults. "
                    "This should only be the case with 'THUDM/CogVideoX-5b-I2V'.")
        pos_emb = self._positional(Hh, Ww, Fr, S)
        ws = self._workspace(N, S, P)
        x, y, qk, vt, att, h, mod = ws["x"], ws["y"], ws["qk"], ws["vt"], ws["att"], ws["h"], ws["mod"]
        S_pad = ws["S_pad"]
        cos, sin = self._rope(image_rotary_emb)
        G = _lib.gemm
        TM = self._timed

        ts = timestep.to(device=self.device, dtype=torch.float32).contiguous()
        if ts.numel() != N:
            ts = ts.reshape(-1)[:1].expand(N).contiguous()
        _lib.timestep_embedding(ts, ws["tsin"], N, D, cfg.flip_sin_to_cos)
        E = cfg.time_embed_dim
        G(ws["tsin"], self.w_t1, ws["t1"], N, E, D, D, D, E, bias=self.b_t1, act=_lib.ACT_SILU)
        if cfg.ofs_embed_dim is None:
            G(ws["t1"], self.w_t2, ws["semb"], N, E, E, E, E, E, bias=self.b_t2, act=_lib.ACT_SILU)
        else:
            if ofs is None:
                raise ValueError("this transformer has an ofs embedding: pass `ofs` (cog:998)")
            O = cfg.ofs_embed_dim
            emb, osin, o1, oemb = (torch.empty(N, E, device=self.device, dtype=torch.bfloat16) for _ in range(4))
            G(ws["t1"], self.w_t2, emb, N, E, E, E, E, E, bias=self.b_t2)
            ofs_v = ofs.to(device=self.device, dtype=torch.float32).reshape(-1)
            ofs_v = (ofs_v if ofs_v.numel() == N else ofs_v[:1].expand(N)).contiguous()
            _lib.timestep_embedding(ofs_v, osin, N, O, cfg.flip_sin_to_cos)
            G(osin, self.w_o1, o1, N, O, O, O, O, O, bias=self.b_o1, act=_lib.ACT_SILU)
            G(o1, self.w_o2, oemb, N, O, O, O, O, O, bias=self.b_o2)
            _lib.lincomb([(1.0, emb), (1.0, oemb)], torch.bfloat16, out=emb)
            _lib.silu(emb, ws["semb"])
        G(ws["semb"], self.w_mod, mod, N, self.mod_cols, E, E, E, self.mod_cols, bias=self.b_mod)

        G(ehs, self.w_text, x, T, D, cfg.text_embed_dim, cfg.text_embed_dim, cfg.text_embed_dim, D,
          bias=self.b_text, R=pos_emb, ldr=D, batch=N, strideA=T * cfg.text_embed_dim, strideC=S * D)
        _lib.patchify(lat, 0 if Bl == 1 else Fr * C * Hh * Ww, conds, ws["patches"], N, Fr, C, Hh, Ww, p, p_t)
        G(ws["patches"], self.w_patch, x, P, D, self.k_patch, self.k_patch, self.k_patch, D, bias=self.b_patch,
          R=pos_emb, ldr=D, r_off=T * D, batch=N, strideA=P * self.k_patch, strideC=S * D, c_off=T * D)

        scale = 1.0 / math.sqrt(cfg.attention_head_dim)
        prescale = self.attn_prescale
        q_scale = scale * 1.4426950408889634 if prescale else 1.0
        F4 = cfg.ff_inner_mult * D
        packed = self.packed_weights and os.environ.get("ALG_GEMM_PIPE", "10") == "10"
        wo_k, wf1_k, wf2_k = ("pwo", "pwf1", "pwf2") if packed else ("wo", "wf1", "wf2")
        for li, L in enumerate(self.layers):
            m1 = li * 12 * D
            m2 = m1 + 6 * D
            TM("ln_mod", _lib.layernorm_modulate, x, y, L["norm1_w"], L["norm1_b"], mod, mod, self.mod_cols, N, S, D,
               T, cfg.norm_eps, scale_off=m1 + 2 * D, shift_off=m1)
            qk_call = ((y, L["wqk"], qk, S, 2 * D, D, D, D, 2 * D), dict(bias=L["bqk"], batch=N, strideA=S * D, strideC=S * 2 * D))
            vt_call = ((L["wv"], y, vt, D, S, D, D, D, S_pad), dict(bias=L["bv"], batch=N, strideB=S * D, strideC=D * S_pad,
                                                                   flags=_lib.GEMM_BIAS_PER_ROW | _lib.GEMM_PERMUTE_COLS))
            if self.pair_qkv and self.fuse_qk_norm:
                TM("gemm_qkv", _lib.gemm_pair_qk, qk_call, vt_call, L["norm_q_w"], L["norm_q_b"], L["norm_k_w"], L["norm_k_b"], cos, sin,
                               Hn, T, cfg.qk_norm_eps, q_scale=q_scale)
            else:
                if self.pair_qkv:
                    TM("gemm_qkv", _lib.gemm_pair, qk_call, vt_call)
                else:
                    TM("gemm_qk", G, *qk_call[0], **qk_call[1])
                    TM("gemm_vt", G, *vt_call[0], **vt_call[1])
                TM("qk_norm_rope", _lib.qk_norm_rope_, qk, L["norm_q_w"], L["norm_q_b"], L["norm_k_w"], L["norm_k_b"], cos, sin, N, S, Hn, T,
                                   cfg.qk_norm_eps, q_scale=q_scale)
            TM("attn", _lib.flash_attn_d64, qk, qk, vt, att, N, Hn, S, S * 2 * D, 2 * D, D * S_pad, S_pad, S * D, D, scale,
                                k_off=D, q_prescaled=prescale)
            TM("gemm_out", G, att, L[wo_k], x, S, D, D, D, D, D, bias=L["bo"], R=x, ldr=D, gate=mod, gate_off=m1 + 4 * D,
              strideGate=self.mod_cols, seg_split=T, batch=N, strideA=S * D, strideC=S * D, strideR=S * D)
            TM("ln_mod", _lib.layernorm_modulate, x, y, L["norm2_w"], L["norm2_b"], mod, mod, self.mod_cols, N, S, D,
               T, cfg.norm_eps, scale_off=m2 + 2 * D, shift_off=m2)
            TM("gemm_ff1", G, y, L[wf1_k], h, S, F4, D, D, D, F4, bias=L["bf1"], act=_lib.ACT_GELU_TANH, batch=N, strideA=S * D,
              strideC=S * F4)
            TM("gemm_ff2", G, h, L[wf2_k], x, S, D, F4, F4, F4, D, bias=L["bf2"], R=x, ldr=D, gate=mod, gate_off=m2 + 4 * D,
              strideGate=self.mod_cols, seg_split=T, batch=N, strideA=S * F4, strideC=S * D, strideR=S * D)

        _lib.layernorm_modulate(x, y, self.norm_final_w, self.norm_final_b, None, None, 0, N, S, D, T, cfg.norm_eps)
        mo = cfg.num_layers * 12 * D
        _lib.layernorm_modulate(y, att, self.norm_out_w, self.norm_out_b, mod, mod, self.mod_cols, N, P, D, 0,
                                cfg.norm_eps, x_bstride=S * D, y_bstride=P * D, x_off=T * D, scale_off=mo + 2 * D,
                                shift_off=mo)
        n_out = self.w_out.shape[0]
        G(att, self.w_out, ws["po"], N * P, n_out, D, D, D, n_out, bias=self.b_out)
        out = torch.empty(N, Fr, cfg.out_channels, Hh, Ww, device=self.device, dtype=torch.bfloat16)
        _lib.unpatchify(ws["po"], out, N, Fr, cfg.out_channels, Hh, Ww, p, p_t)
        return out

    def __call__(self, hidden_states, encoder_hidden_states, timestep, timestep_cond=None, ofs=None,
                 image_rotary_emb=None, attention_kwargs=None, return_dict=True):
        if timestep_cond is not None:
            raise NotImplementedError("timestep_cond is not used by the CogVideoX I2V checkpoints")
        C = hidden_states.shape[2] // 2
        lat = hidden_states[:, :, :C].contiguous()
        conds = [hidden_states[n:n + 1, :, C:].contiguous() for n in range(hidden_states.shape[0])]
        out = self.forward_assembled(lat, conds, encoder_hidden_states, timestep, image_rotary_emb, ofs=ofs)
        if not return_dict:
            return (out,)
        return TransformerOutput(sample=out)


@dataclass
class TransformerOutput:
    sample: torch.Tensor
```

include/alg_hip.h:

```cpp
#ifndef ALG_HIP_H
#define ALG_HIP_H

#include <stdint.h>

#ifdef __cplusplus
extern "C" {
#endif

#define ALG_F32 0
#define ALG_BF16 1

#define ALG_OK 0
#define ALG_EINVAL (-1)
#define ALG_ELAUNCH (-2)
#define ALG_ELIMIT (-3)

#define ALG_VERSION 110

int alg_version(void);
const char* alg_last_error(void);

void alg_reload_env(void);


int alg_down_up(const void* in, void* out, int64_t planes, int H, int W, int h1, int w1, int dtype,
                int round_intermediate, const void* tables, void* workspace, int64_t workspace_bytes, void* stream);

int64_t alg_lowpass_tables_bytes(int H, int W, int h1, int w1);
int alg_lowpass_tables_build(void* tables, int64_t bytes, int H, int W, int h1, int w1, void* stream);

int64_t alg_down_up_workspace_bytes(int64_t planes, int H, int W, int h1, int w1);

int alg_gaussian_blur(const void* in, void* out, int64_t planes, int H, int W, int ksize, float sigma, int dtype,
                      void* workspace, int64_t workspace_bytes, void* stream);
int64_t alg_gaussian_blur_workspace_bytes(int64_t planes, int H, int W, int ksize);

int alg_cfg_ddim_step(const void* pred, int pred_dtype, void* latents, int lat_dtype, int n_pass, int64_t numel,
                      float guidance_scale, float sqrt_alpha_t, float sqrt_beta_t, float coef_a, float coef_b,
                      void* stream);

int alg_cfg_combine(const void* pred, void* out, int dtype, int n_pass, int64_t numel, float guidance_scale,
                    void* stream);

int alg_lincomb(const void* const* xs, const float* coefs, const int* dtypes, int n_terms, void* out, int out_dtype,
                int64_t numel, void* stream);

int alg_concat_cast(const void* const* src0, int dtype0, const void* const* src1, int dtype1, int n, int64_t O,
                    int64_t A0, int64_t A1, int64_t R, int64_t s0_ostride, int64_t s1_ostride, int64_t a1_off,
                    void* out, int out_dtype, void* stream);

int alg_unipc_update(const float* x, const float* m0, const float* m1, const float* m_new, float* out,
                     int64_t numel, float r, float c, float k, float rk, float rho0, float rho_new, void* stream);


#define ALG_ACT_NONE 0
#define ALG_ACT_GELU_TANH 1
#define ALG_ACT_SILU 2

#define ALG_GEMM_BIAS_PER_ROW 1
#define ALG_GEMM_PERMUTE_COLS 4
#define ALG_GEMM_GATE_SEG_STRIDE 16
#define ALG_GEMM_B_PACKED11 32
#define ALG_GEMM_GATE_F32 8

typedef struct alg_gemm_args {
  const void* A;
  const void* B;
  void* C;
  const void* bias;
  const void* R;
  const void* gate;
  int64_t lda, ldb, ldc, ldr;
  int64_t strideA, strideB, strideC, strideR, strideGate;
  int32_t M, N, K, batch;
  int32_t seg_split;
  int32_t act;
  int32_t flags;
  int64_t gate_seg_stride;
  int32_t perm_col0;
  int32_t conv_cin_log2;
  const float* a_scale;
  const float* b_scale;
  int64_t strideAScale, strideBScale;
  int32_t conv_wp;
  int32_t conv_hpwp;
  int32_t conv_kw;
  int32_t reserved1;
} alg_gemm_args;

int alg_gemm_bf16(const alg_gemm_args* args, void* stream);

int64_t alg_pack_b_p11_bytes(int N, int K);
int alg_pack_b_p11(const void* w, void* packed, int N, int K, int64_t ldb, void* stream);

int alg_gemm_bf16_pair(const alg_gemm_args* a, const alg_gemm_args* b, void* stream);

typedef struct alg_qk_norm_rope_args {
  const void *wq, *bq, *wk, *bk;
  const float *cos_tab, *sin_tab;
  int32_t heads, text_len;
  float eps, q_scale;
} alg_qk_norm_rope_args;
int alg_gemm_bf16_pair_qk(const alg_gemm_args* qk, const alg_gemm_args* vt, const alg_qk_norm_rope_args* e, void* stream);

int alg_gemm_fp8(const alg_gemm_args* args, void* stream);

int alg_quantize_fp8_rows(const void* x, int64_t x_rstride, void* q, float* scale, int64_t rows, int K, void* stream);

int alg_flash_attn_d64(const void* q, const void* k, const void* vt, void* o, int batch, int heads, int S,
                       int64_t q_bstride, int64_t q_rstride, int64_t vt_bstride, int64_t vt_rstride,
                       int64_t o_bstride, int64_t o_rstride, float scale, void* stream);

#define ALG_ATTN_Q_PRESCALED 1
int alg_flash_attn_d64_ex(const void* q, const void* k, const void* vt, void* o, int batch, int heads, int S,
                          int64_t q_bstride, int64_t q_rstride, int64_t vt_bstride, int64_t vt_rstride,
                          int64_t o_bstride, int64_t o_rstride, float scale, int flags, void* workspace,
                          int64_t workspace_bytes, void* stream);
int64_t alg_flash_attn_d64_workspace_bytes(int batch, int heads, int S, int flags);

int alg_flash_attn_d128(const void* q, const void* k, const void* vt, void* o, int batch, int heads, int Sq, int Skv,
                        int64_t q_bstride, int64_t q_rstride, int64_t k_bstride, int64_t k_rstride, int64_t vt_bstride,
                        int64_t vt_rstride, int64_t o_bstride, int64_t o_rstride, float scale, void* stream);

int alg_flash_attn_d128_ex(const void* q, const void* k, const void* vt, void* o, int batch, int heads, int Sq, int Skv,
                           int64_t q_bstride, int64_t q_rstride, int64_t k_bstride, int64_t k_rstride, int64_t vt_bstride,
                           int64_t vt_rstride, int64_t o_bstride, int64_t o_rstride, float scale, int kv_group, int causal,
                           void* stream);

int alg_flash_attn_d128_dual(const void* q, const void* k, const void* vt, int Skv, int64_t k_bstride, int64_t k_rstride,
                             int64_t vt_bstride, int64_t vt_rstride, const void* k2, const void* vt2, int Skv2, int64_t k2_bstride,
                             int64_t k2_rstride, int64_t vt2_bstride, int64_t vt2_rstride, void* o, int batch, int heads, int Sq,
                             int64_t q_bstride, int64_t q_rstride, int64_t o_bstride, int64_t o_rstride, float scale, void* stream);

int alg_rope_half(void* x, const float* cos_tab, const float* sin_tab, const int* pos, int64_t rows, int heads,
                  int64_t x_rstride, void* stream);


int alg_embed_rows(const int64_t* ids, const void* table, void* out, int64_t n, int D, int vocab, void* stream);

int alg_t5_layernorm(const void* x, const void* weight, void* y, int64_t rows, int D, float eps, void* stream);

int alg_attn_bias(const void* q, const void* k, const void* v, void* out, const void* bias_table, const int* rel_bucket,
                  const int* key_mask, int batch, int heads, int head_dim, int L, int64_t qkv_rstride, int64_t out_rstride,
                  float scale, int causal, void* stream);

int alg_quick_gelu(void* x, int64_t numel, void* stream);

int alg_mul_bf16(const void* a, const void* b, void* out, int64_t numel, void* stream);


#define ALG_CONV_PLAIN 0
#define ALG_CONV_PAIR 1
#define ALG_CONV_STRIDE2 2
int alg_conv_cl_bf16(const void* x, const void* w, const void* bias, const void* res, void* y, int frames, int Hp,
                     int Wp, int Cin, int Cout, int kt, int mode, void* stream);

typedef struct alg_vae_geom {
  int32_t frames, H, W, C;
  int32_t first_len, seg_len;
  int32_t lat_first_single;
  int32_t lat_rate, lat_scale;
  int32_t lat_h, lat_w;
} alg_vae_geom;

int64_t alg_vae_groupnorm_workspace(const alg_vae_geom* g);
int alg_vae_groupnorm_stats(const void* x, const alg_vae_geom* g, float eps, void* workspace, float* stats, void* stream);

int alg_vae_spatial_norm(const void* x, const float* stats, const void* gamma, const void* beta, const void* zyb,
                         void* out, const alg_vae_geom* g, int silu, void* stream);

int alg_vae_group_norm(const void* x, const float* stats, const void* gamma, const void* beta, void* out,
                       const alg_vae_geom* g, int silu, void* stream);

int alg_vae_pad(const void* x, void* out, int frames, int H, int W, int C, void* stream);

int alg_vae_repitch(const void* x, void* out, int frames, int H, int W, int C, int src_rows, int src_wp, void* stream);

int alg_vae_unpack_planes(const void* x, void* out, int frames, int H, int W, int C, void* stream);

int alg_vae_upsample(const void* x, void* out, int frames_out, int H, int W, int C, int compress_time, int first_single,
                     void* stream);

int alg_vae_pack_latent(const void* z, int64_t c_stride, int64_t frame_stride, void* out, int frames, int h, int w,
                        int channels, float scale, void* stream);

int alg_vae_unpack_video(const void* x, void* out, int frames, int H, int W, int to_uint8, void* stream);


int alg_headnorm_rope(void* x, const void* weight, const float* cos_tab, const float* sin_tab, int64_t x_rstride,
                      int64_t x_bstride, int batch, int rows, int heads, int rope_tokens, float eps, void* stream);

int alg_masked_mean(const void* x, const int* valid, void* out, int batch, int L, int D, void* stream);

int alg_silu(const void* x, void* y, int64_t numel, void* stream);


int alg_layernorm_mod_f32(const void* x, void* y, const float* weight, const float* bias, const float* scale,
                          const float* shift, int64_t mod_bstride, int batch, int rows, int D, float eps, void* stream);

int alg_layernorm_mod_f32_fp8(const void* x, void* q8, float* q8_scale, const float* weight, const float* bias,
                              const float* scale, const float* shift, int64_t mod_bstride, int batch, int rows, int D,
                              float eps, void* stream);

int alg_rmsnorm_rope(void* x, const void* weight, const float* cos_tab, const float* sin_tab, int64_t x_rstride,
                     int batch, int rows, int D, float eps, void* stream);

int alg_wan_modulation(const float* table, const void* vec, float* out, int layers, int batch, int J, int D,
                       int vec_per_j, void* stream);

int alg_patchify3d(const void* in, void* out, int n, int C, int F, int H, int W, int ph, int pw, int Kpad, void* stream);

int alg_unpatchify3d(const void* in, int64_t ldin, void* out, int n, int C, int F, int H, int W, int ph, int pw,
                     int channel_major, void* stream);

int alg_timestep_embedding_f32(const float* t, float* out, int n, int dim, void* stream);

int alg_linear_f32(const float* x, const float* W, const float* b, float* y, void* y_bf16, void* y_silu_bf16, int M,
                   int N, int K, int act, void* stream);

int alg_gelu_erf(void* x, int64_t numel, void* stream);

int alg_layernorm_modulate(const void* x, void* y, const void* weight, const void* bias, const void* scale,
                           const void* shift, int64_t mod_bstride, int batch, int rows, int D, int64_t x_bstride,
                           int64_t y_bstride, int seg_split, float eps, void* stream);
int alg_layernorm_modulate_seg(const void* x, void* y, const void* weight, const void* bias, const void* scale,
                               const void* shift, int64_t mod_bstride, int64_t seg_stride, int batch, int rows, int D,
                               int64_t x_bstride, int64_t y_bstride, int seg_split, float eps, void* stream);

int alg_qk_norm_rope(void* qk, const void* wq, const void* bq, const void* wk, const void* bk, const float* cos_tab,
                     const float* sin_tab, int batch, int S, int heads, int text_len, float eps, void* stream);

int alg_qk_norm_rope_scaled(void* qk, const void* wq, const void* bq, const void* wk, const void* bk, const float* cos_tab,
                            const float* sin_tab, int batch, int S, int heads, int text_len, float eps, float q_scale,
                            void* stream);

int alg_patchify(const void* latents, int64_t lat_bstride, const void* const* cond_ptrs, void* out, int n_samples,
                 int frames, int C, int H, int W, int p, void* stream);

int alg_unpatchify(const void* in, void* out, int n_samples, int frames, int C, int H, int W, int p, void* stream);

int alg_patchify_t(const void* latents, int64_t lat_bstride, const void* const* cond_ptrs, void* out, int n_samples,
                   int frames, int C, int H, int W, int p, int p_t, void* stream);
int alg_unpatchify_t(const void* in, void* out, int n_samples, int frames, int C, int H, int W, int p, int p_t,
                     void* stream);

int alg_timestep_embedding(const float* t, void* out, int n, int dim, int flip_sin_to_cos, void* stream);


int alg_rms_norm_rows(const void* x, const void* gamma, void* y, int64_t rows, int C, int Cp, int silu, void* stream);

int alg_softmax_hilo(const void* neg_hi, const void* lo, void* p, int64_t rows, int cols, int64_t ld, float scale, void* stream);


int alg_calib_mfma_bf16(float* sink, int iters, unsigned seed, int blocks, uint64_t* clocks, void* stream);

int alg_wall_clock_khz(void);

void alg_attn_clock_tap(uint64_t* buffer, int slots);

#ifdef __cplusplus
}
#endif
#endif
```

Baseline: 1.557 frames/s.

## Fold QKV projection into one packed schedule-11 GEMM with transposed V store

Concatenates the QK and V weights into a single packed-B matrix and runs one schedule-11 GEMM per layer. Output tiles past n_split are written transposed into the V^T buffer via LDS transpose reads (ds_read_tr16) instead of the normal row store. This replaces the previous pair launch (schedule 9/10 QK plus a separate V^T GEMM) and so cuts launch overhead and duplicate A-operand reads. The cost is a more complex epilogue, with strided scalar stores on the unaligned fallback path. It also adds alg_get_opt so the pipe choice is read from the library's options rather than the environment.

```diff
diff --git a/alg_amd/_lib.py b/alg_amd/_lib.py
--- a/alg_amd/_lib.py
+++ b/alg_amd/_lib.py
@@ -16,7 +16,7 @@
 GEMM_B_PACKED11 = 32
 
 EXPORTS = (
-    "alg_version", "alg_last_error", "alg_reload_env", "alg_down_up", "alg_gaussian_blur", "alg_cfg_ddim_step", "alg_gemm_bf16", "alg_gemm_bf16_pair", "alg_gemm_bf16_pair_qk", "alg_pack_b_p11", "alg_pack_b_p11_bytes",
+    "alg_version", "alg_last_error", "alg_reload_env", "alg_get_opt", "alg_down_up", "alg_gaussian_blur", "alg_cfg_ddim_step", "alg_gemm_bf16", "alg_gemm_bf16_pair", "alg_gemm_bf16_pair_qk", "alg_gemm_bf16_qkv", "alg_pack_b_p11", "alg_pack_b_p11_bytes",
     "alg_flash_attn_d64", "alg_layernorm_modulate", "alg_qk_norm_rope", "alg_patchify", "alg_unpatchify",
     "alg_timestep_embedding", "alg_cfg_combine", "alg_lincomb", "alg_unipc_update", "alg_concat_cast", "alg_flash_attn_d128", "alg_layernorm_mod_f32", "alg_layernorm_mod_f32_fp8", "alg_rmsnorm_rope",
     "alg_wan_modulation", "alg_patchify3d", "alg_unpatchify3d", "alg_timestep_embedding_f32", "alg_linear_f32",
@@ -47,6 +47,10 @@
         ("a_scale", c_void_p), ("b_scale", c_void_p), ("strideAScale", c_int64), ("strideBScale", c_int64),
         ("conv_wp", c_int32), ("conv_hpwp", c_int32), ("conv_kw", c_int32), ("reserved1", c_int32),
     ]
+
+
+class GemmVtArgs(Structure):
+    _fields_ = [("vt", c_void_p), ("ldvt", c_int64), ("strideVt", c_int64), ("n_split", c_int32), ("col0", c_int32)]
 
 
 class QkNormRopeArgs(Structure):
@@ -151,6 +155,8 @@
     lib.alg_gemm_bf16.argtypes = [POINTER(GemmArgs), c_void_p]
     lib.alg_gemm_bf16_pair.argtypes = [POINTER(GemmArgs), POINTER(GemmArgs), c_void_p]
     lib.alg_gemm_bf16_pair_qk.argtypes = [POINTER(GemmArgs), POINTER(GemmArgs), POINTER(QkNormRopeArgs), c_void_p]
+    lib.alg_gemm_bf16_qkv.argtypes = [POINTER(GemmArgs), POINTER(GemmVtArgs), c_void_p]
+    lib.alg_get_opt.argtypes = [c_char_p, POINTER(c_int)]
     lib.alg_flash_attn_d64.argtypes = [c_void_p, c_void_p, c_void_p, c_void_p, c_int, c_int, c_int, c_int64, c_int64,
                                        c_int64, c_int64, c_int64, c_int64, c_float, c_void_p]
     lib.alg_layernorm_modulate.argtypes = [c_void_p, c_void_p, c_void_p, c_void_p, c_void_p, c_void_p, c_int64, c_int,
@@ -180,6 +186,16 @@
 
 def reload_env():
     load_library().alg_reload_env()
+
+
+def get_opt(name):
+    v = c_int(0)
+    _check(load_library().alg_get_opt(name.encode(), byref(v)), "alg_get_opt")
+    return v.value
+
+
+def gemm_pipe():
+    return get_opt("ALG_GEMM_PIPE")
 
 
 def _check(rc, what):
@@ -740,6 +756,15 @@
     _check(lib.alg_gemm_bf16_pair(ctypes.byref(a), ctypes.byref(b), _stream()), "alg_gemm_bf16_pair")
 
 
+def gemm_qkv(vt, ldvt, strideVt, n_split, *a, col0=0, **kw):
+    lib = load_library()
+    args, fp8 = gemm_args(*a, **kw)
+    if fp8:
+        raise AlgHipError("gemm_qkv takes bf16 operands")
+    v = GemmVtArgs(vt.data_ptr(), ldvt, strideVt, n_split, col0)
+    _check(lib.alg_gemm_bf16_qkv(ctypes.byref(args), ctypes.byref(v), _stream()), "alg_gemm_bf16_qkv")
+
+
 def gemm_pair_qk(first, second, wq, bq, wk, bk, cos, sin, heads, text_len, eps, q_scale=1.0):
     lib = load_library()
     a, fa = gemm_args(*first[0], **first[1])
diff --git a/alg_amd/csrc/capi.hip b/alg_amd/csrc/capi.hip
--- a/alg_amd/csrc/capi.hip
+++ b/alg_amd/csrc/capi.hip
@@ -68,5 +68,14 @@
 }
 
 extern "C" void alg_reload_env(void) { alg::load_options(); }
+extern "C" int alg_get_opt(const char* name, int* value) {
+  for (int i = 0; name && value && i < alg::OPT_COUNT; ++i)
+    if (strcmp(name, alg::g_defs[i].name) == 0) {
+      *value = alg::opt((alg::Opt)i);
+      return ALG_OK;
+    }
+  alg::set_error("alg_get_opt: unknown option %s", name ? name : "(null)");
+  return ALG_EINVAL;
+}
 extern "C" int alg_version(void) { return ALG_VERSION; }
 extern "C" const char* alg_last_error(void) { return alg::g_err; }
diff --git a/alg_amd/csrc/gemm.hip b/alg_amd/csrc/gemm.hip
--- a/alg_amd/csrc/gemm.hip
+++ b/alg_amd/csrc/gemm.hip
@@ -16,6 +16,7 @@
 int launch_gemm_p10_pair_qk(const alg_gemm_args* a, int m_tiles_a, int n_tiles_a, const alg_gemm_args* b, int m_tiles_b, int n_tiles_b,
                             const alg_qk_norm_rope_args* e, hipStream_t s);
 int launch_gemm_p11(const alg_gemm_args* a, int m_tiles, int n_tiles, int64_t nwg, hipStream_t s);
+int launch_gemm_p11_vt(const alg_gemm_args* a, const alg_gemm_vt_args* v, int m_tiles, int n_tiles, int64_t nwg, hipStream_t s);
 int launch_gemm_p6_fp8(const alg_gemm_args* a, int m_tiles, int n_tiles, int64_t nwg, hipStream_t s);
 int launch_gemm_p9_fp8(const alg_gemm_args* a, int m_tiles, int n_tiles, int64_t nwg, hipStream_t s);
 int launch_gemm_p6_conv(const alg_gemm_args* a, int m_tiles, int n_tiles, int64_t nwg, hipStream_t s);
@@ -210,6 +211,49 @@
   if (rc != ALG_OK) return rc;
   return alg_qk_norm_rope_scaled(a->C, e->wq, e->bq, e->wk, e->bk, e->cos_tab, e->sin_tab, a->batch, a->M, e->heads, e->text_len,
                                  e->eps, e->q_scale, stream);
+}
+
+extern "C" int alg_gemm_bf16_qkv(const alg_gemm_args* a, const alg_gemm_vt_args* v, void* stream) {
+  int rc = gemm_entry(a, stream, false, true);
+  if (rc != ALG_OK) return rc;
+  if (!v || !v->vt) {
+    set_error("alg_gemm_bf16_qkv: null V^T output");
+    return ALG_EINVAL;
+  }
+  if (!(a->flags & ALG_GEMM_B_PACKED11) || a->R || a->gate || a->act != ALG_ACT_NONE || (a->N & 7) || v->n_split <= 0 ||
+      v->n_split >= a->N || v->n_split % BN) {
+    set_error("alg_gemm_bf16_qkv: needs a packed B (ALG_GEMM_B_PACKED11), no residual / gate / activation, N %% 8 == 0 and "
+              "0 < n_split < N with n_split a multiple of %d (N=%d n_split=%d)", BN, a->N, v->n_split);
+    return ALG_EINVAL;
+  }
+  const int64_t vrows = (int64_t)a->N - v->n_split;
+  if (v->col0 < 0 || v->ldvt < ((int64_t)v->col0 + a->M + 15) / 16 * 16 || ((uintptr_t)v->vt & 1) ||
+      (a->batch > 1 && v->strideVt < vrows * v->ldvt) || v->strideVt < 0) {
+    set_error("alg_gemm_bf16_qkv: V^T rows must hold columns perm(col0 + s) for s < M (ldvt=%lld col0=%d M=%d), batch items must "
+              "not overlap (strideVt=%lld)", (long long)v->ldvt, v->col0, a->M, (long long)v->strideVt);
+    return ALG_EINVAL;
+  }
+  const int64_t rows = (int64_t)a->M * a->ldc >= (1ll << 31) ? ((1ll << 31) - 1) / a->ldc / BM * BM : a->M;
+  if (rows <= 0) {
+    set_error("alg_gemm_bf16_qkv: M*ldc must stay below 2^31 (32-bit epilogue offsets)");
+    return ALG_ELIMIT;
+  }
+  if ((int64_t)((a->M + BM - 1) / BM) * ((a->N + BN - 1) / BN) * a->batch > 0x7fffffff) {
+    set_error("alg_gemm_bf16_qkv: grid too large");
+    return ALG_ELIMIT;
+  }
+  for (int64_t m0 = 0; m0 < a->M; m0 += rows) {
+    alg_gemm_args c = *a;
+    alg_gemm_vt_args w = *v;
+    c.M = (int32_t)((a->M - m0) < rows ? (a->M - m0) : rows);
+    c.A = (const char*)a->A + m0 * a->lda * 2;
+    c.C = (char*)a->C + m0 * a->ldc * 2;
+    w.col0 = (int32_t)(v->col0 + m0);
+    const int m_tiles = (c.M + BM - 1) / BM, n_tiles = (c.N + BN - 1) / BN;
+    rc = launch_gemm_p11_vt(&c, &w, m_tiles, n_tiles, (int64_t)m_tiles * n_tiles * c.batch, (hipStream_t)stream);
+    if (rc != ALG_OK) return rc;
+  }
+  return ALG_OK;
 }
 
 extern "C" int alg_gemm_fp8(const alg_gemm_args* a, void* stream) { return gemm_entry(a, stream, true); }
diff --git a/alg_amd/csrc/gemm_kernel.h b/alg_amd/csrc/gemm_kernel.h
--- a/alg_amd/csrc/gemm_kernel.h
+++ b/alg_amd/csrc/gemm_kernel.h
@@ -111,9 +111,15 @@
 struct GemmPairQkArgs : GemmPairArgs {
   QkNormRope qe;
 };
+struct GemmVtArgs {
+  bf16_t* vt;
+  int64_t ldvt, strideVt;
+  int n_split, col0;
+};
 template <int PAIR> struct GemmPairT { typedef GemmNoPair type; };
 template <> struct GemmPairT<1> { typedef GemmPairArgs type; };
 template <> struct GemmPairT<2> { typedef GemmPairQkArgs type; };
+template <> struct GemmPairT<3> { typedef GemmVtArgs type; };
 template <int ACT, bool RES, int PIPE, int WNW = 4, bool FP8 = false, bool CONV = false, int PAIR = 0>
 __global__ __launch_bounds__((PIPE == 11 ? 1 : 2) * WNW * 64) void gemm_bf16_kernel(
     const alg_gemm_args p1, int m_tiles1, int n_tiles1, int group_m1, const typename GemmPairT<PAIR>::type pr) {
@@ -122,7 +128,10 @@
   constexpr bool P11 = PIPE == 11;
   constexpr int WMW = P11 ? 1 : 2;
   constexpr int MT = BM / WMW / 32;
-  static_assert(!PAIR || (P9 && !P11 && !RES && ACT == ALG_ACT_NONE), "the pair launch is built for the plain schedule-9 / 10 kernels");
+  constexpr bool PAIRED = PAIR == 1 || PAIR == 2;
+  constexpr bool VTS = PAIR == 3;
+  static_assert(!PAIRED || (P9 && !P11 && !RES && ACT == ALG_ACT_NONE), "the pair launch is built for the plain schedule-9 / 10 kernels");
+  static_assert(!VTS || (P11 && !RES && ACT == ALG_ACT_NONE), "the transposed V store is built for the plain schedule-11 kernel");
   static_assert(!FP8 || PIPE == 6 || PIPE == 9, "the fp8 operands are built on the ping-pong schedule and on schedule 9");
   static_assert(!CONV || (PIPE == 6 && !FP8), "the convolution addressing is built on the bf16 ping-pong schedule");
   typedef typename std::conditional<FP8, uint8_t, bf16_t>::type elem_t;
@@ -162,13 +171,13 @@
   const int total1 = m_tiles1 * n_tiles1 * p1.batch;
   auto do_tile = [&](const int wg_in) __attribute__((always_inline)) {
   bool second = false;
-  if constexpr (PAIR) second = wg_in >= total1;
+  if constexpr (PAIRED) second = wg_in >= total1;
   const alg_gemm_args& p = [&]() -> const alg_gemm_args& {
-    if constexpr (PAIR) return second ? pr.p : p1;
+    if constexpr (PAIRED) return second ? pr.p : p1;
     else return p1;
   }();
   int m_tiles = m_tiles1, n_tiles = n_tiles1, group_m = group_m1, wg = wg_in;
-  if constexpr (PAIR) {
+  if constexpr (PAIRED) {
     if (second) m_tiles = pr.m_tiles, n_tiles = pr.n_tiles, group_m = pr.group_m, wg = wg_in - total1;
   }
   const int tiles = m_tiles * n_tiles;
@@ -777,6 +786,8 @@
   const int ldc = (int)p.ldc, ldr = (int)p.ldr;
   const int col0 = perm ? p.perm_col0 : 0;
   const bool n_vec = (p.N & 3) == 0 && (col0 & 15) == 0;
+  bool vtile = false;
+  if constexpr (VTS) vtile = n0 >= pr.n_split;
   auto blk_row = [&](int mt) { return PP ? (mt >> 1) * 128 + wm * 64 + (mt & 1) * 32 : wm * (MT * 32) + mt * 32; };
   auto blk_col = [&](int nt) { return PP ? nt * 128 + wn * 32 : wn * (NT * 32) + nt * 32; };
   auto quad_row = [](int q, int ln_) { return M16 ? 16 * (q >> 1) + (ln_ & 15) : (ln_ & 31); };
@@ -785,7 +796,10 @@
   auto cq = [](int q) { return M16 ? q & 1 : q; };
   constexpr int NRQ = M16 ? 2 : 1, NCQ = M16 ? 2 : 4;
   if constexpr (PP || PIPE == 8 || P9) {
-    const bool staged = staged_epilogue() && ((!RES && ACT == ALG_ACT_NONE) || !(bias && bias_row));
+    bool vt_aligned = true;
+    if constexpr (VTS)
+      vt_aligned = !vtile || (((uintptr_t)pr.vt & 15) == 0 && (pr.ldvt & 7) == 0 && (pr.strideVt & 7) == 0 && (pr.col0 & 15) == 0);
+    const bool staged = staged_epilogue() && ((!RES && ACT == ALG_ACT_NONE) || !(bias && bias_row)) && vt_aligned;
     int lane_e = lane, l31_e = l31, h2_e = h2;
     if constexpr (P9) {
       int z = 0;
@@ -851,9 +865,11 @@
           for (int g = 0; g < NCQ; ++g) unpack4(bcol[nt][g], bvf[nt][g]);
       }
       __builtin_amdgcn_sched_barrier(0);
-      auto park_band = [&](auto mt_c, auto br_c) {
+      auto vt_swz = [](int r) { return ((r >> 1) & 2) | ((r >> 3) & 1); };
+      auto park_band = [&](auto mt_c, auto br_c, auto vt_c) {
         constexpr int mt = decltype(mt_c)::value;
         constexpr bool BR = decltype(br_c)::value != 0;
+        constexpr bool VT = decltype(vt_c)::value != 0;
         const float a_sc = a_sc4[mt];
         static_for<NT>([&](auto nt_c) {
           constexpr int nt = decltype(nt_c)::value;
@@ -891,7 +907,8 @@
             o.y = pack_bf2(v[2], v[3]);
             if constexpr (M16) {
               const int pr_ = quad_row(g, lane_e), pc_ = quad_col(g, lane_e);
-              *(uint2*)(my + (mt * NT + nt) * 2048 + pr_ * 64 + (((pc_ >> 3) ^ ((pr_ >> 2) & 3)) * 16) + (pc_ & 7) * 2) = o;
+              const int sw_ = VT ? vt_swz(pr_) : ((pr_ >> 2) & 3);
+              *(uint2*)(my + (mt * NT + nt) * 2048 + pr_ * 64 + (((pc_ >> 3) ^ sw_) * 16) + (pc_ & 7) * 2) = o;
             } else {
               *(uint2*)(my + (mt * NT + nt) * 2048 + l31_e * 64 + ((g ^ ((l31_e >> 2) & 3)) * 16) + h2_e * 8) = o;
             }
@@ -941,11 +958,13 @@
       constexpr bool BR_SPLIT = !RES && ACT == ALG_ACT_NONE;
       constexpr bool BR_ALWAYS = BR_SPLIT && FP8 && PIPE == 9;
       if (BR_ALWAYS) {
-        static_for<MT>([&](auto mt_c) { park_band(mt_c, IntC<1>{}); });
+        static_for<MT>([&](auto mt_c) { park_band(mt_c, IntC<1>{}, IntC<0>{}); });
       } else if (BR_SPLIT && bias && bias_row) {
-        static_for<MT>([&](auto mt_c) { park_band(mt_c, IntC<1>{}); });
+        static_for<MT>([&](auto mt_c) { park_band(mt_c, IntC<1>{}, IntC<0>{}); });
+      } else if (VTS && vtile) {
+        static_for<MT>([&](auto mt_c) { park_band(mt_c, IntC<0>{}, IntC<VTS>{}); });
       } else {
-        static_for<MT>([&](auto mt_c) { park_band(mt_c, IntC<0>{}); });
+        static_for<MT>([&](auto mt_c) { park_band(mt_c, IntC<0>{}, IntC<0>{}); });
       }
       }
       asm volatile("s_waitcnt lgkmcnt(0)" ::: "memory");
@@ -1070,6 +1089,56 @@
             __builtin_amdgcn_sched_barrier(0);
           });
         };
+        if constexpr (VTS) {
+          if (vtile) {
+            typedef short v4s __attribute__((ext_vector_type(4)));
+            typedef unsigned int u32x2 __attribute__((ext_vector_type(2)));
+            typedef __attribute__((address_space(3))) v4s* lv4_t;
+            const int grp = lane_e >> 4, li = lane_e & 15, pp = li & 3;
+            const int t_lane = 16 * (grp >> 1) + 4 * (grp & 1);
+            const int ra_ = t_lane + (li >> 2), rb_ = ra_ + 8;
+            const int offA = ra_ * 64 + (((pp >> 1) ^ vt_swz(ra_)) * 16) + (pp & 1) * 8;
+            const int offB = rb_ * 64 + (((pp >> 1) ^ vt_swz(rb_)) * 16) + (pp & 1) * 8;
+            const char* const lds_a[2] = {my + offA, my + (offA ^ 32)};
+            const char* const lds_b[2] = {my + offB, my + (offB ^ 32)};
+            const int dcol = n0 + wn * 64 + li;
+            bf16_t* const vrow = pr.vt + (int64_t)b * pr.strideVt + (int64_t)(dcol - pr.n_split) * pr.ldvt + pr.col0 + m0 + 8 * grp;
+            v4s ra[2][2 * NT], rb[2][2 * NT];
+            auto read_band = [&](auto mt_c) {
+              constexpr int mt = decltype(mt_c)::value;
+              static_for<2 * NT>([&](auto u_c) {
+                constexpr int u = decltype(u_c)::value, nt = u >> 1, h = u & 1;
+                ra[mt & 1][u] = __builtin_amdgcn_ds_read_tr16_b64_v4i16((lv4_t)(lds_a[h] + (mt * NT + nt) * 2048));
+                rb[mt & 1][u] = __builtin_amdgcn_ds_read_tr16_b64_v4i16((lv4_t)(lds_b[h] + (mt * NT + nt) * 2048));
+              });
+            };
+            read_band(IntC<0>{});
+            static_for<MT>([&](auto mt_c) {
+              constexpr int mt = decltype(mt_c)::value;
+              if constexpr (mt + 1 < MT) read_band(IntC<mt + 1>{});
+              const int tok = m0 + mt * 32 + t_lane;
+              static_for<2 * NT>([&](auto u_c) {
+                constexpr int u = decltype(u_c)::value, nt = u >> 1, h = u & 1;
+                if (dcol + nt * 32 + h * 16 < p.N) {
+                  bf16_t* const dst = vrow + (int64_t)(nt * 32 + h * 16) * pr.ldvt + mt * 32;
+                  const v4s va = ra[mt & 1][u], vb = rb[mt & 1][u];
+                  const u32x2 wa = __builtin_bit_cast(u32x2, va), wb = __builtin_bit_cast(u32x2, vb);
+                  if (tok + 11 < p.M) {
+                    ALG_STORE16(dst, make_uint4(wa[0], wa[1], wb[0], wb[1]));
+                  } else {
+#pragma unroll
+                    for (int e = 0; e < 4; ++e) {
+                      if (tok + e < p.M) dst[e] = (bf16_t)va[e];
+                      if (tok + 8 + e < p.M) dst[4 + e] = (bf16_t)vb[e];
+                    }
+                  }
+                }
+              });
+              __builtin_amdgcn_sched_barrier(0);
+            });
+            return;
+          }
+        }
         if constexpr (PAIR == 2) {
           if (!second) {
             const QkNormRope& e = pr.qe;
@@ -1261,7 +1330,16 @@
               if (RES) x = gate_f32 ? rv[i] + gv[i] * x : rv[i] + rbf(gv[i] * x);
               v[i] = x;
             }
-            if (row_ok) {
+            if (VTS && vtile) {
+              if (row_ok) {
+                if constexpr (VTS) {
+                  const int j = pr.col0 + row, jc = (j & ~12) | ((j & 4) << 1) | ((j & 8) >> 1);
+                  bf16_t* const vq = pr.vt + (int64_t)b * pr.strideVt + (int64_t)(n - pr.n_split) * pr.ldvt + jc;
+#pragma unroll
+                  for (int i = 0; i < 4; ++i) vq[i * pr.ldvt] = f2bf(v[i]);
+                }
+              }
+            } else if (row_ok) {
               const int nc = perm ? col0 + ((n & ~12) | ((n & 4) << 1) | ((n & 8) >> 1)) : n;
               uint2 o;
               o.x = pack_bf2(v[0], v[1]);
@@ -1301,7 +1379,7 @@
   };
 
   int total_wg = total1;
-  if constexpr (PAIR) total_wg += pr.m_tiles * pr.n_tiles * pr.p.batch;
+  if constexpr (PAIRED) total_wg += pr.m_tiles * pr.n_tiles * pr.p.batch;
   for (int L = blockIdx.x; L < total_wg; L += gridDim.x) {
     const int xcd = L & 7, q = total_wg >> 3, r = total_wg & 7;
     const int wg = (xcd < r ? xcd * (q + 1) : r * (q + 1) + (xcd - r) * q) + (L >> 3);
diff --git a/alg_amd/csrc/gemm_p11.hip b/alg_amd/csrc/gemm_p11.hip
--- a/alg_amd/csrc/gemm_p11.hip
+++ b/alg_amd/csrc/gemm_p11.hip
@@ -3,6 +3,25 @@
 namespace alg {
 int launch_gemm_p11(const alg_gemm_args* a, int m_tiles, int n_tiles, int64_t nwg, hipStream_t s) {
   return launch_gemm<11, 4>(a, m_tiles, n_tiles, nwg, s);
+}
+
+int launch_gemm_p11_vt(const alg_gemm_args* a, const alg_gemm_vt_args* v, int m_tiles, int n_tiles, int64_t nwg, hipStream_t s) {
+  const void* fn = (const void*)gemm_bf16_kernel<ALG_ACT_NONE, false, 11, 4, false, false, 3>;
+  static PerDeviceOnce attr_set;
+  const int dev_slot = current_device_slot();
+  if (!device_done(attr_set, dev_slot)) {
+    hipError_t e = hipFuncSetAttribute(fn, hipFuncAttributeMaxDynamicSharedMemorySize, GEMM_LDS_P9);
+    if (e != hipSuccess) {
+      set_error("alg_gemm_bf16_qkv: hipFuncSetAttribute(%d B LDS): %s", GEMM_LDS_P9, hipGetErrorString(e));
+      return ALG_ELAUNCH;
+    }
+    device_mark(attr_set, dev_slot);
+  }
+  GemmVtArgs vt;
+  vt.vt = (bf16_t*)v->vt, vt.ldvt = v->ldvt, vt.strideVt = v->strideVt, vt.n_split = v->n_split, vt.col0 = v->col0;
+  hipLaunchKernelGGL((gemm_bf16_kernel<ALG_ACT_NONE, false, 11, 4, false, false, 3>), dim3(gemm_grid(nwg)), dim3(256), GEMM_LDS_P9, s,
+                     *a, m_tiles, n_tiles, gemm_group_m(11, n_tiles, a->K), vt);
+  return check_launch("alg_gemm_bf16_qkv");
 }
 
 __global__ __launch_bounds__(256) void pack_b_p11_kernel(const bf16_t* __restrict__ w, uint4* __restrict__ out, int N, int K, int64_t ldb,
diff --git a/alg_amd/transformer_cogvideox.py b/alg_amd/transformer_cogvideox.py
--- a/alg_amd/transformer_cogvideox.py
+++ b/alg_amd/transformer_cogvideox.py
@@ -1,7 +1,6 @@
 from __future__ import annotations
 
 import math
-import os
 from dataclasses import dataclass, asdict
 from typing import Optional
 
@@ -70,6 +69,8 @@
         self.pair_qkv = True
         self.fuse_qk_norm = False
         self.packed_weights = True
+        self.packed_qkv = True
+        self.gemm_pipe = _lib.gemm_pipe()
         self._sincos = {}
         dev = self.device
         w = weights
@@ -120,6 +121,8 @@
             L["bf2"] = _bf(w[b + "ff.net.2.bias"], dev)
             for nm in ("wo", "wf1", "wf2"):
                 L["p" + nm] = _lib.PackedB(L[nm])
+            L["pwqkv"] = _lib.PackedB(torch.cat([L["wqk"], L["wv"]], dim=0))
+            L["bqkv"] = torch.cat([L["bqk"], L["bv"]]).contiguous()
             self.layers.append(L)
         ow, ob = w["norm_out.linear.weight"], w["norm_out.linear.bias"]
         sh_w, sc_w = ow.chunk(2, dim=0)
@@ -313,7 +316,8 @@
         prescale = self.attn_prescale
         q_scale = scale * 1.4426950408889634 if prescale else 1.0
         F4 = cfg.ff_inner_mult * D
-        packed = self.packed_weights and os.environ.get("ALG_GEMM_PIPE", "10") == "10"
+        packed = self.packed_weights and self.gemm_pipe == 10
+        fold_qkv = packed and self.packed_qkv and not (self.pair_qkv and self.fuse_qk_norm)
         wo_k, wf1_k, wf2_k = ("pwo", "pwf1", "pwf2") if packed else ("wo", "wf1", "wf2")
         for li, L in enumerate(self.layers):
             m1 = li * 12 * D
@@ -327,7 +331,10 @@
                 TM("gemm_qkv", _lib.gemm_pair_qk, qk_call, vt_call, L["norm_q_w"], L["norm_q_b"], L["norm_k_w"], L["norm_k_b"], cos, sin,
                                Hn, T, cfg.qk_norm_eps, q_scale=q_scale)
             else:
-                if self.pair_qkv:
+                if fold_qkv:
+                    TM("gemm_qkv", _lib.gemm_qkv, vt, S_pad, D * S_pad, 2 * D, y, L["pwqkv"], qk, S, 3 * D, D, D, D, 2 * D,
+                       bias=L["bqkv"], batch=N, strideA=S * D, strideC=S * 2 * D)
+                elif self.pair_qkv:
                     TM("gemm_qkv", _lib.gemm_pair, qk_call, vt_call)
                 else:
                     TM("gemm_qk", G, *qk_call[0], **qk_call[1])
diff --git a/include/alg_hip.h b/include/alg_hip.h
--- a/include/alg_hip.h
+++ b/include/alg_hip.h
@@ -21,6 +21,8 @@
 const char* alg_last_error(void);
 
 void alg_reload_env(void);
+
+int alg_get_opt(const char* name, int* value);
 
 
 int alg_down_up(const void* in, void* out, int64_t planes, int H, int W, int h1, int w1, int dtype,
@@ -103,6 +105,14 @@
 } alg_qk_norm_rope_args;
 int alg_gemm_bf16_pair_qk(const alg_gemm_args* qk, const alg_gemm_args* vt, const alg_qk_norm_rope_args* e, void* stream);
 
+typedef struct alg_gemm_vt_args {
+  void* vt;
+  int64_t ldvt, strideVt;
+  int32_t n_split;
+  int32_t col0;
+} alg_gemm_vt_args;
+int alg_gemm_bf16_qkv(const alg_gemm_args* a, const alg_gemm_vt_args* v, void* stream);
+
 int alg_gemm_fp8(const alg_gemm_args* args, void* stream);
 
 int alg_quantize_fp8_rows(const void* x, int64_t x_rstride, void* q, float* scale, int64_t rows, int K, void* stream);
```

Result: no change. 1.566 frames/s, median of 6 (+0.6%).
